# jmhb0/view_neti

Measured on AMD Instinct MI355X. Metric: TI train steps/sec (SD-1.5 512^2 bs=4 per GPU), higher is better.
Workload: dtype f16; 1 GPU; learnable_mode 0, sd15 shapes, 512x512 fp16, bs=4/GPU, grad_accum 1, full train step (VAE+16xCLIP+UNet fwd/bwd+AdamW); global_batch=4, parallelism=dp1, rccl_ranks=1, hipgraph=True

## Files before the change

include/vneti.h:

```cpp
#ifndef VNETI_H
#define VNETI_H
#include <stddef.h>
#include <stdint.h>

#ifdef __cplusplus
extern "C" {
#endif

#define VNETI_ABI_VERSION 1

int vneti_version(void);
int vneti_precision(void);
int vneti_last_error(char* buf, size_t n);

typedef struct vneti_gemm_desc {
  const void* A;
  const void* B;
  void* C;
  long long lda, ldb, ldc;
  int M, N, K;
  int batch;
  long long strideA, strideB, strideC;
  const float* bias;
  const void* rowadd;
  long long ld_rowadd;
  int rows_per_group;
  const void* resid;
  long long ldr;
  float alpha;
  int act;
  int out_f32;
  int conv_mode;
  int Hi, Wi, Ci, Ho, Wo, stride, pad_t, pad_l, ups;
  long long ldx;
  int tile_hint;
  void* workspace;
  long long workspace_bytes;
  int split_k;
  const void* gate_src;
  long long ld_gate;
  int gate_act;
  void* C2;
  long long ldc2;
  int act2;
  void* gn_sums;
  int gn_hw, gn_cpg, gn_groups, gn_slots;
  int geglu;
  int conv_korder;
} vneti_gemm_desc;

int vneti_gemm_f16(const vneti_gemm_desc* d, void* stream);
int vneti_gemm_select_tile(int M, int N, int batch);
int vneti_gemm_select_split(int M, int N, int K, int batch, int tile_hint, long long workspace_bytes);

int vneti_im2col3x3_small(const void* x, int x_is_f32, long long sb, long long sc, long long sy,
                          long long sx, void* out, int Bn, int C, int Hi, int Wi, int Ho, int Wo,
                          int stride, int pad_t, int pad_l, void* stream);

int vneti_conv3x3_in(const void* x, int x_is_f32, long long sb, long long sc, long long sy, long long sx,
                     const void* w_packed, const float* bias, void* out, long long ldo, int Bn, int C, int H, int W,
                     int Co, void* gn_sums, int gn_groups, int gn_slots, void* stream);

int vneti_transpose_f16(const void* in, long long ld_in, long long stride_in, void* out,
                        long long ld_out, long long stride_out, int rows, int cols, int batch,
                        void* stream);
#define VNETI_TRANSPOSE_MAX 4
typedef struct vneti_transpose_desc {
  const void* inp;
  long long ld_in, stride_in;
  void* out;
  long long ld_out, stride_out;
  int rows, cols, batch, _pad;
} vneti_transpose_desc;
int vneti_transpose_f16_multi(const vneti_transpose_desc* descs, int n, void* stream);

long long vneti_groupnorm_ws_floats(int Bn, int HW, int C, int G);
int vneti_groupnorm_fwd(const void* x, long long ldx, void* y, long long ldy, const float* gamma,
                        const float* beta, float* mean, float* rstd, float* ws, int Bn, int HW,
                        int C, int G, float eps, int silu, void* stream);
int vneti_groupnorm_fwd_sums(const void* x, long long ldx, void* y, long long ldy, const float* gamma,
                             const float* beta, const void* sums, int slots, float* mean, float* rstd,
                             int Bn, int HW, int C, int G, float eps, int silu, void* stream);
int vneti_groupnorm_fwd_2l(const void* x, long long ldx, void* y, long long ldy, const float* gamma,
                           const float* beta, void* sums, int slots, float* mean, float* rstd, int Bn, int HW,
                           int C, int G, float eps, int silu, void* stream);
int vneti_groupnorm_bwd_2l(const void* dy, long long lddy, const void* x, long long ldx, const float* gamma,
                           const float* beta, const float* mean, const float* rstd, void* dx, long long lddx,
                           const void* dx_accum, long long ldacc, void* sums, int slots, float* ws, int Bn,
                           int HW, int C, int G, int silu, void* stream);
int vneti_groupnorm_bwd(const void* dy, long long lddy, const void* x, long long ldx,
                        const float* gamma, const float* beta, const float* mean,
                        const float* rstd, void* dx, long long lddx, const void* dx_accum,
                        long long ldacc, float* ws, int Bn, int HW, int C, int G, int silu,
                        void* stream);

int vneti_layernorm_fwd(const void* x, int x_is_f32, long long ldx, void* y, long long ldy,
                        const float* gamma, const float* beta, float* mean, float* rstd, int rows,
                        int C, float eps, void* stream);
int vneti_layernorm_bwd(const void* dy, int dy_is_f32, long long lddy, const void* x,
                        int x_is_f32, long long ldx, const float* gamma, const float* mean,
                        const float* rstd, void* dx, int dx_is_f32, long long lddx,
                        const void* dx_accum, long long ldacc, void* dx_f16_copy, long long ldcopy,
                        int rows, int C, void* stream);

int vneti_attn_fwd(const void* Q, long long ldq, const void* K, long long ldk, const void* V,
                   long long ldv, void* O, long long ldo, float* lse, int Bn, int H, int Nq,
                   int Nk, int D, float scale, int causal, void* stream);
int vneti_attn_bwd_delta(const void* dO, long long lddo, const void* O, long long ldo,
                         float* delta, int Bn, int H, int Nq, int D, void* stream);
int vneti_attn_bwd_dq(const void* Q, long long ldq, const void* K, long long ldk, const void* V,
                      long long ldv, const void* dO, long long lddo, const float* lse, float* delta,
                      const void* O, long long ldo, void* dQ, long long lddq, int Bn, int H, int Nq,
                      int Nk, int D, float scale, int causal, void* stream);
int vneti_attn_bwd_dkv(const void* Q, long long ldq, const void* K, long long ldk, const void* V,
                       long long ldv, const void* dO, long long lddo, const float* lse,
                       const float* delta, void* dK, long long lddk, void* dV, long long lddv,
                       int Bn, int H, int Nq, int Nk, int D, float scale, int causal, float* ws,
                       long long ws_floats, void* stream);
int vneti_attn_bwd_small(const void* Q, long long ldq, const void* K, long long ldk, const void* V, long long ldv,
                         const void* dO, long long lddo, const void* O, long long ldo, const float* lse, void* dQ,
                         long long lddq, void* dK, long long lddk, void* dV, long long lddv, int Bn, int H, int N, int D,
                         float scale, int causal, void* stream);
int vneti_softmax_rows_f16(void* x, long long ld, int rows, int cols, void* stream);

int vneti_add_f16(const void* a, long long lda, const void* b, long long ldb, void* out,
                  long long ldo, int rows, int cols, void* stream);
int vneti_geglu_fwd(const void* p, long long ldp, void* out, long long ldo, int rows, int C4,
                    void* stream);
int vneti_geglu_bwd(const void* dy, long long lddy, const void* p, long long ldp, void* dp,
                    long long lddp, int rows, int C4, void* stream);
int vneti_act_fwd_f16(const void* x, void* y, long long n, int act, void* stream);
int vneti_act_bwd_f16(const void* dy, const void* x, void* dx, long long n, int act, void* stream);
int vneti_timestep_embedding(const void* t, void* out, int Bn, int dim, void* stream);
int vneti_sum2x2_f16(const void* in, long long ldi, void* out, long long ldo, int Bn, int H, int W,
                     int C, void* stream);
int vneti_rng_fill_normal(void* out_f32, long long n, const void* state, unsigned stream_id,
                          void* stream);
int vneti_rng_fill_randint(void* out_i64, int n, int high, const void* state, unsigned stream_id,
                           void* stream);
int vneti_rng_advance(void* state, void* stream);
int vneti_nested_dropout_mask(float* mask, int nl, int Bn, int hidden, float prob, const void* state,
                              unsigned stream_id, void* stream);
int vneti_sample_add_noise(const void* moments, long long ldm, const float* eps,
                           const float* noise, const void* timesteps_i64,
                           const float* alphas_cumprod, float scaling, int v_prediction,
                           float* latents, float* noisy, float* target, int Bn, int Lc, int HW,
                           void* stream);
int vneti_latent_sample(const void* moments, long long ldm, const float* eps, float scaling, float* latents, int Bn,
                        int Lc, int HW, void* stream);
int vneti_add_noise(const float* latents, const float* noise, const void* timesteps_i64, const float* alphas_cumprod,
                    int v_prediction, float* noisy, float* target, int Bn, int Lc, int HW, void* stream);
int vneti_cfg_sampler_step(const void* pred, long long ldp, float* x, float* m_prev, float* x_in, int Bn,
                           int Lc, int HW, float guidance, float alpha_t, float sigma_t, float cx,
                           float c0, float c1, int v_prediction, void* stream);
int vneti_cfg_sampler_step_table(const void* pred, long long ldp, float* x, float* m_prev, float* x_in,
                                 int Bn, int Lc, int HW, float guidance, const float* coef_table,
                                 const int* step, int v_prediction, void* stream);
int vneti_cfg_sampler_step_noise(const void* pred, long long ldp, float* x, float* m_prev, float* x_in,
                                 const float* noise, int Bn, int Lc, int HW, float guidance, float alpha_t,
                                 float sigma_t, float cx, float c0, float c1, float cn, int v_prediction, void* stream);
int vneti_cfg_sampler_step_noise_table(const void* pred, long long ldp, float* x, float* m_prev, float* x_in, int Bn,
                                       int Lc, int HW, float guidance, const float* coef_table,
                                       const float* noise_table, const int* step, int v_prediction, void* stream);
int vneti_table_fill_i64(void* dst_i64, int n, const void* table_i64, const int* step, void* stream);
int vneti_counter_advance(int* counter, void* stream);
int vneti_conv1x1_nchw_f32(const float* x, const float* W, const float* bias, float* out, int Bn, int Ci,
                           int Co, int HW, float in_scale, void* stream);
int vneti_image_postprocess(const void* img, long long ldi, float* out, long long n_pix, int channels,
                            void* stream);
int vneti_mse_loss_grad(const void* pred, long long ldp, const float* target, void* dpred,
                        long long lddp, float* loss_sum, const float* loss_scale, int Bn, int Lc,
                        int HW, void* stream);
int vneti_mse_loss_per_sample(const void* pred, long long ldp, const float* target, float* out, float* ws, int Bn, int Lc,
                              int HW, void* stream);
long long vneti_mse_loss_per_sample_ws_floats(int Bn, int HW);
#define VNETI_OPT_CHECK 1
#define VNETI_OPT_APPLY 2
#define VNETI_OPT_FINISH 4
#define VNETI_OPT_ALL 7
int vneti_adamw_flat(float* p, const float* g, float* m, float* v, long long n, const float* hyper,
                     float* scaler, int* step, int growth_interval, int phases, void* stream);
int vneti_adamw_segments(float* p, const float* g, float* m, float* v, long long seg_len, int n_seg,
                         int* seg_step, const int* active, int n_active, const float* hyper,
                         float* scaler, int* step, int growth_interval, int phases, void* stream);
long long vneti_grad_sumsq_ws_doubles(long long len, int n_active);
int vneti_grad_sumsq(const float* g, long long len, const int* active, int n_active, void* ws, void* stream);
#define VNETI_NORM_OUT_FLOATS 5
int vneti_grad_norm_finish(const void* ws_object, long long n_object, const void* ws_view, long long n_view,
                           const float* scaler, const float* hyper, const float* max_norm, float* out, float* ring,
                           const int* count, int rows, int row_floats, void* stream);
int vneti_adamw_flat_clipped(float* p, const float* g, float* m, float* v, long long n, const float* hyper,
                             float* scaler, int* step, int growth_interval, int phases, const float* clip_coef,
                             void* stream);
int vneti_adamw_segments_clipped(float* p, const float* g, float* m, float* v, long long seg_len, int n_seg,
                                 int* seg_step, const int* active, int n_active, const float* hyper, float* scaler,
                                 int* step, int growth_interval, int phases, const float* clip_coef, void* stream);
#define VNETI_TELEMETRY_SEQ 0
#define VNETI_TELEMETRY_MICRO 1
#define VNETI_TELEMETRY_CLOSED 2
#define VNETI_TELEMETRY_NORM_OBJECT 3
#define VNETI_TELEMETRY_NORM_VIEW 4
#define VNETI_TELEMETRY_NORM_TOTAL 5
#define VNETI_TELEMETRY_FINITE 6
#define VNETI_TELEMETRY_CLIP_COEF 7
#define VNETI_TELEMETRY_LOSS_SCALE 8
#define VNETI_TELEMETRY_LR 9
#define VNETI_TELEMETRY_HEADER 10
int vneti_train_record(float* ring, int* count, int rows, int row_floats, int first_micro, const void* timesteps_i64,
                       const float* losses, int Bn, void* stream);

long long vneti_mapper_num_params(int enc_dim, int hidden, int D, int has_bypass);
long long vneti_mapper_save_floats(int R, int enc_dim, int hidden);
long long vneti_mapper_rowgrad_floats(int R, int hidden, int D, int has_bypass);
int vneti_mapper_fwd(const float* params, const int* slot, long long slot_stride, const float* data,
                     int nfeat, const float* w_enc,
                     const float* hidden_mask, float norm_scale, float* word, float* bypass,
                     float* save, int R, int enc_dim, int hidden, int D, int has_bypass, const float* enc_in,
                     void* stream);
int vneti_mapper_fwd_slots(const float* params, const int* slots, long long slot_stride, int Bn, const float* data,
                           int nfeat, const float* w_enc, const float* hidden_mask, float norm_scale, float* word,
                           float* bypass, float* save, int R, int enc_dim, int hidden, int D, int has_bypass,
                           const float* enc_in, void* stream);
int vneti_mapper_bwd(const float* params, const int* slot, long long slot_stride,
                     const float* hidden_mask, float norm_scale,
                     const float* word, const float* dword_src, const int* dword_rows,
                     long long ld_src, const float* dbypass, const float* save, float* rowgrads,
                     float* grads, int accumulate, int R, int enc_dim, int hidden, int D,
                     int has_bypass, float* denc, void* stream);
long long vneti_mapper_legacy_input_params(int enc_dim, int pe_dim);
int vneti_mapper_legacy_input_fwd(const float* params_in, const int* slot, long long slot_stride,
                                  const void* timesteps_i64, const float* w_pe, float* enc_out, int nl, int Bn,
                                  int enc_dim, int pe_dim, void* stream);
int vneti_mapper_legacy_input_fwd_slots(const float* params_in, const int* slots, long long slot_stride,
                                        const void* timesteps_i64, const float* w_pe, float* enc_out, int nl, int Bn,
                                        int enc_dim, int pe_dim, void* stream);
int vneti_mapper_legacy_input_bwd(const void* timesteps_i64, const float* w_pe, const float* denc, float* grads_in,
                                  const int* slot, long long slot_stride, int accumulate, int nl, int Bn, int enc_dim,
                                  int pe_dim, void* stream);
int vneti_text_embed(const float* tok_emb, const float* pos_emb, const void* ids_i64,
                     const int* pos_obj, const float* word_obj, const int* pos_view,
                     const float* word_view, float* X, int nl, int Bn, int L, int D, void* stream);
int vneti_text_final_fwd(const float* last, const float* gamma, const float* beta, float eps,
                         const int* pos_obj, const float* bypass_obj, float alpha_obj,
                         int unconstrained_obj, const int* pos_view, const float* bypass_view,
                         float alpha_view, int unconstrained_view, float* norm_terms, void* ctx_k,
                         void* ctx_v, int nl, int Bn, int L, int D, void* stream);
int vneti_text_final_bwd(const float* last, const float* gamma, float eps, const int* pos_obj,
// ... 43 lines not shown
```

view_neti_amd/csrc/gemm_conv.hip:

```cpp
#include "common.h"
#include "gemm_args.h"
#include "../../include/vneti.h"

namespace {

template <int BM, int BN, int WM, int WN, bool F32OUT, bool DMA, int NSTG = 2, int EPI = 2, bool CONV = true>
__global__ __launch_bounds__((BM / WM) * (BN / WN) * 64) void gemm_kernel(
    const half_t* pA, const half_t* pB, uint32_t p_a_bytes, uint32_t p_b_bytes, int p_lda, int p_ldb, int pM, int pN, int pK,
    int p_tiles_m, int p_tiles_n, int p_split_conv , const GemmArgs gfull) {
  GemmArgs g = gfull;
  g.A = pA;
  g.B = pB;
  g.a_bytes = p_a_bytes;
  g.b_bytes = p_b_bytes;
  g.lda = p_lda;
  g.ldb = p_ldb;
  g.M = pM;
  g.N = pN;
  g.K = pK;
  g.tiles_m = p_tiles_m;
  g.tiles_n = p_tiles_n;
  g.kt_per_split = p_split_conv & 0xffff;
  g.ksplit = (p_split_conv >> 16) & 0xff;
  g.conv_mode = p_split_conv >> 24;
  static_assert(NSTG == 2 || ((NSTG == 3 || NSTG == 4) && DMA), "the LDS rings are LDS-DMA only");
  const half_t* const e_gate = EPI == 2 ? g.gate_src : nullptr;
  half_t* const e_C2 = EPI == 2 ? g.C2 : nullptr;
  const int e_geglu = EPI == 2 ? g.geglu : 0;
  const int e_act = EPI == 2 ? g.act : 0;
  float* const e_gn_sums = EPI >= 1 ? g.gn_sums : nullptr;
  const half_t* const e_rowadd = EPI >= 1 ? g.rowadd : nullptr;
  const int e_conv = CONV ? g.conv_mode : 0;
  constexpr int NWM = BM / WM, NWN = BN / WN;
  constexpr int NT = NWM * NWN * 64;
  constexpr int RSTEP = NT / 8;
  constexpr int A_IT = BM / RSTEP, B_IT = BN / RSTEP;
  constexpr int STAGE_BYTES = (BM + BN) * 128;
  constexpr int CS_LD = F32OUT ? (BN + 4) : (BN + 8);
  constexpr int CS_BYTES = BM * CS_LD * (F32OUT ? 4 : 2);
  constexpr int LDS_BYTES = (NSTG * STAGE_BYTES > CS_BYTES) ? NSTG * STAGE_BYTES : CS_BYTES;
  constexpr int GN_IMG = 5, GN_NG = BN / 4 + 2;
  constexpr int GN_BYTES = (F32OUT || EPI == 0) ? 0 : GN_IMG * GN_NG * 4 * 8;
  __shared__ __attribute__((aligned(16))) char smem[LDS_BYTES + GN_BYTES];

  const int tid = threadIdx.x;
  const int lane = tid & 63;
  const int wave = __builtin_amdgcn_readfirstlane(tid >> 6);
  const int wm0 = (wave / NWN) * WM;
  const int wn0 = (wave % NWN) * WN;

  int nblk = g.tiles_m * g.tiles_n;
  int bid = blockIdx.x;
  {
    int q = nblk >> 3, r = nblk & 7, xcd = bid & 7, idx = bid >> 3;
    bid = (xcd < r ? xcd * (q + 1) : r * (q + 1) + (xcd - r) * q) + idx;
  }
  const int tile_m = bid / g.tiles_n;
  const int tile_n = bid - tile_m * g.tiles_n;
  const int m0 = tile_m * BM;
  const int n0 = tile_n * BN;
  const int bz = blockIdx.y;
  const int kz = blockIdx.z;

  const half_t* Ab = g.A + (long long)bz * g.strideA;
  const half_t* Bb = g.B + (long long)bz * g.strideB;
  __amdgpu_buffer_rsrc_t rsA = vn_make_rsrc(Ab, g.a_bytes);
  __amdgpu_buffer_rsrc_t rsB = vn_make_rsrc(Bb, g.b_bytes);

  const int lrow = tid >> 3;
  const int gchunk = DMA ? ((tid & 7) ^ ((lrow >> 1) & 7)) : (tid & 7);

  const float rcp_hw = CONV ? __builtin_amdgcn_rcpf((float)(g.Ho * g.Wo)) : 0.f, rcp_wo = CONV ? __builtin_amdgcn_rcpf((float)g.Wo) : 0.f;
  int a_off[A_IT];
  int a_py[A_IT], a_px[A_IT], a_bh[A_IT];
#pragma unroll
  for (int i = 0; i < A_IT; ++i) {
    int m = m0 + lrow + RSTEP * i;
    bool ok = m < g.M;
    if (e_conv == 0) {
      a_off[i] = ok ? (int)((long long)m * g.lda * 2) + gchunk * 16 : -1;
      a_py[i] = a_px[i] = a_bh[i] = 0;
    } else {
      int rem, ox;
      const int b = vn_divmod(m, g.Ho * g.Wo, rcp_hw, rem);
      const int oy = vn_divmod(rem, g.Wo, rcp_wo, ox);
      a_bh[i] = ok ? b * g.Hi : -1;
      if (e_conv == 1) {
        a_py[i] = oy * g.stride - g.pad_t;
        a_px[i] = ox * g.stride - g.pad_l;
      } else {
        a_py[i] = oy + g.pad_t;
        a_px[i] = ox + g.pad_l;
      }
      a_off[i] = ((b * g.Hi + a_py[i]) * g.Wi + a_px[i]) * g.ldx2 + gchunk * 16;
    }
  }
  int b_off[B_IT];
#pragma unroll
  for (int i = 0; i < B_IT; ++i) {
    int n = n0 + lrow + RSTEP * i;
    b_off[i] = (n < g.N) ? (int)((long long)n * g.ldb * 2) + gchunk * 16 : -1;
  }

  u32x4 ra[DMA ? 1 : A_IT], rb[DMA ? 1 : B_IT];

  auto a_offset = [&](int i, int k0, int dy, int dx, int tapoff) -> uint32_t {
    if (e_conv == 0) return a_off[i] < 0 ? VN_OOB : (uint32_t)(a_off[i] + k0 * 2);
    bool ok = a_bh[i] >= 0;
    if (e_conv == 1 && !g.ups) {
      int iy = a_py[i] + dy, ix = a_px[i] + dx;
      ok = ok && (unsigned)iy < (unsigned)g.Hi && (unsigned)ix < (unsigned)g.Wi;
      return ok ? (uint32_t)(a_off[i] + tapoff) : VN_OOB;
    }
    int iy, ix;
    if (e_conv == 1) {
      iy = a_py[i] + dy;
      ix = a_px[i] + dx;
      ok = ok && (unsigned)iy < (unsigned)(2 * g.Hi) && (unsigned)ix < (unsigned)(2 * g.Wi);
      iy >>= 1;
      ix >>= 1;
    } else {
      int ty = a_py[i] - dy, tx = a_px[i] - dx;
      ok = ok && ty >= 0 && tx >= 0;
      if (g.stride == 2) {
        ok = ok && ((ty | tx) & 1) == 0;
        ty >>= 1;
        tx >>= 1;
      }
      iy = ty;
      ix = tx;
      ok = ok && iy < g.Hi && ix < g.Wi;
    }
    return ok ? (uint32_t)(((a_bh[i] + iy) * g.Wi + ix) * g.ldx2 + tapoff) : VN_OOB;
  };

  uint32_t a_cur[A_IT], b_cur[B_IT];
#pragma unroll
  for (int i = 0; i < B_IT; ++i) b_cur[i] = b_off[i] < 0 ? VN_OOB : (uint32_t)b_off[i];

  auto issue = [&](int kt, int stage, bool first) {
    const int k0 = kt * 64;
    bool recompute = first;
    int dy = 0, dx = 0, tapoff = 0;
    if (e_conv != 0) {
      int tap, ci0;
      if (g.korder) {
        const int chunk = kt / 9;
        tap = kt - chunk * 9;
        ci0 = chunk << 6;
        recompute = true;
      } else {
        tap = k0 / g.Ci;
        ci0 = k0 - tap * g.Ci;
        recompute = recompute || ci0 == 0;
// ... 272 lines not shown
      }
      s_lo = q_lo = s_hi = q_hi = 0.f;
    };
    for (int idx = tid; idx < BM * CPR; idx += NT) {
      int r = idx / CPR, c = (idx - r * CPR) * 8;
      int m = m0 + r, n = n0 + c;
      const bool valid = m < g.M && n < g.N;
      if (gn) {
        int gn_rem;
        const int img = valid ? vn_divmod(m, g.gn_hw, rcp_gnhw, gn_rem) : gn_img;
        if (__any(img != gn_img)) {
          gn_flush();
          gn_img = img;
        }
      }
      if (!valid) continue;
      half8 v = as_half8(*reinterpret_cast<const u32x4*>(smem + ((size_t)r * CS_LD + c) * 2));
      int ra_rem;
      const half_t* radd = e_rowadd ? e_rowadd + (long long)vn_divmod(m, g.rows_per_group, rcp_rpg, ra_rem) * g.ld_rowadd + n : nullptr;
      if (n + 8 <= g.N) {
        if (radd) {
          half8 t = *reinterpret_cast<const half8*>(radd);
          v = vn_add8(v, t);
        }
        if (Rb) {
          half8 rr = *reinterpret_cast<const half8*>(Rb + (long long)m * g.ldr + n);
          v = vn_add8(v, rr);
        }
        if (e_geglu == 2) {
          const half_t* pp = e_gate + (long long)m * g.ld_gate + 2 * n;
#pragma unroll
          for (int c2 = 0; c2 < 2; ++c2) {
            const half8 pre = *reinterpret_cast<const half8*>(pp + 8 * c2);
            half8 o;
#pragma unroll
            for (int e = 0; e < 4; ++e) {
              const float d = (float)v[4 * c2 + e], hh = (float)pre[e], gg = (float)pre[4 + e];
              float cdf, xpdf;
              vn_gelu_parts(gg, cdf, xpdf);
              o[e] = (half_t)(d * gg * cdf);
              o[4 + e] = (half_t)(d * hh * (cdf + xpdf));
            }
            vn_st16_wt(rsC, (uint32_t)(((long long)m * g.ldc + 2 * n + 8 * c2) * 2), o);
          }
          continue;
        }
        if (e_gate) {
          half8 pre = *reinterpret_cast<const half8*>(e_gate + (long long)m * g.ld_gate + n);
#pragma unroll
          for (int e = 0; e < 8; ++e) v[e] = (half_t)((float)v[e] * act_grad((float)pre[e], g.gate_act));
        }
        if (e_geglu == 1 || (e_C2 && e_geglu == 0)) vn_st16_wt_saved(rsC, (uint32_t)(((long long)m * g.ldc + n) * 2), v);
        else vn_st16_wt(rsC, (uint32_t)(((long long)m * g.ldc + n) * 2), v);
        if (e_geglu == 1) {
          half4 o2;
#pragma unroll
          for (int e = 0; e < 4; ++e) o2[e] = (half_t)((float)v[e] * vn_gelu_erf((float)v[4 + e]));
          *reinterpret_cast<half4*>(e_C2 + (long long)m * g.ldc2 + (n >> 1)) = o2;
        }
        if (gn) {
#pragma unroll
          for (int e = 0; e < 8; ++e) {
            const float x = (float)v[e];
            if (e < gn_split) {
              s_lo += x;
              q_lo += x * x;
            } else {
              s_hi += x;
              q_hi += x * x;
            }
          }
        }
        if (e_C2 && e_geglu == 0) {
          half8 o2;
#pragma unroll
          for (int e = 0; e < 8; ++e) o2[e] = (half_t)apply_act((float)v[e], g.act2);
          vn_st16_wt(rsC2, (uint32_t)(((long long)m * g.ldc2 + n) * 2), o2);
        }
      } else {
        for (int e = 0; e < 8 && n + e < g.N; ++e) {
          float x = (float)v[e];
          if (radd) x = (float)(half_t)(x + (float)radd[e]);
          if (Rb) x = (float)(half_t)(x + (float)Rb[(long long)m * g.ldr + n + e]);
          if (e_gate) x = (float)(half_t)(x * act_grad((float)e_gate[(long long)m * g.ld_gate + n + e], g.gate_act));
          Cb[(long long)m * g.ldc + n + e] = (half_t)x;
          if (e_C2) e_C2[(long long)m * g.ldc2 + n + e] = (half_t)apply_act((float)(half_t)x, g.act2);
          if (gn) {
            const float xs = (float)(half_t)x;
            if (e < gn_split) {
              s_lo += xs;
              q_lo += xs * xs;
            } else {
              s_hi += xs;
              q_hi += xs * xs;
            }
          }
        }
      }
    }
    if (gn) {
      gn_flush();
      __syncthreads();
      const int slot = tile_m % g.gn_slots;
      for (int i = tid; i < GN_IMG * GN_NG; i += NT) {
        const vn_u64* src = gacc + 4 * i;
        if ((src[0] | src[1] | src[2] | src[3]) == 0) continue;
        const int img = gn_img0 + i / GN_NG, grp = gn_g0t + i % GN_NG;
        vn_u64* dst = reinterpret_cast<vn_u64*>(e_gn_sums) + (((long long)img * g.gn_slots + slot) * g.gn_G + grp) * 4;
#pragma unroll
        for (int w = 0; w < 4; ++w) atomicAdd(dst + w, src[w]);
      }
    }
  }
}

__global__ __launch_bounds__(256) void splitk_reduce_kernel(
    float* p_ws, void* pC, const float* p_bias, const void* p_resid, const half_t* p_rowadd, int pM, int pN, int p_batch,
    int p_ksplit, int p_ldc, int p_ldr, const GemmArgs gfull) {
  GemmArgs g = gfull;
  g.ws = p_ws;
  g.C = pC;
  g.bias = p_bias;
  g.resid = p_resid;
  g.rowadd = p_rowadd;
  g.M = pM;
  g.N = pN;
  g.batch = p_batch;
  g.ksplit = p_ksplit;
  g.ldc = p_ldc;
  g.ldr = p_ldr;
  const unsigned n4 = (unsigned)(g.N + 3) / 4;
  const unsigned gid = blockIdx.x * 256u + threadIdx.x;
  const unsigned total = (unsigned)g.batch * (unsigned)g.M * n4;
  if (gid >= total) return;
  const unsigned row = gid / n4;
  const int c = (int)(gid - row * n4) * 4;
  const int bz = g.batch > 1 ? (int)(row / (unsigned)g.M) : 0;
  const int m = (int)(row - (unsigned)bz * (unsigned)g.M);
  const int ne = min(4, g.N - c);
  const long long zstride = (long long)g.batch * g.M * g.N;
  const float* p0 = g.ws + ((long long)bz * g.M + m) * g.N + c;
  if ((g.N & 3) == 0 && ((g.ldc | g.ldr | g.ld_rowadd | g.ld_gate | g.ldc2) & 3) == 0) {
    const long long co = (long long)bz * g.strideC + (long long)m * g.ldc + c;
    const long long ro = (long long)bz * g.strideC + (long long)m * g.ldr + c;
    f32x4 bv = {0.f, 0.f, 0.f, 0.f}, rf = {0.f, 0.f, 0.f, 0.f};
    half4 rh = {0, 0, 0, 0}, ra = {0, 0, 0, 0}, gt = {0, 0, 0, 0};
    if (g.bias) bv = *reinterpret_cast<const f32x4*>(g.bias + c);
    if (g.resid) {
      if (g.out_f32) rf = *reinterpret_cast<const f32x4*>(reinterpret_cast<const float*>(g.resid) + ro);
      else rh = *reinterpret_cast<const half4*>(reinterpret_cast<const half_t*>(g.resid) + ro);
    }
    if (g.rowadd) ra = *reinterpret_cast<const half4*>(g.rowadd + (long long)(m / g.rows_per_group) * g.ld_rowadd + c);
    if (g.gate_src) gt = *reinterpret_cast<const half4*>(g.gate_src + (long long)m * g.ld_gate + c);
    f32x4 v = {0.f, 0.f, 0.f, 0.f};
    int z = 0;
    for (; z + 4 <= g.ksplit; z += 4) {
      const f32x4 t0 = *reinterpret_cast<const f32x4*>(p0 + (z + 0) * zstride);
      const f32x4 t1 = *reinterpret_cast<const f32x4*>(p0 + (z + 1) * zstride);
      const f32x4 t2 = *reinterpret_cast<const f32x4*>(p0 + (z + 2) * zstride);
      const f32x4 t3 = *reinterpret_cast<const f32x4*>(p0 + (z + 3) * zstride);
      v += t0;
      v += t1;
      v += t2;
      v += t3;
    }
    for (; z < g.ksplit; ++z) v += *reinterpret_cast<const f32x4*>(p0 + z * zstride);
    float x[4];
#pragma unroll
    for (int e = 0; e < 4; ++e) {
      x[e] = v[e] * g.alpha;
      if (g.bias) x[e] += bv[e];
      x[e] = apply_act(x[e], g.act);
    }
    if (g.out_f32) {
      f32x4 o = {x[0], x[1], x[2], x[3]};
      if (g.resid) o += rf;
      vn_st16_wt(vn_make_rsrc(g.C, 0x7fffffffu), (uint32_t)(co * 4), o);
    } else {
      half4 o, o2;
#pragma unroll
      for (int e = 0; e < 4; ++e) {
        float y = (float)(half_t)x[e];
        if (g.rowadd) y = (float)(half_t)(y + (float)ra[e]);
        if (g.resid) y = (float)(half_t)(y + (float)rh[e]);
        if (g.gate_src) y = (float)(half_t)(y * act_grad((float)gt[e], g.gate_act));
        o[e] = (half_t)y;
        o2[e] = (half_t)apply_act((float)(half_t)y, g.act2);
      }
      *reinterpret_cast<half4*>(reinterpret_cast<half_t*>(g.C) + co) = o;
      if (g.C2) *reinterpret_cast<half4*>(g.C2 + (long long)m * g.ldc2 + c) = o2;
    }
    return;
  }
  float v[4] = {0.f, 0.f, 0.f, 0.f};
  for (int z = 0; z < g.ksplit; ++z) {
    const float* p = p0 + z * zstride;
    for (int e = 0; e < ne; ++e) v[e] += p[e];
  }
  for (int e = 0; e < ne; ++e) {
    float x = v[e] * g.alpha;
    if (g.bias) x += g.bias[c + e];
    x = apply_act(x, g.act);
    if (g.out_f32) {
      if (g.resid) x += reinterpret_cast<const float*>(g.resid)[(long long)bz * g.strideC + (long long)m * g.ldr + c + e];
      reinterpret_cast<float*>(g.C)[(long long)bz * g.strideC + (long long)m * g.ldc + c + e] = x;
    } else {
      x = (float)(half_t)x;
      if (g.rowadd) x = (float)(half_t)(x + (float)g.rowadd[(long long)(m / g.rows_per_group) * g.ld_rowadd + c + e]);
      if (g.resid)
        x = (float)(half_t)(x + (float)reinterpret_cast<const half_t*>(g.resid)[(long long)bz * g.strideC + (long long)m * g.ldr + c + e]);
      if (g.gate_src) x = (float)(half_t)(x * act_grad((float)g.gate_src[(long long)m * g.ld_gate + c + e], g.gate_act));
      reinterpret_cast<half_t*>(g.C)[(long long)bz * g.strideC + (long long)m * g.ldc + c + e] = (half_t)x;
      if (g.C2) g.C2[(long long)m * g.ldc2 + c + e] = (half_t)apply_act((float)(half_t)x, g.act2);
    }
  }
}

inline int epilogue_level(const GemmArgs& g) {
  if (g.gate_src || g.C2 || g.geglu || g.act) return 2;
  return (g.gn_sums || g.rowadd) ? 1 : 0;
}

template <int BM, int BN, int WM, int WN, bool F32OUT, bool DMA, int NSTG>
void launch_variant(const GemmArgs& g, dim3 grid, hipStream_t st) {
  const dim3 block((BM / WM) * (BN / WN) * 64);
#define VN_GO(E, C)                                                                                                        \
  hipLaunchKernelGGL((gemm_kernel<BM, BN, WM, WN, F32OUT, DMA, NSTG, E, C>), grid, block, 0, st, g.A, g.B, g.a_bytes, g.b_bytes, \
                     (int)g.lda, (int)g.ldb, g.M, g.N, g.K, g.tiles_m, g.tiles_n, g.kt_per_split | (g.ksplit << 16) | (g.conv_mode << 24), g)
  if constexpr (F32OUT) {
    if (g.conv_mode) { if (g.act) VN_GO(2, true); else VN_GO(0, true); }
    else { if (g.act) VN_GO(2, false); else VN_GO(0, false); }
  } else {
    const int epi = epilogue_level(g);
    if (g.conv_mode) { if (epi == 2) VN_GO(2, true); else if (epi == 1) VN_GO(1, true); else VN_GO(0, true); }
    else { if (epi == 2) VN_GO(2, false); else if (epi == 1) VN_GO(1, false); else VN_GO(0, false); }
  }
#undef VN_GO
}

inline void launch_reduce(const GemmArgs& g, hipStream_t st) {
  if (g.ksplit > 1) {
    long long total = (long long)g.batch * g.M * ((g.N + 3) / 4);
    hipLaunchKernelGGL(splitk_reduce_kernel, dim3((unsigned)cdivl(total, 256)), dim3(256), 0, st, g.ws, g.C, g.bias, g.resid,
                       g.rowadd, g.M, g.N, g.batch, g.ksplit, (int)g.ldc, (int)g.ldr, g);
  }
}

template <int BM, int BN, int WM, int WN, bool DMA>
int launch_cfg(GemmArgs& g, bool f32out, hipStream_t st) {
  g.tiles_m = cdiv(g.M, BM);
  g.tiles_n = cdiv(g.N, BN);
  dim3 grid(g.tiles_m * g.tiles_n, g.batch, g.ksplit);
  if (f32out) launch_variant<BM, BN, WM, WN, true, DMA, 2>(g, grid, st);
  else launch_variant<BM, BN, WM, WN, false, DMA, 2>(g, grid, st);
  launch_reduce(g, st);
  return vneti_check_launch("gemm_kernel");
}

template <int BM, int BN, int WM, int WN, int NSTG = 3>
int launch_cfg_ring(GemmArgs& g, bool f32out, hipStream_t st) {
  g.tiles_m = cdiv(g.M, BM);
  g.tiles_n = cdiv(g.N, BN);
  dim3 grid(g.tiles_m * g.tiles_n, g.batch, g.ksplit);
  if (f32out) launch_variant<BM, BN, WM, WN, true, true, NSTG>(g, grid, st);
  else launch_variant<BM, BN, WM, WN, false, true, NSTG>(g, grid, st);
  launch_reduce(g, st);
  return vneti_check_launch("gemm_kernel");
}

template <int BM, int BN, int WM, int WN, bool DMA>
int launch_cfg_f16(GemmArgs& g, hipStream_t st) {
  g.tiles_m = cdiv(g.M, BM);
  g.tiles_n = cdiv(g.N, BN);
  dim3 grid(g.tiles_m * g.tiles_n, g.batch, g.ksplit);
  launch_variant<BM, BN, WM, WN, false, DMA, 2>(g, grid, st);
  launch_reduce(g, st);
  return vneti_check_launch("gemm_kernel");
}

struct TileDims {
  int bm, bn;
};
constexpr int kMaxTile = 18;
constexpr TileDims kTiles[kMaxTile + 1] = {{0, 0},     {128, 128}, {128, 64},  {64, 64},  {256, 128}, {256, 256}, {256, 128}, {256, 128},
                                          {256, 128}, {128, 128}, {128, 128}, {128, 64},  {64, 64},   {128, 128}, {128, 64},  {64, 64},
                                          {256, 256}, {256, 128}, {256, 128}};

int select_tile(int M, int N, int batch) {
  long long t256 = (long long)cdiv(M, 256) * cdiv(N, 128) * batch;
  long long t128 = (long long)cdiv(M, 128) * cdiv(N, 128) * batch;
  long long t12864 = (long long)cdiv(M, 128) * cdiv(N, 64) * batch;
  if (N <= 64) return (M >= 2048) ? 2 : 3;
  (void)t256;
  if (t128 >= 384) return 1;
  if (t12864 >= 384) return 2;
  return 3;
}

int select_ksplit(int M, int N, int K, int batch, int tile, long long ws_floats) {
  if (ws_floats <= 0) return 1;
  const int nk = K / 64;
  long long tiles = (long long)cdiv(M, kTiles[tile].bm) * cdiv(N, kTiles[tile].bn) * batch;
  if (tiles >= 256 || nk < 16) return 1;
  int s = (int)(512 / tiles);
  if (s > nk / 8) s = nk / 8;
  if (s > 16) s = 16;
  while (s > 1 && (long long)s * batch * M * N > ws_floats) --s;
  return s < 2 ? 1 : s;
}

}

extern "C" int vneti_gemm_select_tile(int M, int N, int batch) { return select_tile(M, N, batch > 0 ? batch : 1); }

extern "C" int vneti_gemm_select_split(int M, int N, int K, int batch, int tile_hint, long long workspace_bytes) {
  if (batch <= 0) batch = 1;
  int cfg = tile_hint >= 100 ? tile_hint - 100 : tile_hint;
  if (cfg == 0) cfg = select_tile(M, N, batch);
  if (cfg < 1 || cfg > kMaxTile || K % 64 != 0) return -1;
  int ks = select_ksplit(M, N, K, batch, cfg, workspace_bytes / 4);
  const int nk = K / 64;
  if (ks > nk) ks = nk;
  if (ks < 1) ks = 1;
  return cdiv(nk, cdiv(nk, ks));
}

extern "C" int vneti_gemm_f16(const vneti_gemm_desc* d, void* stream) {
  VN_REQUIRE(d != nullptr, "gemm: null descriptor");
  VN_REQUIRE(d->A && d->B && d->C, "gemm: null operand pointer");
  VN_REQUIRE(d->M > 0 && d->N > 0 && d->K > 0, "gemm: bad shape M=%d N=%d K=%d", d->M, d->N, d->K);
  VN_REQUIRE(d->K % 64 == 0, "gemm: K=%d must be a multiple of 64", d->K);
  VN_REQUIRE(d->ldb % 8 == 0, "gemm: ldb=%lld must be a multiple of 8", d->ldb);
  int batch = d->batch > 0 ? d->batch : 1;
  GemmArgs g;
  memset(&g, 0, sizeof(g));
  g.A = (const half_t*)d->A;
  g.B = (const half_t*)d->B;
  g.C = d->C;
  g.bias = d->bias;
  g.rowadd = (const half_t*)d->rowadd;
  g.resid = d->resid;
  g.gate_src = (const half_t*)d->gate_src;
  g.ld_gate = d->ld_gate;
  g.gate_act = d->gate_act;
  g.C2 = (half_t*)d->C2;
  g.ldc2 = d->ldc2;
  g.act2 = d->act2;
  g.gn_sums = (float*)d->gn_sums;
  g.gn_hw = d->gn_hw;
  g.gn_cpg = d->gn_cpg;
  g.gn_G = d->gn_groups;
  g.gn_slots = d->gn_slots;
  g.geglu = d->geglu;
  g.lda = d->lda;
  g.ldb = d->ldb;
  g.ldc = d->ldc;
  g.ld_rowadd = d->ld_rowadd;
  g.ldr = d->ldr;
  g.strideA = d->strideA;
  g.strideB = d->strideB;
  g.strideC = d->strideC;
  g.M = d->M;
  g.N = d->N;
  g.K = d->K;
  g.batch = batch;
  g.rows_per_group = d->rows_per_group > 0 ? d->rows_per_group : 1;
  g.alpha = d->alpha;
  g.act = d->act;
  g.out_f32 = d->out_f32 ? 1 : 0;
  g.conv_mode = d->conv_mode;
  long long a_bytes;
  if (d->conv_mode == 0) {
    VN_REQUIRE(d->lda % 8 == 0, "gemm: lda=%lld must be a multiple of 8", d->lda);
    a_bytes = ((long long)(d->M - 1) * d->lda + d->K) * 2;
  } else {
    VN_REQUIRE(d->conv_mode == 1 || d->conv_mode == 2, "gemm: bad conv_mode %d", d->conv_mode);
    VN_REQUIRE(d->Ci > 0 && d->Ci % 64 == 0, "conv: Ci=%d must be a multiple of 64", d->Ci);
    VN_REQUIRE(d->K == 9 * d->Ci, "conv: K=%d must equal 9*Ci=%d", d->K, 9 * d->Ci);
    VN_REQUIRE(d->stride == 1 || d->stride == 2, "conv: stride %d unsupported", d->stride);
    VN_REQUIRE(d->Ho > 0 && d->Wo > 0 && d->M % (d->Ho * d->Wo) == 0, "conv: M=%d not a multiple of Ho*Wo", d->M);
    VN_REQUIRE(d->ldx % 8 == 0, "conv: ldx must be a multiple of 8");
    VN_REQUIRE(!(d->ups && d->conv_mode != 1), "conv: fused upsample only in forward gather mode");
    VN_REQUIRE(!(d->ups && d->stride != 1), "conv: fused upsample needs stride 1");
    g.Hi = d->Hi;
    g.Wi = d->Wi;
    g.Ci = d->Ci;
    g.Ho = d->Ho;
    g.Wo = d->Wo;
    g.stride = d->stride;
    g.pad_t = d->pad_t;
    g.pad_l = d->pad_l;
    g.ups = d->ups;
    g.ldx2 = (int)(d->ldx * 2);
    VN_REQUIRE(!d->conv_korder || d->Ci % 64 == 0, "conv: conv_korder=1 needs Ci=%d to be a multiple of 64", d->Ci);
    g.korder = d->conv_korder ? 1 : 0;
    long long nb = d->M / (d->Ho * d->Wo);
    a_bytes = nb * d->Hi * d->Wi * d->ldx * 2;
  }
  long long b_bytes = ((long long)(d->N - 1) * d->ldb + d->K) * 2;
  VN_REQUIRE(a_bytes < 0x7fffffffLL && b_bytes < 0x7fffffffLL, "gemm: operand larger than 2 GiB");
  g.a_bytes = (uint32_t)a_bytes;
  g.b_bytes = (uint32_t)b_bytes;
  if (!d->out_f32) {
    VN_REQUIRE(d->ldc % 8 == 0 || d->N < 8, "gemm: ldc=%lld must be a multiple of 8", d->ldc);
  }
  VN_REQUIRE_OUT("gemm C", vn_out_bytes(d->M, d->ldc, d->N, d->out_f32 ? 4 : 2, batch, d->strideC));
  if (d->C2) VN_REQUIRE_OUT("gemm C2", vn_out_bytes(d->M, d->ldc2, d->geglu == 1 ? d->N / 2 : d->N, 2));
  hipStream_t st = (hipStream_t)stream;
  bool f32 = d->out_f32 != 0;
  VN_REQUIRE(!(f32 && d->rowadd), "gemm: rowadd is only supported for f16 output");
  if (d->gate_src || d->C2) {
    VN_REQUIRE(!f32 && batch == 1, "gemm: gate/C2 epilogues need f16 output and batch 1");
    VN_REQUIRE(!d->gate_src || (d->gate_act >= 1 && d->gate_act <= 3 && d->ld_gate % 8 == 0), "gemm: bad gate arguments");
    VN_REQUIRE(!d->C2 || (d->act2 >= 0 && d->act2 <= 3 && d->ldc2 % 8 == 0), "gemm: bad C2 arguments");
  }

  if (d->geglu) {
    VN_REQUIRE(d->geglu == 1 || d->geglu == 2, "gemm: geglu must be 0, 1 or 2");
    VN_REQUIRE(!f32 && batch == 1 && d->N % 8 == 0, "gemm: geglu needs f16 output, batch 1 and N %% 8 == 0");
    VN_REQUIRE(d->split_k == 1, "gemm: geglu needs split_k = 1 (it lives in the fused epilogue)");
    VN_REQUIRE(!d->gn_sums, "gemm: geglu and gn_sums are exclusive");
    if (d->geglu == 1) {
      VN_REQUIRE(d->C2 && d->ldc2 % 4 == 0 && !d->gate_src, "gemm: geglu forward needs C2 ([M][N/2]) and no gate");
    } else {
      VN_REQUIRE(d->gate_src && d->ld_gate % 8 == 0 && !d->C2 && !d->resid && !d->rowadd,
                 "gemm: geglu backward needs gate_src ([M][2N] saved pre-activation) and a plain epilogue");
      VN_REQUIRE(d->ldc % 8 == 0, "gemm: geglu backward writes [M][2N]: ldc %% 8");
    }
  }
  if (d->gn_sums) {
    VN_REQUIRE(!f32 && batch == 1, "gemm: gn_sums needs f16 output and batch 1");
    VN_REQUIRE(d->gn_hw >= 64 && d->gn_cpg >= 4 && d->gn_groups > 0 && d->gn_slots > 0 && d->N == d->gn_cpg * d->gn_groups &&
                   d->M % d->gn_hw == 0 && (d->gn_cpg >= 8 || d->gn_cpg == 4),
               "gemm: bad gn_sums geometry hw=%d cpg=%d G=%d", d->gn_hw, d->gn_cpg, d->gn_groups);
    VN_REQUIRE(d->split_k == 1, "gemm: gn_sums needs split_k = 1 (the statistics live in the fused epilogue)");
  }

  int cfg = d->tile_hint;
  bool dma = true;
  if (cfg >= 100) {
    dma = false;
    cfg -= 100;
  }
  if (cfg == 0) cfg = select_tile(d->M, d->N, batch);
  VN_REQUIRE(cfg >= 1 && cfg <= kMaxTile, "gemm: unknown tile_hint %d", d->tile_hint);
  if (cfg == 18 &&
      (d->conv_mode < 1 || d->conv_mode > 2 || d->stride != 1 || d->ups || d->pad_t != 1 || d->pad_l != 1 || d->Hi != d->Ho ||
       d->Wi != d->Wo || (d->Ho & 15) || (d->Wo & 15) || (d->Ci & 63) || !d->conv_korder || batch != 1 || f32))
    cfg = 17;
  if (cfg == 18 && d->gn_sums && (d->gn_cpg & 1)) cfg = 17;
  if ((cfg == 16 || cfg == 17) && (!dma || (d->conv_mode && (d->ups || (d->conv_mode == 2 && d->stride == 2))) ||
                    (d->gn_sums && (d->gn_cpg & 1)) ||
                    (d->M >= (1 << 24) && (d->conv_mode || d->rowadd || d->gn_sums)))) cfg = cfg == 16 ? 5 : 7;
  if ((cfg == 5 || cfg == 16) && f32) cfg = 4;
  if (cfg == 17 && f32) cfg = 7;
  if ((cfg == 6 || cfg == 7) && !dma) cfg = 4;
  if (cfg >= 10 && !dma) cfg = kTiles[cfg].bm == 128 ? (kTiles[cfg].bn == 128 ? 1 : 2) : 3;
  long long ws_floats = d->workspace ? d->workspace_bytes / 4 : 0;
  int ks = d->split_k;
  if (ks == 0) ks = select_ksplit(d->M, d->N, d->K, batch, cfg, ws_floats);
  if (ks < 1) ks = 1;
  const int nk = d->K / 64;
  if (ks > nk) ks = nk;
  if (ks > 1) {
    VN_REQUIRE(d->workspace && (long long)ks * batch * d->M * d->N <= ws_floats,
               "gemm: split_k=%d needs %lld workspace bytes", ks, (long long)ks * batch * d->M * d->N * 4);
    VN_REQUIRE(batch == 1 || (d->strideC != 0), "gemm: batched split-K needs strideC");
    VN_REQUIRE((long long)batch * d->M * ((d->N + 3) / 4) < 0x7fffffffLL, "gemm: split-K output larger than 2^31 chunks");
    VN_REQUIRE_OUT("gemm split-K workspace", (long long)ks * batch * d->M * d->N * 4);
  }
  if (cfg == 18 && ks > d->Ci / 64) ks = d->Ci / 64;
  g.ksplit = ks;
  g.kt_per_split = cdiv(nk, ks);
  g.ksplit = cdiv(nk, g.kt_per_split);
  VN_REQUIRE(g.ksplit <= 255 && g.kt_per_split <= 0xffff, "gemm: split_k=%d / K=%d out of range", g.ksplit, d->K);
  g.ws = (float*)d->workspace;

#define LAUNCH(BM, BN, WM, WN) \
  return dma ? launch_cfg<BM, BN, WM, WN, true>(g, f32, st) : launch_cfg<BM, BN, WM, WN, false>(g, f32, st)
  switch (cfg) {
    case 1: LAUNCH(128, 128, 64, 64);
    case 2: LAUNCH(128, 64, 64, 32);
    case 3: LAUNCH(64, 64, 32, 32);
    case 4: LAUNCH(256, 128, 64, 64);
    case 6: return launch_cfg_ring<256, 128, 64, 64>(g, f32, st);
    case 7: return launch_cfg_ring<256, 128, 64, 32>(g, f32, st);
    case 8: LAUNCH(256, 128, 64, 32);
    case 9: LAUNCH(128, 128, 64, 32);
    case 10: return launch_cfg_ring<128, 128, 64, 32>(g, f32, st);
    case 11: return launch_cfg_ring<128, 64, 64, 32>(g, f32, st);
    case 12: return launch_cfg_ring<64, 64, 32, 32>(g, f32, st);
    case 13: return launch_cfg_ring<128, 128, 64, 32, 4>(g, f32, st);
    case 14: return launch_cfg_ring<128, 64, 64, 32, 4>(g, f32, st);
    case 15: return launch_cfg_ring<64, 64, 32, 32, 4>(g, f32, st);
    case 16:
    case 17:
    case 18: {
      const int rc = vneti_launch_gemm8(&g, cfg == 16 ? 256 : 128, cfg == 18 ? 1 : 0, st);
      if (rc != VNETI_OK) return rc;
      launch_reduce(g, st);
      return vneti_check_launch("gemm8_kernel");
    }
    default:
      return dma ? launch_cfg_f16<256, 256, 64, 64, true>(g, st) : launch_cfg_f16<256, 256, 64, 64, false>(g, st);
  }
#undef LAUNCH
}
```

view_neti_amd/csrc/norms.hip:

```cpp
#include "common.h"
#include "../../include/vneti.h"

namespace {

#ifndef GN_APPLY_U
#define GN_APPLY_U 4
#endif
struct GNGeom {
  int Bn, HW, C, G, cpg, CC, TX, TY, rps, nslab;
  double inv_n;
};

__device__ __forceinline__ void vn_mean_rstd(double s0, double s1, double inv_n, float eps, float& m, float& r) {
  const double mu = s0 * inv_n;
  const double var = s1 * inv_n - mu * mu;
  const float v = fmaxf((float)var, 0.f) + eps;
  float y = __builtin_amdgcn_rsqf(v);
  y = y * (1.5f - 0.5f * v * y * y);
  m = (float)mu;
  r = y;
}

__device__ __forceinline__ void gn_thread_coords(const GNGeom& g, int& tx, int& ty, bool& active) {
  int tid = threadIdx.x;
  tx = tid % g.TX;
  ty = tid / g.TX;
  active = ty < g.TY;
}

template <bool BWD, bool SILU, bool SLOTS = false>
__global__ __launch_bounds__(256) void gn_stats_kernel(GNGeom g, const half_t* __restrict__ x, long long ldx,
                                                       const half_t* __restrict__ dy, long long lddy,
                                                       const float* __restrict__ gamma,
                                                       const float* __restrict__ beta,
                                                       const float* __restrict__ mean,
                                                       const float* __restrict__ rstd,
                                                       float* __restrict__ part, int slots = 0) {
  __shared__ vn_u64 gacc[64 * 4];
  const int slab = blockIdx.x, b = blockIdx.y;
  for (int i = threadIdx.x; i < 4 * g.G; i += 256) gacc[i] = 0;
  __syncthreads();
  int tx, ty;
  bool active;
  gn_thread_coords(g, tx, ty, active);
  const int r0 = slab * g.rps;
  const int r1 = min(r0 + g.rps, g.HW);
  if (active) {
    for (int cb = 0; cb < g.CC; cb += g.TX) {
      const int cx = cb + tx;
      if (cx >= g.CC) break;
      const int ch0 = cx * 8;
      const int g0 = ch0 / g.cpg;
      const int split = (g0 + 1) * g.cpg - ch0;
      float ga[8], be[8];
      float mlo = 0.f, rlo = 0.f, mhi = 0.f, rhi = 0.f;
      if (BWD) {
#pragma unroll
        for (int j = 0; j < 8; ++j) {
          ga[j] = gamma[ch0 + j];
          be[j] = beta[ch0 + j];
        }
        mlo = mean[b * g.G + g0];
        rlo = rstd[b * g.G + g0];
        if (split < 8) {
          mhi = mean[b * g.G + g0 + 1];
          rhi = rstd[b * g.G + g0 + 1];
        }
      }
      float a_lo = 0.f, b_lo = 0.f, a_hi = 0.f, b_hi = 0.f;
      constexpr int U = 4;
      for (int rb = r0 + ty; rb < r1; rb += U * g.TY) {
        half8 xu[U], du[U];
#pragma unroll
        for (int u = 0; u < U; ++u) {
          const int r = rb + u * g.TY;
          const long long row = (long long)b * g.HW + (r < r1 ? r : rb);
          xu[u] = *reinterpret_cast<const half8*>(x + row * ldx + ch0);
          if (BWD) du[u] = *reinterpret_cast<const half8*>(dy + row * lddy + ch0);
        }
#pragma unroll
        for (int u = 0; u < U; ++u) {
          if (rb + u * g.TY >= r1) continue;
          const half8 xv = xu[u];
          if (!BWD) {
#pragma unroll
            for (int j = 0; j < 8; ++j) {
              float v = (float)xv[j];
              if (j < split) {
                a_lo += v;
                b_lo += v * v;
              } else {
                a_hi += v;
                b_hi += v * v;
              }
            }
          } else {
            const half8 dv = du[u];
#pragma unroll
            for (int j = 0; j < 8; ++j) {
              const bool lo = j < split;
              float xh = ((float)xv[j] - (lo ? mlo : mhi)) * (lo ? rlo : rhi);
              float d = (float)dv[j];
              if (SILU) {
                float z = xh * ga[j] + be[j];
                float s = vn_sigmoid(z);
                d *= s * (1.f + z * (1.f - s));
              }
              float dxh = d * ga[j];
              if (lo) {
                a_lo += dxh;
                b_lo += dxh * xh;
              } else {
                a_hi += dxh;
                b_hi += dxh * xh;
              }
            }
          }
        }
      }
      vn_fx_add2(&gacc[4 * g0], a_lo, b_lo);
      if (split < 8) vn_fx_add2(&gacc[4 * (g0 + 1)], a_hi, b_hi);
    }
  }
  __syncthreads();
  if constexpr (SLOTS) {
    vn_u64* p = reinterpret_cast<vn_u64*>(part) + ((long long)b * slots + slab % slots) * (4 * g.G);
    for (int i = threadIdx.x; i < 4 * g.G; i += 256) atomicAdd(p + i, gacc[i]);
  } else {
    float* p = part + ((long long)b * g.nslab + slab) * (2 * g.G);
    for (int i = threadIdx.x; i < 2 * g.G; i += 256) p[i] = (float)vn_fx_decode(gacc[2 * i], gacc[2 * i + 1]);
  }
}

template <bool BWD>
__global__ __launch_bounds__(256) void gn_finalize_kernel(GNGeom g, const float* __restrict__ part, float eps,
                                                          float* __restrict__ o0, float* __restrict__ o1) {
  __shared__ double red[2][256];
  const int b = blockIdx.x;
  const int lpg = 256 / g.G;
  const int gi = threadIdx.x % g.G, ln = threadIdx.x / g.G;
  double s0 = 0.0, s1 = 0.0;
  if (ln < lpg) {
    for (int s = ln; s < g.nslab; s += lpg) {
      const float* p = part + ((long long)b * g.nslab + s) * (2 * g.G) + 2 * gi;
      s0 += (double)p[0];
      s1 += (double)p[1];
    }
  }
  red[0][threadIdx.x] = s0;
  red[1][threadIdx.x] = s1;
  __syncthreads();
  if (threadIdx.x < g.G) {
    s0 = 0.0;
// ... 68 lines not shown
      for (int sl = 0; sl < 8; ++sl) {
        const vn_u64* p = p0 + (long long)(sl < slots ? sl : 0) * g.G * 4;
#pragma unroll
        for (int w = 0; w < 4; ++w) v[sl][w] = p[w];
      }
#pragma unroll
      for (int sl = 0; sl < 8; ++sl)
#pragma unroll
        for (int w = 0; w < 4; ++w) t[w] += sl < slots ? v[sl][w] : 0;
      for (int s0 = 8; s0 < slots; s0 += 8) {
#pragma unroll
        for (int sl = 0; sl < 8; ++sl) {
          const vn_u64* p = p0 + (long long)(s0 + sl < slots ? s0 + sl : 0) * g.G * 4;
#pragma unroll
          for (int w = 0; w < 4; ++w) v[sl][w] = p[w];
        }
#pragma unroll
        for (int sl = 0; sl < 8; ++sl)
#pragma unroll
          for (int w = 0; w < 4; ++w) t[w] += s0 + sl < slots ? v[sl][w] : 0;
      }
      const double s0 = vn_fx_decode(t[0], t[1]), s1 = vn_fx_decode(t[2], t[3]);
      if constexpr (!BWD) {
        float m, r;
        vn_mean_rstd(s0, s1, g.inv_n, eps, m, r);
        s_stat[0][gi] = m;
        s_stat[1][gi] = r;
        if (slab == 0) {
          mean_out[b * g.G + gi] = m;
          rstd_out[b * g.G + gi] = r;
        }
      } else {
        s_stat[0][gi] = (float)(s0 * g.inv_n);
        s_stat[1][gi] = (float)(s1 * g.inv_n);
      }
    }
    __syncthreads();
  }
  if (!active) return;
  const int r0 = slab * g.rps;
  const int r1 = min(r0 + g.rps, g.HW);
  for (int cb = 0; cb < g.CC; cb += g.TX) {
    const int cx = cb + tx;
    if (cx >= g.CC) break;
    const int ch0 = cx * 8;
    const int g0 = ch0 / g.cpg;
    const int split = (g0 + 1) * g.cpg - ch0;
    const int g1 = (split < 8) ? g0 + 1 : g0;
    float ga[8], be[8];
    {
      const f32x4 ga0 = *reinterpret_cast<const f32x4*>(gamma + ch0), ga1 = *reinterpret_cast<const f32x4*>(gamma + ch0 + 4);
      const f32x4 be0 = *reinterpret_cast<const f32x4*>(beta + ch0), be1 = *reinterpret_cast<const f32x4*>(beta + ch0 + 4);
#pragma unroll
      for (int j = 0; j < 4; ++j) {
        ga[j] = ga0[j];
        ga[4 + j] = ga1[j];
        be[j] = be0[j];
        be[4 + j] = be1[j];
      }
    }
    float mlo, rlo, mhi, rhi;
    if constexpr (FROM_SUMS && !BWD) {
      mlo = s_stat[0][g0];
      rlo = s_stat[1][g0];
      mhi = s_stat[0][g1];
      rhi = s_stat[1][g1];
    } else {
      mlo = mean[b * g.G + g0];
      rlo = rstd[b * g.G + g0];
      mhi = mean[b * g.G + g1];
      rhi = rstd[b * g.G + g1];
    }
    float c1lo = 0.f, c2lo = 0.f, c1hi = 0.f, c2hi = 0.f;
    if constexpr (BWD && FROM_SUMS) {
      c1lo = s_stat[0][g0];
      c2lo = s_stat[1][g0];
      c1hi = s_stat[0][g1];
      c2hi = s_stat[1][g1];
    } else if (BWD) {
      c1lo = c1[b * g.G + g0];
      c2lo = c2[b * g.G + g0];
      c1hi = c1[b * g.G + g1];
      c2hi = c2[b * g.G + g1];
    }
    int r = r0 + ty;
    float sc[8], sh[8];
    if (!BWD) {
#pragma unroll
      for (int j = 0; j < 8; ++j) {
        const bool lo = j < split;
        sc[j] = (lo ? rlo : rhi) * ga[j];
        sh[j] = fmaf(-(lo ? mlo : mhi), sc[j], be[j]);
      }
    }
    if (!BWD) {
      constexpr int U = GN_APPLY_U;
      for (; r + (U - 1) * g.TY < r1; r += U * g.TY) {
        half8 xv[U];
#pragma unroll
        for (int u = 0; u < U; ++u)
          xv[u] = __builtin_nontemporal_load(reinterpret_cast<const half8*>(x + ((long long)b * g.HW + r + u * g.TY) * ldx + ch0));
#pragma unroll
        for (int u = 0; u < U; ++u) {
          half8 ov;
#pragma unroll
          for (int j = 0; j < 8; ++j) {
            float z = fmaf((float)xv[u][j], sc[j], sh[j]);
            if (SILU) z = vn_silu(z);
            ov[j] = (half_t)z;
          }
          vn_st16_wt(rsO, (uint32_t)((((long long)b * g.HW + r + u * g.TY) * ldo + ch0) * 2), ov);
        }
      }
    }
    for (; r < r1; r += g.TY) {
      const long long row = (long long)b * g.HW + r;
      half8 xv = *reinterpret_cast<const half8*>(x + row * ldx + ch0);
      half8 ov;
      if (!BWD) {
#pragma unroll
        for (int j = 0; j < 8; ++j) {
          const bool lo = j < split;
          float xh = ((float)xv[j] - (lo ? mlo : mhi)) * (lo ? rlo : rhi);
          float z = xh * ga[j] + be[j];
          if (SILU) z = vn_silu(z);
          ov[j] = (half_t)z;
        }
      } else {
        half8 dv = *reinterpret_cast<const half8*>(dy + row * lddy + ch0);
        half8 av;
        if (accum) av = *reinterpret_cast<const half8*>(accum + row * ldacc + ch0);
#pragma unroll
        for (int j = 0; j < 8; ++j) {
          const bool lo = j < split;
          const float rs = lo ? rlo : rhi;
          float xh = ((float)xv[j] - (lo ? mlo : mhi)) * rs;
          float d = (float)dv[j];
          if (SILU) {
            float z = xh * ga[j] + be[j];
            float s = vn_sigmoid(z);
            d *= s * (1.f + z * (1.f - s));
          }
          float dxh = d * ga[j];
          float dx = rs * (dxh - (lo ? c1lo : c1hi) - xh * (lo ? c2lo : c2hi));
          if (accum) dx += (float)av[j];
          ov[j] = (half_t)dx;
        }
      }
      vn_st16_wt(rsO, (uint32_t)((row * ldo + ch0) * 2), ov);
    }
  }
}

template <bool BWD, bool SILU>
__global__ __launch_bounds__(512) void gn_small_kernel(int HW, int C, int G, const half_t* __restrict__ x, long long ldx,
                                                       const half_t* __restrict__ dy, long long lddy,
                                                       const float* __restrict__ gamma, const float* __restrict__ beta,
                                                       float* __restrict__ mean, float* __restrict__ rstd, float eps,
                                                       half_t* __restrict__ out, long long ldo,
                                                       const half_t* __restrict__ accum, long long ldacc, double inv_n) {
  constexpr int MAXU = BWD ? 16 : 20;
  constexpr int NTH = 512;
  __shared__ double red[2][8];
  __shared__ float stat[2];
  __shared__ float sga[128], sbe[128];
  const int gi = blockIdx.x, b = blockIdx.y;
  const int cpg = C / G, hp = cpg / 2;
  const int c0 = gi * cpg;
  const int total = HW * hp;
  const int lane = threadIdx.x & 63, wave = threadIdx.x >> 6;
  typedef half2v half2_t;
  for (int i = threadIdx.x; i < cpg; i += NTH) {
    sga[i] = gamma[c0 + i];
    sbe[i] = beta[c0 + i];
  }
  float m = 0.f, rs = 0.f;
  if (BWD) {
    m = mean[b * G + gi];
    rs = rstd[b * G + gi];
  }
  const half_t* xb = x + (long long)b * HW * ldx + c0;
  const half_t* dyb = BWD ? dy + (long long)b * HW * lddy + c0 : nullptr;
  const half_t* ab = accum ? accum + (long long)b * HW * ldacc + c0 : nullptr;
  const float rcp_hp = __builtin_amdgcn_rcpf((float)hp);
  half2_t xv[MAXU], dv[BWD ? MAXU : 1], av[BWD ? MAXU : 1];
  int rows[MAXU], cps[MAXU];
#pragma unroll
  for (int u = 0; u < MAXU; ++u) {
    const int p = threadIdx.x + u * NTH;
    int cp;
    rows[u] = vn_divmod(p, hp, rcp_hp, cp);
    cps[u] = cp * 2;
    xv[u] = half2_t{(half_t)0.f, (half_t)0.f};
    if (BWD) {
      dv[u] = xv[u];
      av[u] = xv[u];
    }
    if (p < total) {
      xv[u] = *reinterpret_cast<const half2_t*>(xb + (long long)rows[u] * ldx + cps[u]);
      if (BWD) {
        dv[u] = *reinterpret_cast<const half2_t*>(dyb + (long long)rows[u] * lddy + cps[u]);
        if (ab) av[u] = *reinterpret_cast<const half2_t*>(ab + (long long)rows[u] * ldacc + cps[u]);
      }
    }
  }
  __syncthreads();
  float s0 = 0.f, s1 = 0.f;
#pragma unroll
  for (int u = 0; u < MAXU; ++u) {
    if (!BWD) {
      const float v0 = (float)xv[u][0], v1 = (float)xv[u][1];
      s0 += v0 + v1;
      s1 += v0 * v0 + v1 * v1;
    } else if (threadIdx.x + u * NTH < total) {
#pragma unroll
      for (int j = 0; j < 2; ++j) {
        const float ga = sga[cps[u] + j];
        const float xh = ((float)xv[u][j] - m) * rs;
        float d = (float)dv[u][j];
        if (SILU) {
          const float z = xh * ga + sbe[cps[u] + j];
          const float sg = vn_sigmoid(z);
          d *= sg * (1.f + z * (1.f - sg));
        }
        const float dxh = d * ga;
        s0 += dxh;
        s1 += dxh * xh;
      }
    }
  }
  double d0 = (double)s0, d1 = (double)s1;
#pragma unroll
  for (int off = 32; off > 0; off >>= 1) {
    d0 += __shfl_xor(d0, off);
    d1 += __shfl_xor(d1, off);
  }
  if (lane == 0) {
    red[0][wave] = d0;
    red[1][wave] = d1;
  }
  __syncthreads();
  if (threadIdx.x == 0) {
    double t0 = 0.0, t1 = 0.0;
    for (int w = 0; w < (NTH >> 6); ++w) {
      t0 += red[0][w];
      t1 += red[1][w];
    }
    if (!BWD) {
      vn_mean_rstd(t0, t1, inv_n, eps, stat[0], stat[1]);
      mean[b * G + gi] = stat[0];
      rstd[b * G + gi] = stat[1];
    } else {
      stat[0] = (float)(t0 * inv_n);
      stat[1] = (float)(t1 * inv_n);
    }
  }
  __syncthreads();
  const float a0 = stat[0], a1 = stat[1];
  half_t* ob = out + (long long)b * HW * ldo + c0;
#pragma unroll
  for (int u = 0; u < MAXU; ++u) {
    if (threadIdx.x + u * NTH >= total) break;
    half2_t ov;
#pragma unroll
    for (int j = 0; j < 2; ++j) {
      const float ga = sga[cps[u] + j], be = sbe[cps[u] + j];
      if (!BWD) {
        float z = ((float)xv[u][j] - a0) * a1 * ga + be;
        if (SILU) z = vn_silu(z);
        ov[j] = (half_t)z;
      } else {
        const float xh = ((float)xv[u][j] - m) * rs;
        float d = (float)dv[u][j];
        if (SILU) {
          const float z = xh * ga + be;
          const float sg = vn_sigmoid(z);
          d *= sg * (1.f + z * (1.f - sg));
        }
        float dx = rs * (d * ga - a0 - xh * a1);
        if (ab) dx += (float)av[u][j];
        ov[j] = (half_t)dx;
      }
    }
    *reinterpret_cast<half2_t*>(ob + (long long)rows[u] * ldo + cps[u]) = ov;
  }
}

inline bool gn_use_small(int Bn, int HW, int C, int G, bool bwd) {
  const int cpg = C / G;
  if (cpg % 2 != 0 || cpg > 128 || getenv("VNETI_GN_NO_SMALL")) return false;
  return (long long)HW * cpg * 2 <= (bwd ? 32 : 40) * 1024 && Bn * G >= 64;
}

int gn_geom(GNGeom& g, int Bn, int HW, int C, int G) {
  if (Bn <= 0 || HW <= 0 || C <= 0 || G <= 0 || G > 64 || C % G != 0 || C % 8 != 0) return -1;
  g.Bn = Bn;
  g.HW = HW;
  g.C = C;
  g.G = G;
  g.cpg = C / G;
  if (g.cpg < 4) return -1;
  g.CC = C / 8;
  g.TX = g.CC < 256 ? g.CC : 256;
  g.TY = 256 / g.TX;
  int rps = 8192 / C;
  if (rps < 1) rps = 1;
  rps = ((rps + g.TY - 1) / g.TY) * g.TY;
  int nslab = (HW + rps - 1) / rps;
  while (nslab > 256) {
    rps *= 2;
    nslab = (HW + rps - 1) / rps;
  }
  g.rps = rps;
  g.nslab = nslab;
  g.inv_n = 1.0 / ((double)HW * g.cpg);
  return 0;
}

template <bool XF32>
__device__ __forceinline__ void ln_load(const void* x, long long off, float v[8]) {
  if (XF32) {
    const float* p = reinterpret_cast<const float*>(x) + off;
    f32x4 a = *reinterpret_cast<const f32x4*>(p);
    f32x4 b = *reinterpret_cast<const f32x4*>(p + 4);
#pragma unroll
    for (int j = 0; j < 4; ++j) {
      v[j] = a[j];
      v[4 + j] = b[j];
    }
  } else {
    half8 h = *reinterpret_cast<const half8*>(reinterpret_cast<const half_t*>(x) + off);
#pragma unroll
    for (int j = 0; j < 8; ++j) v[j] = (float)h[j];
  }
}
template <bool F32>
__device__ __forceinline__ void ln_store(void* y, long long off, const float v[8]) {
  const __amdgpu_buffer_rsrc_t rs = vn_make_rsrc(y, 0x7fffffffu);
  if (F32) {
    f32x4 a = {v[0], v[1], v[2], v[3]}, b = {v[4], v[5], v[6], v[7]};
    vn_st16_wt(rs, (uint32_t)(off * 4), a);
    vn_st16_wt(rs, (uint32_t)(off * 4 + 16), b);
  } else {
    half8 h;
#pragma unroll
    for (int j = 0; j < 8; ++j) h[j] = (half_t)v[j];
    vn_st16_wt(rs, (uint32_t)(off * 2), h);
  }
}

constexpr int LN_MAXC = 4;

__device__ __forceinline__ void ln_load_f32x8(const float* p, float v[8]) {
  const f32x4 a = *reinterpret_cast<const f32x4*>(p), b = *reinterpret_cast<const f32x4*>(p + 4);
#pragma unroll
  for (int j = 0; j < 4; ++j) {
    v[j] = a[j];
    v[4 + j] = b[j];
  }
}

template <bool XF32, int NC>
__global__ __launch_bounds__(256) void ln_fwd_kernel(const void* __restrict__ x, long long ldx,
                                                     half_t* __restrict__ y, long long ldy,
                                                     const float* __restrict__ gamma,
                                                     const float* __restrict__ beta, float* __restrict__ mean,
                                                     float* __restrict__ rstd, int rows, int C, float eps) {
  const int row = blockIdx.x * 4 + (threadIdx.x >> 6);
  const int lane = threadIdx.x & 63;
  if (row >= rows) return;
  const int CC = C / 8;
  float v[NC][8], ga[NC][8], be[NC][8];
  bool ok[NC];
  int cc[NC];
#pragma unroll
  for (int i = 0; i < NC; ++i) {
    const int c = lane + 64 * i;
    ok[i] = c < CC;
    cc[i] = ok[i] ? c : CC - 1;
    ln_load<XF32>(x, (long long)row * ldx + cc[i] * 8, v[i]);
  }
#pragma unroll
  for (int i = 0; i < NC; ++i) {
    ln_load_f32x8(gamma + cc[i] * 8, ga[i]);
    ln_load_f32x8(beta + cc[i] * 8, be[i]);
  }
  float s = 0.f;
#pragma unroll
  for (int i = 0; i < NC; ++i) {
    float t = 0.f;
#pragma unroll
    for (int j = 0; j < 8; ++j) t += v[i][j];
    s += ok[i] ? t : 0.f;
  }
  s = wave_sum(s);
  const float inv_c = __builtin_amdgcn_rcpf((float)C);
  const float m = s * inv_c;
  float q = 0.f;
#pragma unroll
  for (int i = 0; i < NC; ++i) {
    float t = 0.f;
#pragma unroll
    for (int j = 0; j < 8; ++j) {
      const float d = v[i][j] - m;
      t += d * d;
    }
    q += ok[i] ? t : 0.f;
  }
  q = wave_sum(q);
  const float rs = rsqrtf(q * inv_c + eps);
  if (lane == 0) {
    if (mean) mean[row] = m;
    if (rstd) rstd[row] = rs;
  }
#pragma unroll
  for (int i = 0; i < NC; ++i) {
    if (ok[i]) {
      float o[8];
#pragma unroll
      for (int j = 0; j < 8; ++j) o[j] = (v[i][j] - m) * rs * ga[i][j] + be[i][j];
      ln_store<false>(y, (long long)row * ldy + cc[i] * 8, o);
    }
  }
}

template <bool DYF32, bool XF32, bool DXF32, int NC>
__global__ __launch_bounds__(256) void ln_bwd_kernel(const void* __restrict__ dy, long long lddy,
                                                     const void* __restrict__ x, long long ldx,
                                                     const float* __restrict__ gamma,
                                                     const float* __restrict__ mean,
                                                     const float* __restrict__ rstd, void* __restrict__ dx,
                                                     long long lddx, const void* __restrict__ accum,
                                                     long long ldacc, half_t* __restrict__ dx16, long long ld16,
                                                     int rows, int C) {
  const int row = blockIdx.x * 4 + (threadIdx.x >> 6);
  const int lane = threadIdx.x & 63;
  if (row >= rows) return;
  const int CC = C / 8;
  float xh[NC][8], dh[NC][8], ac[NC][8];
  bool ok[NC];
  int cc[NC];
#pragma unroll
  for (int i = 0; i < NC; ++i) {
    const int c = lane + 64 * i;
    ok[i] = c < CC;
    cc[i] = ok[i] ? c : CC - 1;
    ln_load<XF32>(x, (long long)row * ldx + cc[i] * 8, xh[i]);
    ln_load<DYF32>(dy, (long long)row * lddy + cc[i] * 8, dh[i]);
  }
  const float m = mean[row], rs = rstd[row];
  if (accum) {
#pragma unroll
    for (int i = 0; i < NC; ++i) ln_load<DXF32>(accum, (long long)row * ldacc + cc[i] * 8, ac[i]);
  }
  float s1 = 0.f, s2 = 0.f;
#pragma unroll
  for (int i = 0; i < NC; ++i) {
    float g8[8];
    ln_load_f32x8(gamma + cc[i] * 8, g8);
    float t1 = 0.f, t2 = 0.f;
#pragma unroll
    for (int j = 0; j < 8; ++j) {
      xh[i][j] = (xh[i][j] - m) * rs;
      dh[i][j] = dh[i][j] * g8[j];
      t1 += dh[i][j];
      t2 += dh[i][j] * xh[i][j];
    }
    s1 += ok[i] ? t1 : 0.f;
    s2 += ok[i] ? t2 : 0.f;
  }
  const float inv_c = __builtin_amdgcn_rcpf((float)C);
  s1 = wave_sum(s1) * inv_c;
  s2 = wave_sum(s2) * inv_c;
#pragma unroll
  for (int i = 0; i < NC; ++i) {
    if (ok[i]) {
      float o[8];
#pragma unroll
      for (int j = 0; j < 8; ++j) o[j] = rs * (dh[i][j] - s1 - xh[i][j] * s2);
      if (accum) {
#pragma unroll
        for (int j = 0; j < 8; ++j) o[j] += ac[i][j];
      }
      ln_store<DXF32>(dx, (long long)row * lddx + cc[i] * 8, o);
      if (dx16) ln_store<false>(dx16, (long long)row * ld16 + cc[i] * 8, o);
    }
  }
}

constexpr int SM_MAXC = 8;
__global__ __launch_bounds__(256) void softmax_rows_kernel(half_t* __restrict__ x, long long ld, int cols) {
  __shared__ float red[4];
  half_t* p = x + (long long)blockIdx.x * ld;
  const int CC = cols / 8;
  float v[SM_MAXC][8];
  float mx = -INFINITY;
#pragma unroll
  for (int i = 0; i < SM_MAXC; ++i) {
    int c = threadIdx.x + 256 * i;
    if (c < CC) {
      half8 h = *reinterpret_cast<const half8*>(p + c * 8);
#pragma unroll
      for (int j = 0; j < 8; ++j) {
        v[i][j] = (float)h[j];
        mx = fmaxf(mx, v[i][j]);
      }
    }
  }
  mx = wave_max(mx);
  if ((threadIdx.x & 63) == 0) red[threadIdx.x >> 6] = mx;
  __syncthreads();
  mx = fmaxf(fmaxf(red[0], red[1]), fmaxf(red[2], red[3]));
  __syncthreads();
  float s = 0.f;
#pragma unroll
  for (int i = 0; i < SM_MAXC; ++i) {
    int c = threadIdx.x + 256 * i;
    if (c < CC) {
#pragma unroll
      for (int j = 0; j < 8; ++j) {
        v[i][j] = __expf(v[i][j] - mx);
        s += v[i][j];
      }
    }
  }
  s = wave_sum(s);
  if ((threadIdx.x & 63) == 0) red[threadIdx.x >> 6] = s;
  __syncthreads();
  s = red[0] + red[1] + red[2] + red[3];
  const float inv = 1.f / s;
#pragma unroll
  for (int i = 0; i < SM_MAXC; ++i) {
    int c = threadIdx.x + 256 * i;
    if (c < CC) {
      half8 h;
#pragma unroll
      for (int j = 0; j < 8; ++j) h[j] = (half_t)(v[i][j] * inv);
      *reinterpret_cast<half8*>(p + c * 8) = h;
    }
  }
}

}

extern "C" long long vneti_groupnorm_ws_floats(int Bn, int HW, int C, int G) {
  GNGeom g;
  if (gn_geom(g, Bn, HW, C, G) != 0) return -1;
  return (long long)Bn * g.nslab * 2 * G + 2LL * Bn * G;
}

extern "C" int vneti_groupnorm_fwd(const void* x, long long ldx, void* y, long long ldy, const float* gamma,
                                   const float* beta, float* mean, float* rstd, float* ws, int Bn, int HW,
                                   int C, int G, float eps, int silu, void* stream) {
  GNGeom g;
  VN_REQUIRE(gn_geom(g, Bn, HW, C, G) == 0, "groupnorm: unsupported shape B=%d HW=%d C=%d G=%d", Bn, HW, C, G);
  VN_REQUIRE(x && y && gamma && beta && mean && rstd && ws, "groupnorm_fwd: null pointer");
  VN_REQUIRE(ldx % 8 == 0 && ldy % 8 == 0, "groupnorm_fwd: ld must be a multiple of 8");
  VN_REQUIRE_OUT("groupnorm_fwd", vn_out_bytes((long long)Bn * HW, ldy, C, 2));
  hipStream_t st = (hipStream_t)stream;
  if (gn_use_small(Bn, HW, C, G, false)) {
    if (silu)
      hipLaunchKernelGGL((gn_small_kernel<false, true>), dim3(G, Bn), dim3(512), 0, st, HW, C, G, (const half_t*)x, ldx,
                         (const half_t*)nullptr, 0LL, gamma, beta, mean, rstd, eps, (half_t*)y, ldy,
                         (const half_t*)nullptr, 0LL, g.inv_n);
    else
      hipLaunchKernelGGL((gn_small_kernel<false, false>), dim3(G, Bn), dim3(512), 0, st, HW, C, G, (const half_t*)x, ldx,
                         (const half_t*)nullptr, 0LL, gamma, beta, mean, rstd, eps, (half_t*)y, ldy,
                         (const half_t*)nullptr, 0LL, g.inv_n);
    return vneti_check_launch("groupnorm_fwd");
  }
  dim3 grid(g.nslab, Bn);
  hipLaunchKernelGGL((gn_stats_kernel<false, false>), grid, dim3(256), 0, st, g, (const half_t*)x, ldx,
                     (const half_t*)nullptr, 0LL, gamma, beta, (const float*)nullptr, (const float*)nullptr, ws);
  hipLaunchKernelGGL((gn_finalize_kernel<false>), dim3(Bn), dim3(256), 0, st, g, (const float*)ws, eps, mean, rstd);
  if (silu)
    hipLaunchKernelGGL((gn_apply_kernel<false, true>), grid, dim3(256), 0, st, g, (const half_t*)x, ldx,
                       (const half_t*)nullptr, 0LL, gamma, beta, (const float*)mean, (const float*)rstd,
                       (const float*)nullptr, (const float*)nullptr, (half_t*)y, ldy, (const half_t*)nullptr, 0LL);
  else
    hipLaunchKernelGGL((gn_apply_kernel<false, false>), grid, dim3(256), 0, st, g, (const half_t*)x, ldx,
                       (const half_t*)nullptr, 0LL, gamma, beta, (const float*)mean, (const float*)rstd,
                       (const float*)nullptr, (const float*)nullptr, (half_t*)y, ldy, (const half_t*)nullptr, 0LL);
  return vneti_check_launch("groupnorm_fwd");
}

extern "C" int vneti_groupnorm_fwd_sums(const void* x, long long ldx, void* y, long long ldy, const float* gamma,
                                        const float* beta, const void* sums_v, int slots, float* mean, float* rstd,
                                        int Bn, int HW, int C, int G, float eps, int silu, void* stream) {
  const float* sums = reinterpret_cast<const float*>(sums_v);
  GNGeom g;
  VN_REQUIRE(gn_geom(g, Bn, HW, C, G) == 0, "groupnorm: unsupported shape B=%d HW=%d C=%d G=%d", Bn, HW, C, G);
  VN_REQUIRE(x && y && gamma && beta && sums && mean && rstd && slots > 0, "groupnorm_fwd_sums: null pointer");
  VN_REQUIRE(ldx % 8 == 0 && ldy % 8 == 0, "groupnorm_fwd_sums: ld % 8 != 0");
  VN_REQUIRE_OUT("groupnorm_fwd_sums", vn_out_bytes((long long)Bn * HW, ldy, C, 2));
  hipStream_t st = (hipStream_t)stream;
  dim3 grid(g.nslab, Bn);
  if (silu)
    hipLaunchKernelGGL((gn_apply_kernel<false, true, true>), grid, dim3(256), 0, st, g, (const half_t*)x, ldx,
                       (const half_t*)nullptr, 0LL, gamma, beta, (const float*)nullptr, (const float*)nullptr,
                       (const float*)nullptr, (const float*)nullptr, (half_t*)y, ldy, (const half_t*)nullptr, 0LL,
                       sums, slots, eps, mean, rstd);
  else
    hipLaunchKernelGGL((gn_apply_kernel<false, false, true>), grid, dim3(256), 0, st, g, (const half_t*)x, ldx,
                       (const half_t*)nullptr, 0LL, gamma, beta, (const float*)nullptr, (const float*)nullptr,
                       (const float*)nullptr, (const float*)nullptr, (half_t*)y, ldy, (const half_t*)nullptr, 0LL,
                       sums, slots, eps, mean, rstd);
  return vneti_check_launch("groupnorm_fwd_sums");
}

extern "C" int vneti_groupnorm_fwd_2l(const void* x, long long ldx, void* y, long long ldy, const float* gamma,
                                      const float* beta, void* sums_v, int slots, float* mean, float* rstd, int Bn, int HW,
                                      int C, int G, float eps, int silu, void* stream) {
  float* sums = reinterpret_cast<float*>(sums_v);
  GNGeom g;
  VN_REQUIRE(gn_geom(g, Bn, HW, C, G) == 0, "groupnorm: unsupported shape B=%d HW=%d C=%d G=%d", Bn, HW, C, G);
  VN_REQUIRE(x && y && gamma && beta && mean && rstd && sums && slots > 0, "groupnorm_fwd_2l: null pointer");
  VN_REQUIRE(ldx % 8 == 0 && ldy % 8 == 0, "groupnorm_fwd_2l: ld must be a multiple of 8");
  VN_REQUIRE_OUT("groupnorm_fwd_2l", vn_out_bytes((long long)Bn * HW, ldy, C, 2));
  if (gn_use_small(Bn, HW, C, G, false))
    return vneti_groupnorm_fwd(x, ldx, y, ldy, gamma, beta, mean, rstd, sums, Bn, HW, C, G, eps, silu, stream);
  hipStream_t st = (hipStream_t)stream;
  dim3 grid(g.nslab, Bn);
  hipLaunchKernelGGL((gn_stats_kernel<false, false, true>), grid, dim3(256), 0, st, g, (const half_t*)x, ldx,
                     (const half_t*)nullptr, 0LL, gamma, beta, (const float*)nullptr, (const float*)nullptr, sums, slots);
  return vneti_groupnorm_fwd_sums(x, ldx, y, ldy, gamma, beta, sums, slots, mean, rstd, Bn, HW, C, G, eps, silu, stream);
}

extern "C" int vneti_groupnorm_bwd_2l(const void* dy, long long lddy, const void* x, long long ldx, const float* gamma,
                                      const float* beta, const float* mean, const float* rstd, void* dx, long long lddx,
                                      const void* dx_accum, long long ldacc, void* sums_v, int slots, float* ws, int Bn,
                                      int HW, int C, int G, int silu, void* stream);

extern "C" int vneti_groupnorm_bwd(const void* dy, long long lddy, const void* x, long long ldx,
                                   const float* gamma, const float* beta, const float* mean, const float* rstd,
                                   void* dx, long long lddx, const void* dx_accum, long long ldacc, float* ws,
                                   int Bn, int HW, int C, int G, int silu, void* stream) {
  GNGeom g;
  VN_REQUIRE(gn_geom(g, Bn, HW, C, G) == 0, "groupnorm: unsupported shape B=%d HW=%d C=%d G=%d", Bn, HW, C, G);
  VN_REQUIRE(dy && x && gamma && beta && mean && rstd && dx && ws, "groupnorm_bwd: null pointer");
  VN_REQUIRE(ldx % 8 == 0 && lddy % 8 == 0 && lddx % 8 == 0 && ldacc % 8 == 0, "groupnorm_bwd: ld % 8 != 0");
  VN_REQUIRE_OUT("groupnorm_bwd", vn_out_bytes((long long)Bn * HW, lddx, C, 2));
  hipStream_t st = (hipStream_t)stream;
  if (gn_use_small(Bn, HW, C, G, true)) {
    if (silu)
      hipLaunchKernelGGL((gn_small_kernel<true, true>), dim3(G, Bn), dim3(512), 0, st, HW, C, G, (const half_t*)x, ldx,
                         (const half_t*)dy, lddy, gamma, beta, const_cast<float*>(mean), const_cast<float*>(rstd), 0.f,
                         (half_t*)dx, lddx, (const half_t*)dx_accum, ldacc, g.inv_n);
    else
      hipLaunchKernelGGL((gn_small_kernel<true, false>), dim3(G, Bn), dim3(512), 0, st, HW, C, G, (const half_t*)x, ldx,
                         (const half_t*)dy, lddy, gamma, beta, const_cast<float*>(mean), const_cast<float*>(rstd), 0.f,
                         (half_t*)dx, lddx, (const half_t*)dx_accum, ldacc, g.inv_n);
    return vneti_check_launch("groupnorm_bwd");
  }
  dim3 grid(g.nslab, Bn);
  float* c1 = ws + (long long)Bn * g.nslab * 2 * G;
  float* c2 = c1 + (long long)Bn * G;
  if (silu)
    hipLaunchKernelGGL((gn_stats_kernel<true, true>), grid, dim3(256), 0, st, g, (const half_t*)x, ldx,
                       (const half_t*)dy, lddy, gamma, beta, mean, rstd, ws);
  else
    hipLaunchKernelGGL((gn_stats_kernel<true, false>), grid, dim3(256), 0, st, g, (const half_t*)x, ldx,
                       (const half_t*)dy, lddy, gamma, beta, mean, rstd, ws);
  hipLaunchKernelGGL((gn_finalize_kernel<true>), dim3(Bn), dim3(256), 0, st, g, (const float*)ws, 0.f, c1, c2);
  if (silu)
    hipLaunchKernelGGL((gn_apply_kernel<true, true>), grid, dim3(256), 0, st, g, (const half_t*)x, ldx,
                       (const half_t*)dy, lddy, gamma, beta, mean, rstd, (const float*)c1, (const float*)c2,
                       (half_t*)dx, lddx, (const half_t*)dx_accum, ldacc);
  else
    hipLaunchKernelGGL((gn_apply_kernel<true, false>), grid, dim3(256), 0, st, g, (const half_t*)x, ldx,
                       (const half_t*)dy, lddy, gamma, beta, mean, rstd, (const float*)c1, (const float*)c2,
                       (half_t*)dx, lddx, (const half_t*)dx_accum, ldacc);
  return vneti_check_launch("groupnorm_bwd");
}

extern "C" int vneti_groupnorm_bwd_2l(const void* dy, long long lddy, const void* x, long long ldx, const float* gamma,
                                      const float* beta, const float* mean, const float* rstd, void* dx, long long lddx,
                                      const void* dx_accum, long long ldacc, void* sums_v, int slots, float* ws, int Bn,
                                      int HW, int C, int G, int silu, void* stream) {
  float* sums = reinterpret_cast<float*>(sums_v);
  GNGeom g;
  VN_REQUIRE(gn_geom(g, Bn, HW, C, G) == 0, "groupnorm: unsupported shape B=%d HW=%d C=%d G=%d", Bn, HW, C, G);
  VN_REQUIRE(dy && x && gamma && beta && mean && rstd && dx && sums && slots > 0, "groupnorm_bwd_2l: null pointer");
  VN_REQUIRE(ldx % 8 == 0 && lddy % 8 == 0 && lddx % 8 == 0 && ldacc % 8 == 0, "groupnorm_bwd_2l: ld % 8 != 0");
  VN_REQUIRE_OUT("groupnorm_bwd_2l", vn_out_bytes((long long)Bn * HW, lddx, C, 2));
  if (gn_use_small(Bn, HW, C, G, true))
    return vneti_groupnorm_bwd(dy, lddy, x, ldx, gamma, beta, mean, rstd, dx, lddx, dx_accum, ldacc, ws, Bn, HW, C, G, silu,
                               stream);
  hipStream_t st = (hipStream_t)stream;
  dim3 grid(g.nslab, Bn);
#define GN_BWD_2L(S)                                                                                                     \
  hipLaunchKernelGGL((gn_stats_kernel<true, S, true>), grid, dim3(256), 0, st, g, (const half_t*)x, ldx, (const half_t*)dy, \
                     lddy, gamma, beta, mean, rstd, sums, slots);                                                         \
  hipLaunchKernelGGL((gn_apply_kernel<true, S, true>), grid, dim3(256), 0, st, g, (const half_t*)x, ldx, (const half_t*)dy, \
                     lddy, gamma, beta, mean, rstd, (const float*)nullptr, (const float*)nullptr, (half_t*)dx, lddx,      \
                     (const half_t*)dx_accum, ldacc, (const float*)sums, slots, 0.f, (float*)nullptr, (float*)nullptr)
  if (silu) {
    GN_BWD_2L(true);
  } else {
    GN_BWD_2L(false);
  }
#undef GN_BWD_2L
  return vneti_check_launch("groupnorm_bwd_2l");
}

extern "C" int vneti_layernorm_fwd(const void* x, int x_is_f32, long long ldx, void* y, long long ldy,
                                   const float* gamma, const float* beta, float* mean, float* rstd, int rows,
                                   int C, float eps, void* stream) {
  VN_REQUIRE(x && y && gamma && beta, "layernorm_fwd: null pointer");
  VN_REQUIRE(rows > 0 && C > 0 && C % 8 == 0 && C <= 8 * 64 * LN_MAXC, "layernorm: unsupported C=%d", C);
  VN_REQUIRE(ldx % 8 == 0 && ldy % 8 == 0, "layernorm_fwd: ld % 8 != 0");
  VN_REQUIRE_OUT("layernorm_fwd", vn_out_bytes(rows, ldy, C, 2));
  hipStream_t st = (hipStream_t)stream;
  dim3 grid(cdiv(rows, 4));
#define LN_FWD(F, NCH)                                                                                        \
  hipLaunchKernelGGL((ln_fwd_kernel<F, NCH>), grid, dim3(256), 0, st, x, ldx, (half_t*)y, ldy, gamma, beta, mean, \
                     rstd, rows, C, eps)
  const int nc = cdiv(C / 8, 64);
  if (x_is_f32) {
    switch (nc) {
      case 1: LN_FWD(true, 1); break;
      case 2: LN_FWD(true, 2); break;
      case 3: LN_FWD(true, 3); break;
      default: LN_FWD(true, 4); break;
    }
  } else {
    switch (nc) {
      case 1: LN_FWD(false, 1); break;
      case 2: LN_FWD(false, 2); break;
      case 3: LN_FWD(false, 3); break;
      default: LN_FWD(false, 4); break;
    }
  }
#undef LN_FWD
  return vneti_check_launch("layernorm_fwd");
}

extern "C" int vneti_layernorm_bwd(const void* dy, int dy_is_f32, long long lddy, const void* x, int x_is_f32,
                                   long long ldx, const float* gamma, const float* mean, const float* rstd,
                                   void* dx, int dx_is_f32, long long lddx, const void* dx_accum, long long ldacc,
                                   void* dx_f16_copy, long long ldcopy, int rows, int C, void* stream) {
  VN_REQUIRE(dy && x && gamma && mean && rstd && dx, "layernorm_bwd: null pointer");
  VN_REQUIRE(ldcopy % 8 == 0, "layernorm_bwd: ldcopy % 8 != 0");
  VN_REQUIRE(rows > 0 && C > 0 && C % 8 == 0 && C <= 8 * 64 * LN_MAXC, "layernorm: unsupported C=%d", C);
  VN_REQUIRE(ldx % 8 == 0 && lddy % 8 == 0 && lddx % 8 == 0 && ldacc % 8 == 0, "layernorm_bwd: ld % 8 != 0");
  VN_REQUIRE_OUT("layernorm_bwd", vn_out_bytes(rows, lddx, C, dx_is_f32 ? 4 : 2));
  if (dx_f16_copy) VN_REQUIRE_OUT("layernorm_bwd f16 copy", vn_out_bytes(rows, ldcopy, C, 2));
  hipStream_t st = (hipStream_t)stream;
  dim3 grid(cdiv(rows, 4));
  const int nc = cdiv(C / 8, 64);
#define LN_BWD_N(A, B, Cc, NCH)                                                                                         \
  hipLaunchKernelGGL((ln_bwd_kernel<A, B, Cc, NCH>), grid, dim3(256), 0, st, dy, lddy, x, ldx, gamma, mean, rstd, dx, \
                     lddx, dx_accum, ldacc, (half_t*)dx_f16_copy, ldcopy, rows, C)
#define LN_BWD(A, B, Cc)                      \
  switch (nc) {                               \
    case 1: LN_BWD_N(A, B, Cc, 1); break;     \
    case 2: LN_BWD_N(A, B, Cc, 2); break;     \
    case 3: LN_BWD_N(A, B, Cc, 3); break;     \
    default: LN_BWD_N(A, B, Cc, 4); break;    \
  }
  int key = (dy_is_f32 ? 4 : 0) | (x_is_f32 ? 2 : 0) | (dx_is_f32 ? 1 : 0);
  switch (key) {
    case 0: LN_BWD(false, false, false); break;
    case 1: LN_BWD(false, false, true); break;
    case 2: LN_BWD(false, true, false); break;
    case 3: LN_BWD(false, true, true); break;
    case 4: LN_BWD(true, false, false); break;
    case 5: LN_BWD(true, false, true); break;
    case 6: LN_BWD(true, true, false); break;
    default: LN_BWD(true, true, true); break;
  }
#undef LN_BWD
#undef LN_BWD_N
  return vneti_check_launch("layernorm_bwd");
}

extern "C" int vneti_softmax_rows_f16(void* x, long long ld, int rows, int cols, void* stream) {
  VN_REQUIRE(x && rows > 0 && cols > 0 && cols % 8 == 0 && cols <= 8 * 256 * SM_MAXC && ld % 8 == 0,
             "softmax_rows: unsupported cols=%d ld=%lld", cols, ld);
  hipLaunchKernelGGL(softmax_rows_kernel, dim3(rows), dim3(256), 0, (hipStream_t)stream, (half_t*)x, ld, cols);
  return vneti_check_launch("softmax_rows");
}
```

view_neti_amd/engine/schedule.py:

```python
from __future__ import annotations

from functools import partial
from typing import Dict, List

import torch

from .. import lib, ops, packing


class T:

    __slots__ = ("v", "g", "gw", "rows", "cols", "children", "need_grad", "producer")

    def __init__(self, v, g=None, need_grad=True):
        self.v = v
        self.g = g
        self.gw = False
        self.rows, self.cols = v.shape
        self.children: List["T"] = []
        self.need_grad = need_grad
        self.producer = None


def rup(x, m):
# ... 2 lines not shown

class Schedule:
    def __init__(self, batch: int, groups: int, eps: float, device: str = "cuda", need_backward: bool = True):
        self.B = batch
        self.groups = groups
        self.eps = eps
        self.dev = device
        self.need_backward = need_backward
        self.fwd_pre: List = []
        self.fwd: List = []
        self.bwd: List = []
        self.tape: List = []
        self.bytes = 0
        self._scratch: Dict[str, torch.Tensor] = {}
        self.temb_off: Dict[str, tuple] = {}
        self.temb_all = None
        self.gn_ws = self._buf((batch * 256 * 2 * groups + 2 * batch * groups,), torch.float32)
        self.ws = self._buf((16 * 2 ** 20,), torch.float32)
        self._gn_fusable: List[dict] = []
        self.gn_sums = None
        if ops._default_ws is None or ops._default_ws.device != torch.device(device, torch.cuda.current_device()):
            ops.set_default_gemm_workspace(torch.empty(16 * 2 ** 20, dtype=torch.float32, device=device))

    def _buf(self, shape, dtype=None, zero=False):
        dtype = dtype or lib.act_dtype()
        t = (torch.zeros if zero else torch.empty)(shape, dtype=dtype, device=self.dev)
        self.bytes += t.numel() * t.element_size()
        return t

    def _tmp(self, name, rows, cols, dtype=None):
        dtype = dtype or lib.act_dtype()
        key = f"{name}:{dtype}"
        n = rows * cols
        cur = self._scratch.get(key)
        if cur is None or cur.numel() < n:
            self._scratch[key] = self._buf((n,), dtype)
            cur = self._scratch[key]
        return cur[:n].view(rows, cols)

    def _w16(self, t):
        w = t.to(device=self.dev, dtype=lib.act_dtype()).contiguous()
        self.bytes += w.numel() * 2
        return w

    def _w32(self, t):
        w = t.to(device=self.dev, dtype=torch.float32).contiguous()
        self.bytes += w.numel() * 4
        return w

    def _grad(self, t: T):
        if t.g is None:
            t.g = self._buf((t.rows, t.cols))
        return t.g

    def _contrib(self, t: T, fn, extra=None):
        g = self._grad(t)
        if t.gw:
            if extra is not None:
                self.bwd.append(partial(ops.add, g, extra, g))
            self.bwd.append(self._tagged(partial(fn, g, g), fn))
        else:
            self.bwd.append(self._tagged(partial(fn, g, extra), fn))
            t.gw = True
            for c in t.children:
                c.gw = True

    @staticmethod
    def _tagged(p, fn):
        if hasattr(fn, "vn_cost"):
            p.vn_cost = fn.vn_cost
        return p

    def _contrib_gemm(self, t: T, A, Bm, **kw):
        g = self._grad(t)
        resid = g if t.gw else None
        self.bwd.append(partial(ops.gemm, A, Bm, g, resid=resid, **kw))
        if not t.gw:
            t.gw = True
            for c in t.children:
                c.gw = True

    _tile_cache: Dict[tuple, int] = {}
    _TILE_DIMS = {1: (128, 128), 2: (128, 64), 3: (64, 64), 4: (256, 128), 5: (256, 256), 6: (256, 128), 7: (256, 128),
                  8: (256, 128), 9: (128, 128), 10: (128, 128), 11: (128, 64), 12: (64, 64), 13: (128, 128), 14: (128, 64),
                  15: (64, 64), 16: (256, 256), 17: (256, 128), 18: (256, 128)}

    @staticmethod
    def _gemm_key(f):
        kw = f.keywords
        A, Bm, out = f.args[:3]
        conv = kw.get("conv")
        M = kw.get("M") or A.shape[-2]
        N = kw.get("N") or Bm.shape[-2]
        K = kw.get("K") or Bm.shape[-1]
        ck = (conv["mode"], conv["stride"], conv["ups"], conv["Hi"], conv["Wi"]) if conv else None
        return (M, N, K, kw.get("batch") or 1, ck, out.dtype == torch.float32, kw.get("geglu") or 0)

    def autotune(self, candidates=(1, 2, 3, 5, 6, 7, 8, 9, 10, 11, 12, 13, 14, 15, 16, 17, 18), reps=8):
        if not torch.cuda.is_available():
            return
        import json
        import os
        from .. import parallel
        if os.environ.get("VNETI_AUTOTUNE_CANDS"):
            candidates = tuple(int(x) for x in os.environ["VNETI_AUTOTUNE_CANDS"].split(","))
        how = _timing_switches(self.dev, reps)
        cache = Schedule._tile_cache
        cache_path = os.environ.get("VNETI_AUTOTUNE_CACHE")
        if cache_path and os.path.exists(cache_path) and not cache:
            cache.update(picks_from_json(json.load(open(cache_path))))
        n_before = len(cache)
        share = parallel.sharing_picks() and parallel._dist() is not None
        rank0 = (not share) or parallel._dist().get_rank() == 0
        if share and not rank0:
            cache.update(parallel.share_from_rank0(None))
        for lst in (self.fwd_pre, self.fwd, self.bwd):
            for idx, f in enumerate(lst):
                if getattr(f, "func", None) is not ops.gemm or f.keywords.get("tile_hint"):
                    continue
                key = self._gemm_key(f)
                B_cm = None
                if key not in cache:
                    cache[key], B_cm = self._measure(f, key, candidates, how)
                lst[idx] = self._pin(f, cache[key], B_cm)
        if share and rank0:
            parallel.share_from_rank0(dict(cache))
        if cache_path and len(cache) != n_before and parallel.world_info()[0] == 0:
            tmp = f"{cache_path}.{os.getpid()}.tmp"
            with open(tmp, "w") as fh:
                json.dump(picks_to_json(cache), fh)
            os.replace(tmp, cache_path)

    def _measure(self, f, key, candidates, how):
        conv = f.keywords.get("conv")
        B_cm = packing._chunk_major(f.args[1], f.args[1].shape[0], conv["Ci"]) if _chunk_major_ok(conv) else None
        best, best_t = (0, 0, 0), float("inf")
        for h, sk, ko in gemm_variants(key, conv, f.keywords.get("geglu"), candidates):
            kw = dict(f.keywords)
            kw["tile_hint"], kw["split_k"] = h, sk
            args = f.args
            if ko:
                kw["conv"] = dict(conv, korder=1)
                args = (f.args[0], B_cm) + tuple(f.args[2:])
            t = _time_call(partial(ops.gemm, *args, **kw), args[0], *how)
            if t < best_t:
                best, best_t = (h, sk, ko), t
        return best, B_cm

    def _pin(self, f, pick, B_cm=None):
        pick = tuple(pick) + (0,) * (3 - len(pick))
        conv = f.keywords.get("conv")
        kw = dict(f.keywords)
        kw["tile_hint"], kw["split_k"] = pick[0], pick[1]
        args = f.args
        if pick[2] and _chunk_major_ok(conv):
            if B_cm is None:
                B_cm = packing._chunk_major(f.args[1], f.args[1].shape[0], conv["Ci"])
            kw["conv"] = dict(conv, korder=1)
            self.bytes += B_cm.numel() * B_cm.element_size()
            args = (f.args[0], B_cm) + tuple(f.args[2:])
        return partial(ops.gemm, *args, **kw)

    def bind_workspace(self):
        for lst in (self.fwd_pre, self.fwd, self.bwd):
            for idx, f in enumerate(lst):
                fn = getattr(f, "func", None)
                if fn is ops.gemm or fn is ops.attn_bwd_dkv:
                    lst[idx] = self._rebound(f, fn, dict(f.keywords, workspace=self.ws))

    @staticmethod
    def _rebound(f, fn, kw):
        return partial(fn, *f.args, **kw)

    GN_SLOTS = 8

    def _produced(self, t: T):
        t.producer = len(self.fwd) - 1
        return t

    GN2_MAX = 512

    def _gn2_slice(self):
        if not hasattr(self, "_gn2_arena"):
            self._gn2_arena = self._buf((self.GN2_MAX, self.B, self.GN_SLOTS, self.groups, 4), torch.int64, zero=True)
            self._gn2_used = 0
        assert self._gn2_used < self.GN2_MAX
        self._gn2_used += 1
        return self._gn2_arena[self._gn2_used - 1]

    def fuse_gn_stats(self, fuse: bool = True):
        n = self._fuse_gn_stats() if fuse else 0
        if getattr(self, "_gn2_used", 0):
            self.fwd.insert(0, self._gn2_arena[:self._gn2_used].zero_)
        return n

    def _fuse_gn_stats(self):
        import os
        if os.environ.get("VNETI_NO_GN_FUSE"):
            return 0
        S, G, B = self.GN_SLOTS, self.groups, self.B
        todo = []
        for rec in self._gn_fusable:
            f = self.fwd[rec["prod"]]
            kw = f.keywords
            hw, Cc = rec["hw"], rec["C"]
            cpg = Cc // G
            if getattr(f, "func", None) is ops.conv3x3_in:
                if hw % 256 == 0 and cpg % 4 == 0 and 128 % cpg == 0 and kw.get("gn_sums") is None:
                    todo.append(rec)
                continue
            if getattr(f, "func", None) is not ops.gemm or kw.get("batch"):
                continue
            if kw.get("split_k") != 1:
                M_, N_, K_ = self._gemm_key(f)[:3]
                ws = kw.get("workspace")
                wsb = ws.numel() * ws.element_size() if ws is not None else 0
                if ops.gemm_select_split(M_, N_, K_, 1, kw.get("tile_hint") or 0, wsb) != 1:
                    continue
            if hw < 64 or not (cpg >= 8 or cpg == 4) or kw.get("gn_sums") is not None:
                continue
            todo.append(rec)
        if not todo:
            return 0
        self.gn_sums = self._buf((len(todo), B, S, G, 4), torch.int64, zero=True)
        for i, rec in enumerate(todo):
            sums = self.gn_sums[i]
            f = self.fwd[rec["prod"]]
            kw = dict(f.keywords)
            kw.update(gn_sums=sums, gn_hw=rec["hw"], gn_groups=G, gn_slots=S)
            if f.func is ops.gemm:
                kw.update(split_k=1)
            self.fwd[rec["prod"]] = self._rebound(f, f.func, kw)
            g = rec["gn"]
            self.fwd[rec["idx"]] = partial(ops.groupnorm_fwd_sums, rec["x"], rec["y"], g["gamma"], g["beta"], sums, S,
                                           g["mean"], g["rstd"], B, rec["hw"], rec["C"], G, rec["eps"], rec["silu"])
        arena = self.gn_sums
        self.fwd.insert(0, arena.zero_)
        self._gn_fusable = []
        return len(todo)

    def _gn(self, x: T, name, w, eps, silu):
        Cc = x.cols
        hw = x.rows // self.B
        rec = dict(kind="gn", x=x, gamma=self._w32(w[name + ".weight"]), beta=self._w32(w[name + ".bias"]),
                   mean=self._buf((self.B * self.groups,), torch.float32),
                   rstd=self._buf((self.B * self.groups,), torch.float32), silu=silu, hw=hw)
        y = self._buf((x.rows, Cc))
        import os
        if os.environ.get("VNETI_GN_3L"):
            self.fwd.append(partial(ops.groupnorm_fwd, x.v, y, rec["gamma"], rec["beta"], rec["mean"], rec["rstd"],
                                    self.gn_ws, self.B, hw, Cc, self.groups, eps, silu))
        else:
            self.fwd.append(partial(ops.groupnorm_fwd_2l, x.v, y, rec["gamma"], rec["beta"], self._gn2_slice(),
                                    self.GN_SLOTS, rec["mean"], rec["rstd"], self.B, hw, Cc, self.groups, eps, silu))
            if self.need_backward:
                rec["bsums"] = self._gn2_slice()
        if x.producer is not None:
            self._gn_fusable.append(dict(idx=len(self.fwd) - 1, prod=x.producer, gn=rec, x=x.v, y=y, hw=hw, C=Cc,
                                         eps=eps, silu=silu))
        return y, rec

    def _gn_bwd_fn(self, rec, dy):
        x = rec["x"]
        if "bsums" not in rec:
            fn = lambda out, accum: ops.groupnorm_bwd(dy, x.v, rec["gamma"], rec["beta"], rec["mean"], rec["rstd"], out,
                                                      self.gn_ws, self.B, rec["hw"], x.cols, self.groups,
                                                      rec["silu"], accum=accum)
        else:
            fn = lambda out, accum: ops.groupnorm_bwd_2l(dy, x.v, rec["gamma"], rec["beta"], rec["mean"], rec["rstd"], out,
                                                         rec["bsums"], self.GN_SLOTS, self.gn_ws, self.B, rec["hw"], x.cols,
                                                         self.groups, rec["silu"], accum=accum)
        fn.vn_cost = ("GroupNorm(+SiLU) bwd", 5.0 * self.B * rec["hw"] * x.cols * 2)
        return fn

    def _conv_desc(self, Hi, Wi, Ci, Ho, Wo, stride, pad, ups, ldx, mode=1):
        return dict(mode=mode, Hi=Hi, Wi=Wi, Ci=Ci, Ho=Ho, Wo=Wo, stride=stride, pad_t=pad, pad_l=pad, ups=ups,
                    ldx=ldx, korder=1 if (packing.KORDER_CM and Ci % 64 == 0) else 0)

    def _resnet(self, x: T, cin, cout, name, w, out_view, h, wd, need_dx=True):
        M = x.rows
        n1, gn1 = self._gn(x, name + "norm1", w, self.eps, True)
        w1 = self._w16(packing.conv3x3_fwd(w[name + "conv1.weight"]))
        b1 = self._w32(w[name + "conv1.bias"])
        radd = None
        if name in self.temb_off:
            off, n = self.temb_off[name]
            radd = self.temb_all[:, off:off + n]
        h1 = T(self._buf((M, cout)))
        self.fwd.append(partial(ops.gemm, n1, w1, h1.v, bias=b1, rowadd=radd, rows_per_group=h * wd, M=M,
                                conv=self._conv_desc(h, wd, cin, h, wd, 1, 1, 0, cin)))
        self._produced(h1)
        n2, gn2 = self._gn(h1, name + "norm2", w, self.eps, True)
        w2 = self._w16(packing.conv3x3_fwd(w[name + "conv2.weight"]))
        b2 = self._w32(w[name + "conv2.bias"])
        out = T(out_view if out_view is not None else self._buf((M, cout)))
        wsc = None
        if cin != cout:
            wsc = self._w16(w[name + "conv_shortcut.weight"].reshape(cout, cin))
            bsc = self._w32(w[name + "conv_shortcut.bias"])
            sc_buf = self._buf((M, cout))
            self.fwd.append(partial(ops.gemm, x.v, wsc, sc_buf, bias=bsc))
            resid = sc_buf
        else:
            resid = x.v
        self.fwd.append(partial(ops.gemm, n2, w2, out.v, bias=b2, resid=resid, M=M,
                                conv=self._conv_desc(h, wd, cout, h, wd, 1, 1, 0, cout)))
        self._produced(out)
        rec = dict(kind="resnet", x=x, out=out, h1=h1, gn1=gn1, gn2=gn2, cin=cin, cout=cout, h=h, wd=wd,
                   need_dx=need_dx, name=name)
        if self.need_backward and need_dx:
            rec["w2d"] = self._w16(packing.conv3x3_dgrad(w[name + "conv2.weight"]))
            rec["w1d"] = self._w16(packing.conv3x3_dgrad(w[name + "conv1.weight"]))
            if wsc is not None:
                rec["wscd"] = self._w16(w[name + "conv_shortcut.weight"].reshape(cout, cin).t())
        self.tape.append(rec)
        return out

    def _resnet_bwd(self, r):
        if not r["need_dx"]:
            return
        x, out, h, wd, cin, cout = r["x"], r["out"], r["h"], r["wd"], r["cin"], r["cout"]
        M = x.rows
        dout = out.g
        assert out.gw, f"resnet {r['name']}: output gradient was never produced"
        dn2 = self._tmp("dA", M, cout)
        self.bwd.append(partial(ops.gemm, dout, r["w2d"], dn2, M=M,
                                conv=self._conv_desc(h, wd, cout, h, wd, 1, 1, 0, dout.stride(0), mode=2)))
        dh1 = self._tmp("dB", M, cout)
        self.bwd.append(partial(self._gn_bwd_fn(r["gn2"], dn2), dh1, None))
        dn1 = self._tmp("dC", M, cin)
        self.bwd.append(partial(ops.gemm, dh1, r["w1d"], dn1, M=M,
                                conv=self._conv_desc(h, wd, cout, h, wd, 1, 1, 0, cout, mode=2)))
        if "wscd" in r:
            self._contrib_gemm(x, dout, r["wscd"])
            self._contrib(x, self._gn_bwd_fn(r["gn1"], dn1))
        else:
            self._contrib(x, self._gn_bwd_fn(r["gn1"], dn1), extra=dout)

    def _ln(self, xv, name, w):
        rows, Cc = xv.shape
        rec = dict(x=xv, gamma=self._w32(w[name + ".weight"]), beta=self._w32(w[name + ".bias"]),
                   mean=self._buf((rows,), torch.float32), rstd=self._buf((rows,), torch.float32))
        y = self._buf((rows, Cc))
        self.fwd.append(partial(ops.layernorm_fwd, xv, y, rec["gamma"], rec["beta"], rec["mean"], rec["rstd"], 1e-5))
        return y, rec

    def _ln_bwd(self, rec, dy, dx, accum, f16_copy=None):
        ops.layernorm_bwd(dy, rec["x"], rec["gamma"], rec["mean"], rec["rstd"], dx, accum=accum, f16_copy=f16_copy)

    def _downsample(self, x: T, Cc, name, w, out_view, h, wd, pad=1):
        M = x.rows // 4
        wf = self._w16(packing.conv3x3_fwd(w[name + "weight"]))
        b = self._w32(w[name + "bias"])
        out = T(out_view if out_view is not None else self._buf((M, Cc)))
        self.fwd.append(partial(ops.gemm, x.v, wf, out.v, bias=b, M=M,
                                conv=self._conv_desc(h, wd, Cc, h // 2, wd // 2, 2, pad, 0, x.v.stride(0))))
        self._produced(out)
        rec = dict(kind="down", x=x, out=out, C=Cc, h=h, wd=wd, pad=pad)
        if self.need_backward:
            rec["wd_"] = self._w16(packing.conv3x3_dgrad(w[name + "weight"]))
        self.tape.append(rec)
        return out

    def _downsample_bwd(self, r):
        x, out, Cc, h, wd = r["x"], r["out"], r["C"], r["h"], r["wd"]
        assert out.gw
        desc = self._conv_desc(h // 2, wd // 2, Cc, h, wd, 2, r["pad"], 0, out.g.stride(0), mode=2)
        self._contrib_gemm(x, out.g, r["wd_"], M=x.rows, conv=desc)

    def forward_pre(self):
        for f in self.fwd_pre:
            f()

    def forward_main(self):
        for f in self.fwd:
            f()

    def forward(self):
        self.forward_pre()
        self.forward_main()

    def backward(self):
        for f in self.bwd:
            f()


def _chunk_major_ok(conv) -> bool:
    return bool(conv) and not conv.get("ups") and not conv.get("korder") and \
        not (conv["mode"] == 2 and conv["stride"] == 2) and conv["Ci"] % 64 == 0 and conv["Ci"] >= 128


def gemm_variants(key, conv, geglu, candidates) -> List[tuple]:
    M, N, K, batch = key[:4]
    try_cm = _chunk_major_ok(conv)
    halo_ok = try_cm and conv["mode"] in (1, 2) and conv["stride"] == 1 and conv["pad_t"] == 1 and conv["pad_l"] == 1 \
        and conv["Ho"] % 16 == 0 and conv["Wo"] % 16 == 0 and conv["Hi"] == conv["Ho"] and conv["Wi"] == conv["Wo"]
    tiles_ko = [(h, 0) for h in candidates if h != 18] + \
        ([(h, 1) for h in candidates if h in (16, 17) or (h == 18 and halo_ok)] if try_cm else [])
    out = []
    for h, ko in tiles_ko:
        bm, bn = Schedule._TILE_DIMS[h]
        tiles = -(-M // bm) * -(-N // bn) * batch
        sks = (0, 1) + (tuple(x for x in (2, 3, 4, 6, 8, 12)
                              if x * 8 <= K // 64 and tiles * x <= 1024 and x * batch * M * N <= 16 * 2 ** 20)
                        if tiles < 256 else ())
        if geglu:
            sks = (1,)
        out += [(h, sk, ko) for sk in sks]
    return out


def _timing_switches(dev, reps):
    import os
    cold = None if os.environ.get("VNETI_AUTOTUNE_HOT") else torch.empty(160 * 2 ** 20, dtype=torch.float32, device=dev)
    return (cold, reps, int(os.environ.get("VNETI_AUTOTUNE_REPS", "9")),
            bool(int(os.environ.get("VNETI_AUTOTUNE_WARM_A", "1"))))


def _time_call(call, act, cold, reps, cold_reps, warm_a):
    call()
    call()

    def timed(n):
        s, e = torch.cuda.Event(enable_timing=True), torch.cuda.Event(enable_timing=True)
        s.record()
        for _ in range(n):
            call()
        e.record()
        e.synchronize()
        return s.elapsed_time(e)

    if cold is None:
        return timed(reps)
    ts = []
    for _ in range(cold_reps):
        cold.fill_(0)
        if warm_a:
            act.add_(0)
        ts.append(timed(1))
    return sorted(ts)[len(ts) // 2]


def picks_to_json(cache: Dict) -> Dict:
    return {repr(k): [int(x) for x in v] for k, v in cache.items()}


def picks_from_json(data: Dict) -> Dict:
    import ast
    return {ast.literal_eval(k): tuple(int(x) for x in v) for k, v in data.items()}


def export_picks() -> Dict:
    from ..roofline import kernel_tree_sha
    return {"kernel_tree_sha": kernel_tree_sha(), "picks": picks_to_json(Schedule._tile_cache)}


def preload_picks(data: Dict) -> bool:
    from ..roofline import kernel_tree_sha
    if data.get("kernel_tree_sha") != kernel_tree_sha():
        return False
    Schedule._tile_cache.update(picks_from_json(data["picks"]))
    return True
```

view_neti_amd/engine/unet.py:

```python
from __future__ import annotations

from functools import partial
from typing import Dict

import torch

from .. import ops, packing
from .. import sd_config as sc
from .schedule import Schedule, T, rup as _rup


class UNetEngine(Schedule):
    def __init__(self, cfg: sc.UNetConfig, weights: Dict[str, torch.Tensor], batch: int, height: int, width: int,
                 ctx_len: int = 77, device: str = "cuda", need_backward: bool = True, autotune: bool = True,
                 fuse_gn: bool = True):
        super().__init__(batch, cfg.norm_num_groups, cfg.norm_eps, device, need_backward)
        self.cfg = cfg
        self.H, self.W = height, width
        self.L = ctx_len
        self.nl = cfg.n_cross_layers
        B, L, Dc = batch, ctx_len, cfg.cross_attention_dim
        self.x_in = self._buf((B, cfg.in_channels, height, width), torch.float32)
        self.timesteps = torch.zeros(B, dtype=torch.int64, device=device)
        self.ctx_k = self._buf((self.nl, B * L, Dc))
# ... 65 lines not shown
        while l0 < len(ws):
            n = 1
            while l0 + n < len(ws) and ws[l0 + n] == ws[l0]:
                n += 1
            Cc = ws[l0]
            run = dict(l0=l0, n=n, C=Cc, wk=self._buf((n, Cc, Dc)), wv=self._buf((n, Cc, Dc)),
                       k=self._buf((n, B * L, Cc)), v=self._buf((n, B * L, Cc)))
            if self.need_backward:
                run.update(wkd=self._buf((n, Dc, Cc)), wvd=self._buf((n, Dc, Cc)),
                           dk=self._buf((n, B * L, Cc)), dv=self._buf((n, B * L, Cc)))
            for j in range(n):
                self.kv_slot[l0 + j] = (run, j)
            self.kv_runs.append(run)
            l0 += n

    def _kv_fwd_ops(self):
        B, L, Dc = self.B, self.L, self.cfg.cross_attention_dim
        for run in self.kv_runs:
            l0, n, Cc = run["l0"], run["n"], run["C"]
            for ctx, wgt, out in ((self.ctx_k, run["wk"], run["k"]), (self.ctx_v, run["wv"], run["v"])):
                self.fwd_pre.append(partial(ops.gemm, ctx[l0], wgt[0], out[0], batch=n, strideA=B * L * Dc,
                                            strideB=Cc * Dc, strideC=B * L * Cc))

    def _kv_bwd_ops(self):
        B, L, Dc = self.B, self.L, self.cfg.cross_attention_dim
        for run in self.kv_runs:
            l0, n, Cc = run["l0"], run["n"], run["C"]
            for dsrc, wgt, dctx in ((run["dk"], run["wkd"], self.dctx_k), (run["dv"], run["wvd"], self.dctx_v)):
                self.bwd.append(partial(ops.gemm, dsrc[0], wgt[0], dctx[l0], batch=n, strideA=B * L * Cc,
                                        strideB=Dc * Cc, strideC=B * L * Dc))

    def _transformer(self, x: T, Cc, heads, name, w, layer_idx, out_view, h, wd, need_dx=True):
        cfg = self.cfg
        B, L, Dc = self.B, self.L, cfg.cross_attention_dim
        M, N = x.rows, h * wd
        D = Cc // heads
        scale = D ** -0.5
        t = name + "transformer_blocks.0."
        r = dict(kind="transformer", x=x, C=Cc, heads=heads, D=D, N=N, name=name, layer=layer_idx, need_dx=need_dx,
                 scale=scale)
        g, r["gn"] = self._gn(x, name + "norm", w, 1e-6, False)
        w_in = w[name + "proj_in.weight"].reshape(Cc, Cc)
        r["w_in"], b_in = self._w16(w_in), self._w32(w[name + "proj_in.bias"])
        h0 = self._buf((M, Cc))
        self.fwd.append(partial(ops.gemm, g, r["w_in"], h0, bias=b_in))
        n1, r["ln1"] = self._ln(h0, t + "norm1", w)
        wqkv = torch.cat([w[t + "attn1.to_q.weight"], w[t + "attn1.to_k.weight"], w[t + "attn1.to_v.weight"]], 0)
        r["wqkv"] = self._w16(wqkv)
        qkv = self._buf((M, 3 * Cc))
        self.fwd.append(partial(ops.gemm, n1, r["wqkv"], qkv))
        q, k, v = qkv[:, :Cc], qkv[:, Cc:2 * Cc], qkv[:, 2 * Cc:]
        o1 = self._buf((M, Cc))
        lse1 = self._buf((B, heads, N), torch.float32)
        self.fwd.append(partial(ops.attn_fwd, q, k, v, o1, lse1, B, heads, N, N, D, scale, False))
        r["wo1"], bo1 = self._w16(w[t + "attn1.to_out.0.weight"]), self._w32(w[t + "attn1.to_out.0.bias"])
        h1 = self._buf((M, Cc))
        self.fwd.append(partial(ops.gemm, o1, r["wo1"], h1, bias=bo1, resid=h0))
        n2, r["ln2"] = self._ln(h1, t + "norm2", w)
        r["wq2"] = self._w16(w[t + "attn2.to_q.weight"])
        run, slot = self.kv_slot[layer_idx]
        assert run["C"] == Cc, (name, layer_idx, Cc, run["C"])
        run["wk"][slot].copy_(w[t + "attn2.to_k.weight"])
        run["wv"][slot].copy_(w[t + "attn2.to_v.weight"])
        q2 = self._buf((M, Cc))
        k2, v2 = run["k"][slot], run["v"][slot]
        self.fwd.append(partial(ops.gemm, n2, r["wq2"], q2))
        o2 = self._buf((M, Cc))
        lse2 = self._buf((B, heads, N), torch.float32)
        self.fwd.append(partial(ops.attn_fwd, q2, k2, v2, o2, lse2, B, heads, N, L, D, scale, False))
        r["wo2"], bo2 = self._w16(w[t + "attn2.to_out.0.weight"]), self._w32(w[t + "attn2.to_out.0.bias"])
        h2 = self._buf((M, Cc))
        self.fwd.append(partial(ops.gemm, o2, r["wo2"], h2, bias=bo2, resid=h1))
        n3, r["ln3"] = self._ln(h2, t + "norm3", w)
        wff1_il = packing.geglu_interleave(w[t + "ff.net.0.proj.weight"])
        r["wff1"], bff1 = self._w16(wff1_il), self._w32(packing.geglu_interleave(w[t + "ff.net.0.proj.bias"]))
        r["wff2"], bff2 = self._w16(w[t + "ff.net.2.weight"]), self._w32(w[t + "ff.net.2.bias"])
        p = self._buf((M, 8 * Cc))
        gg = self._buf((M, 4 * Cc))
        self.fwd.append(partial(ops.gemm, n3, r["wff1"], p, bias=bff1, out2=gg, geglu=1, split_k=1))
        h3 = self._buf((M, Cc))
        self.fwd.append(partial(ops.gemm, gg, r["wff2"], h3, bias=bff2, resid=h2))
        r["w_out"], b_out = self._w16(w[name + "proj_out.weight"].reshape(Cc, Cc)), self._w32(w[name + "proj_out.bias"])
        out = T(out_view if out_view is not None else self._buf((M, Cc)))
        self.fwd.append(partial(ops.gemm, h3, r["w_out"], out.v, bias=b_out, resid=x.v))
        self._produced(out)
        r.update(out=out, h0=h0, h1=h1, h2=h2, qkv=qkv, o1=o1, lse1=lse1, q2=q2, k2=k2, v2=v2, o2=o2, lse2=lse2,
                 p=p)
        if self.need_backward:
            tr = lambda a: self._w16(a.t())
            run["wkd"][slot].copy_(w[t + "attn2.to_k.weight"].t())
            run["wvd"][slot].copy_(w[t + "attn2.to_v.weight"].t())
            r["w_outd"] = tr(w[name + "proj_out.weight"].reshape(Cc, Cc))
            r["wff2d"], r["wff1d"] = tr(w[t + "ff.net.2.weight"]), tr(wff1_il)
            r["wo2d"] = tr(w[t + "attn2.to_out.0.weight"])
            if need_dx:
                r["wq2d"] = tr(w[t + "attn2.to_q.weight"])
                r["wo1d"] = tr(w[t + "attn1.to_out.0.weight"])
                r["wqkvd"] = tr(wqkv)
                r["w_ind"] = tr(w_in)
        self.tape.append(r)
        return out

    def _transformer_bwd(self, r):
        B, L, Cc, heads, D, N = self.B, self.L, r["C"], r["heads"], r["D"], r["N"]
        x, out = r["x"], r["out"]
        M = x.rows
        dout = out.g
        assert out.gw, f"transformer {r['name']}: output gradient was never produced"
        li = r["layer"]
        bw = self.bwd
        dh3 = self._tmp("tA", M, Cc)
        bw.append(partial(ops.gemm, dout, r["w_outd"], dh3))
        dp = self._tmp("tC", M, 8 * Cc)
        bw.append(partial(ops.gemm, dh3, r["wff2d"], dp, gate=r["p"], gate_act=ops.ACT_GELU, geglu=2, split_k=1))
        dn3 = self._tmp("tD", M, Cc)
        bw.append(partial(ops.gemm, dp, r["wff1d"], dn3))
        dh2 = self._tmp("tE", M, Cc)
        bw.append(partial(self._ln_bwd, r["ln3"], dn3, dh2, dh3))
        do2 = self._tmp("tA", M, Cc)
        bw.append(partial(ops.gemm, dh2, r["wo2d"], do2))
        delta = self._tmp("tdelta", B * heads, N, torch.float32)
        dq2 = self._tmp("tD", M, Cc)
        if r["need_dx"]:
            bw.append(partial(ops.attn_bwd_dq, r["q2"], r["k2"], r["v2"], do2, r["lse2"], delta, dq2, B, heads, N, L, D,
                              r["scale"], False, O=r["o2"]))
        else:
            bw.append(partial(ops.attn_bwd_delta, do2, r["o2"], delta, B, heads, N, D))
        run, slot = self.kv_slot[li]
        dk2, dv2 = run["dk"][slot], run["dv"][slot]
        bw.append(partial(ops.attn_bwd_dkv, r["q2"], r["k2"], r["v2"], do2, r["lse2"], delta, dk2, dv2, B, heads, N, L,
                          D, r["scale"], False))
        if not r["need_dx"]:
            return
        dn2 = self._tmp("tA", M, Cc)
        bw.append(partial(ops.gemm, dq2, r["wq2d"], dn2))
        dh1 = self._tmp("tF", M, Cc)
        bw.append(partial(self._ln_bwd, r["ln2"], dn2, dh1, dh2))
        do1 = self._tmp("tA", M, Cc)
        bw.append(partial(ops.gemm, dh1, r["wo1d"], do1))
        qkv = r["qkv"]
        q, k, v = qkv[:, :Cc], qkv[:, Cc:2 * Cc], qkv[:, 2 * Cc:]
        dqkv = self._tmp("tC", M, 3 * Cc)
        dq, dk, dv = dqkv[:, :Cc], dqkv[:, Cc:2 * Cc], dqkv[:, 2 * Cc:]
        bw.append(partial(ops.attn_bwd_dq, q, k, v, do1, r["lse1"], delta, dq, B, heads, N, N, D, r["scale"], False,
                          O=r["o1"]))
        bw.append(partial(ops.attn_bwd_dkv, q, k, v, do1, r["lse1"], delta, dk, dv, B, heads, N, N, D, r["scale"],
                          False))
        dn1 = self._tmp("tD", M, Cc)
        bw.append(partial(ops.gemm, dqkv, r["wqkvd"], dn1))
        dh0 = self._tmp("tE", M, Cc)
        bw.append(partial(self._ln_bwd, r["ln1"], dn1, dh0, dh1))
        dg = self._tmp("tA", M, Cc)
        bw.append(partial(ops.gemm, dh0, r["w_ind"], dg))
        self._contrib(x, self._gn_bwd_fn(r["gn"], dg), extra=dout)

    def _upsample(self, x: T, Cc, name, w, out_view, h, wd):
        M = x.rows * 4
        wf = self._w16(packing.conv3x3_fwd(w[name + "weight"]))
        b = self._w32(w[name + "bias"])
        out = T(out_view if out_view is not None else self._buf((M, Cc)))
        self.fwd.append(partial(ops.gemm, x.v, wf, out.v, bias=b, M=M,
                                conv=self._conv_desc(h, wd, Cc, 2 * h, 2 * wd, 1, 1, 1, x.v.stride(0))))
        self._produced(out)
        rec = dict(kind="up", x=x, out=out, C=Cc, h=h, wd=wd)
        if self.need_backward:
            rec["wd_"] = self._w16(packing.conv3x3_dgrad(w[name + "weight"]))
        self.tape.append(rec)
        return out

    def _upsample_bwd(self, r):
        x, out, Cc, h, wd = r["x"], r["out"], r["C"], r["h"], r["wd"]
        assert out.gw and not x.gw
        M = out.rows
        dup = self._tmp("dA", M, Cc)
        self.bwd.append(partial(ops.gemm, out.g, r["wd_"], dup, M=M,
                                conv=self._conv_desc(2 * h, 2 * wd, Cc, 2 * h, 2 * wd, 1, 1, 0, out.g.stride(0), mode=2)))
        g = self._grad(x)
        self.bwd.append(partial(ops.sum2x2, dup, g, self.B, h, wd, Cc))
        x.gw = True

    def _build(self, w):
        cfg = self.cfg
        B, H, W = self.B, self.H, self.W
        boc = cfg.block_out_channels
        nlev = len(boc)
        nres = cfg.layers_per_block + 1
        self._time_ops()
        catT = {}
        for i in range(nlev):
            lvl = nlev - 1 - i
            m = B * (H >> lvl) * (W >> lvl)
            for j in range(nres):
                rin, skip, _ = sc.up_block_channels(cfg, i, j)
                catT[(i, j)] = T(self._buf((m, rin + skip)),
                                 self._buf((m, rin + skip)) if self.need_backward else None)

        def h_slot(key):
            rin = sc.up_block_channels(cfg, *key)[0]
            return catT[key].v[:, :rin]

        def adopt(t: T, key, part):
            rin = sc.up_block_channels(cfg, *key)[0]
            cat = catT[key]
            if cat.g is not None:
                t.g = cat.g[:, :rin] if part == "h" else cat.g[:, rin:]
            cat.children.append(t)
            return t

        skip_targets = list(reversed([(i, j) for i in range(nlev) for j in range(nres)]))
        nskip = [0]

        def next_skip():
            key = skip_targets[nskip[0]]
            nskip[0] += 1
            rin = sc.up_block_channels(cfg, *key)[0]
            return key, catT[key].v[:, rin:]

        M0 = B * H * W
        col = self._buf((M0, 64))
        w_in = self._w16(packing.pad_rows(packing.conv3x3_fwd(w["conv_in.weight"]), 64))
        b_in = self._w32(w["conv_in.bias"])
        key, sv = next_skip()
        self.fwd.append(partial(ops.im2col3x3_small, self.x_in, col, B, cfg.in_channels, H, W, H, W, 1, 1, 1,
                                self.x_in.stride()))
        self.fwd.append(partial(ops.gemm, col, w_in, sv, bias=b_in))
        hcur = adopt(self._produced(T(sv, need_grad=False)), key, "skip")
        layer = 0
        first = True
        cin = boc[0]
        for i, cout in enumerate(boc):
            h, wd = H >> i, W >> i
            for j in range(cfg.layers_per_block):
                name = f"down_blocks.{i}.resnets.{j}."
                key, sv = next_skip()
                if cfg.down_has_attn[i]:
                    r_out = self._resnet(hcur, cin if j == 0 else cout, cout, name, w, None, h, wd, need_dx=not first)
                    hcur = self._transformer(r_out, cout, cfg.num_heads[i], f"down_blocks.{i}.attentions.{j}.", w,
                                             layer, sv, h, wd, need_dx=not first)
                    layer += 1
                else:
                    hcur = self._resnet(hcur, cin if j == 0 else cout, cout, name, w, sv, h, wd, need_dx=not first)
                adopt(hcur, key, "skip")
                first = False
            if i < nlev - 1:
                key, sv = next_skip()
                hcur = self._downsample(hcur, cout, f"down_blocks.{i}.downsamplers.0.conv.", w, sv, h, wd)
                adopt(hcur, key, "skip")
            cin = cout
        assert nskip[0] == len(skip_targets)
        lvl = nlev - 1
        h, wd = H >> lvl, W >> lvl
        cm = boc[-1]
        hcur = self._resnet(hcur, cm, cm, "mid_block.resnets.0.", w, None, h, wd)
        hcur = self._transformer(hcur, cm, cfg.num_heads[-1], "mid_block.attentions.0.", w, layer, None, h, wd)
        layer += 1
        hcur = self._resnet(hcur, cm, cm, "mid_block.resnets.1.", w, h_slot((0, 0)), h, wd)
        adopt(hcur, (0, 0), "h")
        up_has_attn = tuple(reversed(cfg.down_has_attn))
        up_heads = tuple(reversed(cfg.num_heads))
        for i in range(nlev):
            lvl = nlev - 1 - i
            h, wd = H >> lvl, W >> lvl
            for j in range(nres):
                rin, skip, out_c = sc.up_block_channels(cfg, i, j)
                nxt = (i, j + 1) if j < nres - 1 else None
                nxt_view = h_slot(nxt) if nxt is not None else None
                name = f"up_blocks.{i}.resnets.{j}."
                if up_has_attn[i]:
                    r_out = self._resnet(catT[(i, j)], rin + skip, out_c, name, w, None, h, wd)
                    hcur = self._transformer(r_out, out_c, up_heads[i], f"up_blocks.{i}.attentions.{j}.", w, layer,
                                             nxt_view, h, wd)
                    layer += 1
                else:
                    hcur = self._resnet(catT[(i, j)], rin + skip, out_c, name, w, nxt_view, h, wd)
                if nxt is not None:
                    adopt(hcur, nxt, "h")
            if i < nlev - 1:
                out_c = tuple(reversed(boc))[i]
                hcur = self._upsample(hcur, out_c, f"up_blocks.{i}.upsamplers.0.conv.", w, h_slot((i + 1, 0)), h, wd)
                adopt(hcur, (i + 1, 0), "h")
        assert layer == self.nl
        c0 = boc[0]
        n, gn = self._gn(hcur, "conv_norm_out", w, cfg.norm_eps, True)
        w_o = self._w16(packing.conv3x3_fwd(w["conv_out.weight"]))
        b_o = self._w32(w["conv_out.bias"])
        self.fwd.append(partial(ops.gemm, n, w_o, self.pred, bias=b_o, M=M0,
                                conv=self._conv_desc(H, W, c0, H, W, 1, 1, 0, c0)))
        rec = dict(kind="head", x=hcur, gn=gn)
        if self.need_backward:
            wt = w["conv_out.weight"].flip(2, 3).transpose(0, 1).contiguous()
            rec["wd_"] = self._w16(packing.pad_rows(packing.conv3x3_fwd(wt), 64))
        self.tape.append(rec)

    def _head_bwd(self, r):
        x = r["x"]
        M0 = self.B * self.H * self.W
        col = self._tmp("hcol", M0, 64)
        dp = self.dpred
        ld = dp.stride(0)
        self.bwd.append(partial(ops.im2col3x3_small, dp, col, self.B, self.cfg.out_channels, self.H, self.W, self.H,
                                self.W, 1, 1, 1, (self.H * self.W * ld, 1, self.W * ld, ld)))
        dn = self._tmp("dA", M0, x.cols)
        self.bwd.append(partial(ops.gemm, col, r["wd_"], dn))
        self._contrib(x, self._gn_bwd_fn(r["gn"], dn))

    def _build_backward(self):
        for r in reversed(self.tape):
            k = r["kind"]
            if k == "head":
                self._head_bwd(r)
            elif k == "resnet":
                self._resnet_bwd(r)
            elif k == "transformer":
                self._transformer_bwd(r)
            elif k == "down":
                self._downsample_bwd(r)
            elif k == "up":
                self._upsample_bwd(r)
```

view_neti_amd/lib.py:

```python
from __future__ import annotations

import ctypes as C
import keyword
import os
import re

_HERE = os.path.dirname(os.path.abspath(__file__))
HEADER_PATH = os.path.join(os.path.dirname(_HERE), "include", "vneti.h")

_PRECISIONS = {"fp16": ("libvneti_hip.so", 0), "bf16": ("libvneti_hip_bf16.so", 1)}
_precision = os.environ.get("VNETI_PRECISION", "fp16")
if _precision not in _PRECISIONS:
    raise RuntimeError(f"VNETI_PRECISION={_precision!r}: expected one of {sorted(_PRECISIONS)}")

_lib = None


def so_path(precision: str = None) -> str:
    return os.environ.get("VNETI_LIB_PATH") or os.path.join(_HERE, "csrc", _PRECISIONS[precision or _precision][0])


SO_PATH = so_path()


def precision() -> str:
    return _precision


def set_precision(p: str) -> None:
    global _precision, SO_PATH
    if p not in _PRECISIONS:
        raise ValueError(f"precision {p!r}: expected one of {sorted(_PRECISIONS)}")
    if _lib is not None and p != _precision:
        raise RuntimeError(f"libvneti is already loaded in {_precision}; {p} needs its own process")
    _precision = p
    SO_PATH = so_path()


def act_dtype():
    import torch
    return torch.bfloat16 if _precision == "bf16" else torch.float16


_SCALARS = {"int": C.c_int, "long long": C.c_longlong, "float": C.c_float, "unsigned": C.c_uint, "unsigned int": C.c_uint,
            "uint32_t": C.c_uint, "size_t": C.c_size_t}


def _ctype(ctype: str, structs: dict, where: str):
    words = [w for w in ctype.replace("*", " * ").split() if w != "const"]
    stars, base = words.count("*"), " ".join(w for w in words if w != "*")
    if stars == 0 and base in _SCALARS:
        return _SCALARS[base]
    if stars == 1 and base == "char":
        return C.c_char_p
    if stars == 1 and base in structs:
        return C.POINTER(structs[base])
    if stars and (base in _SCALARS or base in ("void", "char")):
        return C.c_void_p
    raise ValueError(f"vneti.h {where}: no ctypes rule for the type {ctype.strip()!r}")


def _declarator(decl: str, where: str):
    m = re.fullmatch(r"(.*[\s*])(\w+)", decl.strip(), re.S)
    if not m:
        raise ValueError(f"vneti.h {where}: cannot read the declaration {' '.join(decl.split())!r}")
    return m.group(1), m.group(2)


def parse_header(text: str):
    blank = lambda m: "\n" * m.group().count("\n")
    text = re.sub(r"/\*.*?\*/|//[^\n]*", blank, text, flags=re.S)
    text = re.sub(r'^[ \t]*#.*$|extern\s+"C"\s*\{|^\}[ \t]*$', "", text, flags=re.M)
    at = lambda src, pos: f"line {src.count(chr(10), 0, pos) + 1}"
    structs, protos = {}, {}
    typedef = r"typedef\s+struct\s+\w*\s*\{(.*?)\}\s*(\w+)\s*;"
    for m in re.finditer(typedef, text, flags=re.S):
        fields = []
        for d in re.finditer(r"[^;\s][^;]*", m.group(1)):
            where = at(text, m.start(1) + d.start())
            first, *more = d.group().split(",")
            ctype, name = _declarator(first, where)
            for n in [name] + [x.strip() for x in more]:
                if not n.isidentifier() or keyword.iskeyword(n):
                    raise ValueError(f"vneti.h {where}: cannot bind the field {n!r}")
                fields.append((n, _ctype(ctype, structs, where)))
        structs[m.group(2)] = type(m.group(2), (C.Structure,), {"_fields_": fields})
    rest = re.sub(typedef, blank, text, flags=re.S)
    for m in re.finditer(r"[^;\s][^;]*", rest):
        p = re.fullmatch(r"(int|long long)\s+(vneti_\w+)\s*\((.*)\)\s*", m.group(), re.S)
        if not p:
            raise ValueError(f"vneti.h {at(rest, m.start())}: cannot read {' '.join(m.group().split())!r} as a prototype")
        argtypes = []
        for x in re.finditer(r"[^,\s][^,]*", "" if p.group(3).strip() == "void" else p.group(3)):
            where = at(rest, m.start() + p.start(3) + x.start())
            argtypes.append(_ctype(_declarator(x.group(), where)[0], structs, where))
        protos[p.group(2)] = (_SCALARS[p.group(1)], argtypes)
    return structs, protos


with open(HEADER_PATH) as _f:
    _STRUCTS, _PROTOS = parse_header(_f.read())
GemmDesc, TransposeDesc = _STRUCTS["vneti_gemm_desc"], _STRUCTS["vneti_transpose_desc"]
SIGNATURES = {n[len("vneti_"):]: argtypes for n, (_, argtypes) in _PROTOS.items()}
VALUE_FUNCS = frozenset({
    "version", "precision", "last_error", "gemm_select_tile", "gemm_select_split", "img_resample_ksize",
    "groupnorm_ws_floats", "lpips_ws_floats", "mse_loss_per_sample_ws_floats", "mapper_num_params", "mapper_save_floats",
    "mapper_rowgrad_floats", "mapper_legacy_input_params", "grad_sumsq_ws_doubles"})
_stray = ({n[len("vneti_"):] for n, (res, _) in _PROTOS.items() if res is C.c_longlong} - VALUE_FUNCS) | (VALUE_FUNCS - set(SIGNATURES))
if _stray:
    raise RuntimeError(f"lib.VALUE_FUNCS is out of step with include/vneti.h: {sorted(_stray)}")


def declared_symbols() -> list[str]:
    src = open(HEADER_PATH).read()
    src = re.sub(r"/\*.*?\*/", "", src, flags=re.S)
    return sorted(set(re.findall(r"\b(vneti_[a-z0-9_]+)\s*\(", src)))


def load():
    global _lib
    if _lib is not None:
        return _lib
    if not os.path.exists(SO_PATH):
        raise RuntimeError(
            f"{os.path.basename(SO_PATH)} not found at {SO_PATH}: build it with "
            "`python view_neti_amd/csrc/build.py` (hipcc, gfx950). There is no fallback path.")
    lib = C.CDLL(SO_PATH)
    for name, (restype, argtypes) in _PROTOS.items():
        fn = getattr(lib, name, None)
        if fn is None:
            raise RuntimeError(f"{SO_PATH} does not export {name}, which include/vneti.h declares: rebuild it")
        fn.restype, fn.argtypes = restype, argtypes
    if lib.vneti_precision() != _PRECISIONS[_precision][1]:
        raise RuntimeError(f"{SO_PATH} computes in precision {lib.vneti_precision()}, the process asked for {_precision}")
    _lib = lib
    return lib


def last_error() -> str:
    lib = load()
    buf = C.create_string_buffer(512)
    lib.vneti_last_error(buf, 512)
    return buf.value.decode(errors="replace")


def check(rc: int, what: str = ""):
    if rc != 0:
        raise RuntimeError(f"vneti call failed ({what}) rc={rc}: {last_error()}")


def call(name: str, *args):
    check(getattr(load(), "vneti_" + name)(*args), name)


def query(name: str, *args) -> int:
    if name not in VALUE_FUNCS:
        raise KeyError(f"vneti_{name} returns a status: use call()")
    return int(getattr(load(), "vneti_" + name)(*args))
```

view_neti_amd/ops.py:

```python
from __future__ import annotations

import ctypes as C

import torch

from . import lib as _l

ACT_NONE, ACT_SILU, ACT_QUICK_GELU, ACT_GELU = 0, 1, 2, 3


def stream() -> int:
    return torch.cuda.current_stream().cuda_stream


def _p(t):
    return None if t is None else t.data_ptr()


def _ld(t):
    if t is None:
        return 0
    assert t.stride(-1) == 1, "last dim must be contiguous"
    return t.stride(-2) if t.dim() >= 2 else t.shape[-1]


_default_ws = None


def set_default_gemm_workspace(t):
    global _default_ws
    _default_ws = t


def gemm(A, B, out, *, bias=None, rowadd=None, rows_per_group=1, resid=None, alpha=1.0, act=0,
         tile_hint=0, batch=0, strideA=0, strideB=0, strideC=0, M=None, N=None, K=None, conv=None,
         lda=None, ldc=None, workspace=None, split_k=0, gate=None, gate_act=0, out2=None, act2=0,
         gn_sums=None, gn_hw=0, gn_groups=0, gn_slots=0, geglu=0):
    d = _l.GemmDesc()
    d.A, d.B, d.C = _p(A), _p(B), _p(out)
    d.ldb = _ld(B)
    d.ldc = ldc if ldc is not None else _ld(out)
    d.N = N if N is not None else B.shape[-2]
    d.K = K if K is not None else B.shape[-1]
    if conv is None:
        d.M = M if M is not None else A.shape[-2]
        d.lda = lda if lda is not None else _ld(A)
        d.conv_mode = 0
    else:
        d.M = M
        d.lda = 0
        d.conv_mode = conv["mode"]
        for k in ("Hi", "Wi", "Ci", "Ho", "Wo", "stride", "pad_t", "pad_l", "ups", "ldx"):
            setattr(d, k, int(conv.get(k, 0)))
        d.conv_korder = int(conv.get("korder", 0))
    d.batch = batch
    d.strideA, d.strideB, d.strideC = strideA, strideB, strideC
    d.bias = _p(bias)
    d.rowadd = _p(rowadd)
    d.ld_rowadd = _ld(rowadd) if rowadd is not None else 0
    d.rows_per_group = rows_per_group
    d.resid = _p(resid)
    d.ldr = _ld(resid) if resid is not None else 0
    d.alpha = alpha
    d.act = act
    d.out_f32 = 1 if out.dtype == torch.float32 else 0
    d.tile_hint = tile_hint
    if gate is not None:
        d.gate_src, d.ld_gate, d.gate_act = _p(gate), _ld(gate), gate_act
    if out2 is not None:
        d.C2, d.ldc2, d.act2 = _p(out2), _ld(out2), act2
    if gn_sums is not None:
        d.gn_sums, d.gn_hw, d.gn_groups, d.gn_slots = _p(gn_sums), gn_hw, gn_groups, gn_slots
        d.gn_cpg = d.N // gn_groups
    d.geglu = geglu
    ws = workspace if workspace is not None else _default_ws
    if ws is not None:
        d.workspace = ws.data_ptr()
        d.workspace_bytes = ws.numel() * ws.element_size()
    d.split_k = split_k if ws is not None else 1
    _l.call("gemm_f16", C.byref(d), stream())


def im2col3x3_small(x, out, Bn, Cc, Hi, Wi, Ho, Wo, stride, pad_t, pad_l, strides):
    sb, sc, sy, sx = strides
    _l.call("im2col3x3_small", _p(x), 1 if x.dtype == torch.float32 else 0, sb, sc, sy, sx, _p(out),
            Bn, Cc, Hi, Wi, Ho, Wo, stride, pad_t, pad_l, stream())


def conv3x3_in(x, w_packed, bias, out, Bn, Cc, H, W, strides, gn_sums=None, gn_hw=0, gn_groups=0, gn_slots=0):
    sb, sc, sy, sx = strides
    assert gn_sums is None or gn_hw == H * W
    _l.call("conv3x3_in", _p(x), 1 if x.dtype == torch.float32 else 0, sb, sc, sy, sx, _p(w_packed), _p(bias), _p(out),
            _ld(out), Bn, Cc, H, W, w_packed.shape[0], _p(gn_sums), gn_groups, gn_slots, stream())


def transpose(inp, out, rows, cols, batch, ld_in, stride_in, ld_out, stride_out):
    _l.call("transpose_f16", _p(inp), ld_in, stride_in, _p(out), ld_out, stride_out, rows, cols, batch, stream())


def transpose_multi(items):
    arr = (_l.TransposeDesc * len(items))()
    for d, (inp, out, rows, cols, batch, ld_in, stride_in, ld_out, stride_out) in zip(arr, items):
        d.inp, d.ld_in, d.stride_in = _p(inp), ld_in, stride_in
        d.out, d.ld_out, d.stride_out = _p(out), ld_out, stride_out
        d.rows, d.cols, d.batch = rows, cols, batch
    _l.call("transpose_f16_multi", arr, len(items), stream())


def groupnorm_ws_floats(Bn, HW, Cc, G):
    n = _l.query("groupnorm_ws_floats", Bn, HW, Cc, G)
    if n < 0:
        raise RuntimeError(f"groupnorm: unsupported shape {(Bn, HW, Cc, G)}")
    return n


def groupnorm_fwd(x, y, gamma, beta, mean, rstd, ws, Bn, HW, Cc, G, eps, silu):
    _l.call("groupnorm_fwd", _p(x), _ld(x), _p(y), _ld(y), _p(gamma), _p(beta), _p(mean), _p(rstd), _p(ws),
            Bn, HW, Cc, G, eps, 1 if silu else 0, stream())


def groupnorm_fwd_sums(x, y, gamma, beta, sums, slots, mean, rstd, Bn, HW, Cc, G, eps, silu):
    _l.call("groupnorm_fwd_sums", _p(x), _ld(x), _p(y), _ld(y), _p(gamma), _p(beta), _p(sums), slots, _p(mean), _p(rstd),
            Bn, HW, Cc, G, eps, 1 if silu else 0, stream())


def groupnorm_fwd_2l(x, y, gamma, beta, sums, slots, mean, rstd, Bn, HW, Cc, G, eps, silu):
    _l.call("groupnorm_fwd_2l", _p(x), _ld(x), _p(y), _ld(y), _p(gamma), _p(beta), _p(sums), slots, _p(mean), _p(rstd),
            Bn, HW, Cc, G, eps, 1 if silu else 0, stream())


def groupnorm_bwd_2l(dy, x, gamma, beta, mean, rstd, dx, sums, slots, ws, Bn, HW, Cc, G, silu, accum=None):
    _l.call("groupnorm_bwd_2l", _p(dy), _ld(dy), _p(x), _ld(x), _p(gamma), _p(beta), _p(mean), _p(rstd),
            _p(dx), _ld(dx), _p(accum), _ld(accum) if accum is not None else 0, _p(sums), slots, _p(ws),
            Bn, HW, Cc, G, 1 if silu else 0, stream())


def groupnorm_bwd(dy, x, gamma, beta, mean, rstd, dx, ws, Bn, HW, Cc, G, silu, accum=None):
    _l.call("groupnorm_bwd", _p(dy), _ld(dy), _p(x), _ld(x), _p(gamma), _p(beta), _p(mean), _p(rstd),
            _p(dx), _ld(dx), _p(accum), _ld(accum) if accum is not None else 0, _p(ws),
            Bn, HW, Cc, G, 1 if silu else 0, stream())


def layernorm_fwd(x, y, gamma, beta, mean, rstd, eps):
    rows, Cc = x.shape
    _l.call("layernorm_fwd", _p(x), 1 if x.dtype == torch.float32 else 0, _ld(x), _p(y), _ld(y), _p(gamma),
            _p(beta), _p(mean), _p(rstd), rows, Cc, eps, stream())


def layernorm_bwd(dy, x, gamma, mean, rstd, dx, accum=None, f16_copy=None):
    rows, Cc = x.shape
    _l.call("layernorm_bwd", _p(dy), 1 if dy.dtype == torch.float32 else 0, _ld(dy), _p(x),
            1 if x.dtype == torch.float32 else 0, _ld(x), _p(gamma), _p(mean), _p(rstd), _p(dx),
            1 if dx.dtype == torch.float32 else 0, _ld(dx), _p(accum),
            _ld(accum) if accum is not None else 0, _p(f16_copy), _ld(f16_copy) if f16_copy is not None else 0,
            rows, Cc, stream())


def attn_fwd(Q, K, V, O, lse, Bn, H, Nq, Nk, D, scale, causal):
    _l.call("attn_fwd", _p(Q), _ld(Q), _p(K), _ld(K), _p(V), _ld(V), _p(O), _ld(O), _p(lse), Bn, H, Nq, Nk, D,
            scale, 1 if causal else 0, stream())


def attn_bwd_delta(dO, O, delta, Bn, H, Nq, D):
    _l.call("attn_bwd_delta", _p(dO), _ld(dO), _p(O), _ld(O), _p(delta), Bn, H, Nq, D, stream())


def attn_bwd_dq(Q, K, V, dO, lse, delta, dQ, Bn, H, Nq, Nk, D, scale, causal, O=None):
    _l.call("attn_bwd_dq", _p(Q), _ld(Q), _p(K), _ld(K), _p(V), _ld(V), _p(dO), _ld(dO), _p(lse), _p(delta),
            _p(O), _ld(O) if O is not None else 0, _p(dQ), _ld(dQ), Bn, H, Nq, Nk, D, scale, 1 if causal else 0,
            stream())


def attn_bwd_dkv(Q, K, V, dO, lse, delta, dK, dV, Bn, H, Nq, Nk, D, scale, causal, workspace=None):
    ws = workspace if workspace is not None else _default_ws
    _l.call("attn_bwd_dkv", _p(Q), _ld(Q), _p(K), _ld(K), _p(V), _ld(V), _p(dO), _ld(dO), _p(lse), _p(delta),
            _p(dK), _ld(dK), _p(dV), _ld(dV), Bn, H, Nq, Nk, D, scale, 1 if causal else 0, _p(ws),
            ws.numel() if ws is not None else 0, stream())


def attn_bwd_small_ok(N, D):
    return N <= 96 and D == 64


def attn_bwd_small(Q, K, V, dO, O, lse, dQ, dK, dV, Bn, H, N, D, scale, causal):
    _l.call("attn_bwd_small", _p(Q), _ld(Q), _p(K), _ld(K), _p(V), _ld(V), _p(dO), _ld(dO), _p(O), _ld(O), _p(lse),
            _p(dQ), _ld(dQ), _p(dK), _ld(dK), _p(dV), _ld(dV), Bn, H, N, D, scale, 1 if causal else 0, stream())


def softmax_rows(x, rows, cols):
    _l.call("softmax_rows_f16", _p(x), _ld(x), rows, cols, stream())


def add(a, b, out):
    rows, cols = out.shape
    _l.call("add_f16", _p(a), _ld(a), _p(b), _ld(b), _p(out), _ld(out), rows, cols, stream())


def geglu_fwd(p, out):
    rows, c4 = out.shape
    _l.call("geglu_fwd", _p(p), _ld(p), _p(out), _ld(out), rows, c4, stream())


def geglu_bwd(dy, p, dp):
    rows, c4 = dy.shape
    _l.call("geglu_bwd", _p(dy), _ld(dy), _p(p), _ld(p), _p(dp), _ld(dp), rows, c4, stream())


def act_fwd(x, y, act):
    _l.call("act_fwd_f16", _p(x), _p(y), x.numel(), act, stream())


def act_bwd(dy, x, dx, act):
    _l.call("act_bwd_f16", _p(dy), _p(x), _p(dx), x.numel(), act, stream())


def timestep_embedding(t, out):
    Bn, dim = out.shape
    _l.call("timestep_embedding", _p(t), _p(out), Bn, dim, stream())


def sum2x2(inp, out, Bn, H, W, Cc):
    _l.call("sum2x2_f16", _p(inp), _ld(inp), _p(out), _ld(out), Bn, H, W, Cc, stream())


def rng_fill_normal(out, state, stream_id):
    _l.call("rng_fill_normal", _p(out), out.numel(), _p(state), stream_id, stream())


def rng_fill_randint(out, high, state, stream_id):
    _l.call("rng_fill_randint", _p(out), out.numel(), high, _p(state), stream_id, stream())


def rng_advance(state):
    _l.call("rng_advance", _p(state), stream())


def sample_add_noise(moments, eps, noise, t, ac, scaling, vpred, latents, noisy, target, Bn, Lc, HW):
    _l.call("sample_add_noise", _p(moments), _ld(moments), _p(eps), _p(noise), _p(t), _p(ac), scaling,
            1 if vpred else 0, _p(latents), _p(noisy), _p(target), Bn, Lc, HW, stream())


def gn_sums_decode(sums: torch.Tensor) -> torch.Tensor:
    import numpy as np
    a = sums.detach().cpu().numpy().astype(np.int64)
    out = np.empty(a.shape[:-1] + (2,), dtype=np.float64)
    for q in range(2):
        hi, lo = a[..., 2 * q].astype(object), a[..., 2 * q + 1].astype(object)
        k = np.vectorize(lambda h, l: (h * 2 ** 36 - l + 2 ** 63) // 2 ** 64, otypes=[object])(hi, lo)
        out[..., q] = np.vectorize(lambda l, kk: float(l + kk * 2 ** 64) / 2.0 ** 40, otypes=[np.float64])(lo, k)
    return torch.from_numpy(out)


def latent_sample(moments, eps, scaling, latents, Bn, Lc, HW):
    _l.call("latent_sample", _p(moments), _ld(moments), _p(eps), scaling, _p(latents), Bn, Lc, HW, stream())


def add_noise(latents, noise, t, ac, vpred, noisy, target, Bn, Lc, HW):
    _l.call("add_noise", _p(latents), _p(noise), _p(t), _p(ac), 1 if vpred else 0, _p(noisy), _p(target), Bn, Lc, HW,
            stream())


def cfg_sampler_step(pred, x, m_prev, x_in, Bn, Lc, HW, guidance, alpha_t, sigma_t, cx, c0, c1, v_prediction):
    _l.call("cfg_sampler_step", _p(pred), _ld(pred), _p(x), _p(m_prev), _p(x_in), Bn, Lc, HW, guidance, alpha_t,
            sigma_t, cx, c0, c1, 1 if v_prediction else 0, stream())


def cfg_sampler_step_table(pred, x, m_prev, x_in, Bn, Lc, HW, guidance, coef_table, step, v_prediction):
    _l.call("cfg_sampler_step_table", _p(pred), _ld(pred), _p(x), _p(m_prev), _p(x_in), Bn, Lc, HW, guidance,
            _p(coef_table), _p(step), 1 if v_prediction else 0, stream())


def cfg_sampler_step_noise(pred, x, m_prev, x_in, noise, Bn, Lc, HW, guidance, alpha_t, sigma_t, cx, c0, c1, cn,
                           v_prediction):
    _l.call("cfg_sampler_step_noise", _p(pred), _ld(pred), _p(x), _p(m_prev), _p(x_in), _p(noise), Bn, Lc, HW, guidance,
            alpha_t, sigma_t, cx, c0, c1, cn, 1 if v_prediction else 0, stream())


def cfg_sampler_step_noise_table(pred, x, m_prev, x_in, Bn, Lc, HW, guidance, coef_table, noise_table, step,
                                 v_prediction):
    _l.call("cfg_sampler_step_noise_table", _p(pred), _ld(pred), _p(x), _p(m_prev), _p(x_in), Bn, Lc, HW, guidance,
            _p(coef_table), _p(noise_table), _p(step), 1 if v_prediction else 0, stream())


def table_fill_i64(dst, table, step):
    _l.call("table_fill_i64", _p(dst), dst.numel(), _p(table), _p(step), stream())


def counter_advance(counter):
    _l.call("counter_advance", _p(counter), stream())


def conv1x1_nchw(x, W, bias, out, Bn, Ci, Co, HW, in_scale=1.0):
# ... 259 lines not shown
```

view_neti_amd/roofline.py:

```python
from __future__ import annotations

import torch

from . import ops

import os as _os

_CSRC = _os.path.join(_os.path.dirname(_os.path.abspath(__file__)), "csrc")
MFMA_PEAK_TFLOPS = 2500.0
HBM_PEAK_TBS = 8.0
PF, TB = MFMA_PEAK_TFLOPS, HBM_PEAK_TBS


def kernel_tree_sha() -> str:
    import hashlib
    import os
    here = _CSRC
    files = sorted(os.path.join(here, f) for f in os.listdir(here) if f.endswith((".hip", ".h")))
    files.append(os.path.join(os.path.dirname(os.path.dirname(here)), "include", "vneti.h"))
    h = hashlib.sha256()
    for f in files:
        h.update(os.path.basename(f).encode())
        h.update(open(f, "rb").read())
    return h.hexdigest()[:16]


def gemm_cost(f):
    kw = f.keywords
    A, Bm = f.args[0], f.args[1]
    M = kw.get("M") or A.shape[-2]
    N, K = kw.get("N") or Bm.shape[-2], kw.get("K") or Bm.shape[-1]
    batch = kw.get("batch") or 1
    conv = kw.get("conv")
    a_bytes = (M // (conv["Ho"] * conv["Wo"])) * conv["Hi"] * conv["Wi"] * conv["Ci"] * 2 if conv else M * K * 2 * batch
    out = f.args[2]
    c_cols = N * (2 if kw.get("geglu") == 2 else 1)
    extra = sum(M * c * 2 for c, key in ((N, "resid"), (N, "out2"), (c_cols, "gate")) if kw.get(key) is not None)
    if kw.get("geglu") == 1:
        extra -= M * N
    nbytes = a_bytes + N * K * 2 * batch + M * c_cols * out.element_size() * batch + extra
    flops = 2.0 * M * N * K * batch
    return M, N, K, batch, flops, nbytes, flops / (MFMA_PEAK_TFLOPS * 1e12), nbytes / (HBM_PEAK_TBS * 1e12)



def cost(f):
    fn, a, kw = getattr(f, "func", None), getattr(f, "args", ()), getattr(f, "keywords", {}) or {}
    if fn is ops.gemm:
        M, N, K, batch, flops, nbytes, t_mfma, t_hbm = gemm_cost(f)
        if t_hbm > t_mfma:
            return ("gemm, below the ridge (short-K linears: HBM-bound)", 0, nbytes)
        return ("gemm / implicit-GEMM conv (MFMA-bound)", flops, 0)
    if fn in (ops.attn_fwd, ops.attn_bwd_dq, ops.attn_bwd_dkv):
        i = {ops.attn_fwd: 5, ops.attn_bwd_dq: 7, ops.attn_bwd_dkv: 8}[fn]
        Bn, H, Nq, Nk, D = a[i:i + 5]
        causal = a[i + 6]
        mm = {ops.attn_fwd: 2, ops.attn_bwd_dq: 3, ops.attn_bwd_dkv: 4}[fn]
        name = {ops.attn_fwd: "attention fwd", ops.attn_bwd_dq: "attention bwd dQ", ops.attn_bwd_dkv: "attention bwd dK/dV"}[fn]
        scores = Bn * H * Nq * Nk * (0.5 if causal else 1.0)
        ks, db = -(-D // 16), -(-D // 32)
        mfma_c = {ops.attn_fwd: ks + 2 * db, ops.attn_bwd_dq: 2 * ks + 2 * db, ops.attn_bwd_dkv: 2 * ks + 4 * db}[fn] * 32 / 1024.0
        valu_c = {ops.attn_fwd: 2.8, ops.attn_bwd_dq: 4.0, ops.attn_bwd_dkv: 4.0}[fn] * 2 / 64.0 + (2 * 5 / 3) / 64.0
        cob = scores * (mfma_c + valu_c) / (1024 * 2.4e9)
        return (name, mm * 2.0 * scores * D, 0, cob)
    if fn is ops.attn_bwd_small:
        Bn, H, N, D = a[9:13]
        return ("attention bwd (short sequences, one launch)", 7 * 2.0 * Bn * H * N * N * D * (0.5 if a[14] else 1.0), 0)
    if fn in (ops.groupnorm_fwd, ops.groupnorm_fwd_sums, ops.groupnorm_fwd_2l):
        Bn, HW, C = (a[7], a[8], a[9]) if fn is ops.groupnorm_fwd else (a[8], a[9], a[10])
        return ("GroupNorm(+SiLU) fwd" + (" (stats in producer)" if fn is ops.groupnorm_fwd_sums else ""), 0, 2.0 * Bn * HW * C * 2)
    if fn is ops.layernorm_fwd:
        x, y = a[0], a[1]
        return ("LayerNorm fwd", 0, x.numel() * x.element_size() + y.numel() * y.element_size())
    if getattr(f, "vn_cost", None) is not None:
        return (f.vn_cost[0], 0, f.vn_cost[1])
    if getattr(fn, "__name__", "") == "_ln_bwd":
        x = a[0]["x"]
        n = x.numel()
        extra = (a[3].numel() * a[3].element_size() if a[3] is not None else 0) + (n * 2 if len(a) > 4 and a[4] is not None else 0)
        return ("LayerNorm bwd", 0, n * x.element_size() + a[1].numel() * a[1].element_size() + a[2].numel() * a[2].element_size() + extra)
    if fn in (ops.groupnorm_bwd, ops.groupnorm_bwd_2l):
        x = a[1]
        return ("GroupNorm(+SiLU) bwd", 0, 5.0 * x.numel() * 2)
    if fn is ops.add:
        return ("elementwise glue (add, 2x2 sum, transposes, noise, loss)", 0, sum(t.numel() * t.element_size() for t in a[:3]))
    if fn is ops.sum2x2:
        return ("elementwise glue (add, 2x2 sum, transposes, noise, loss)", 0, a[0].numel() * 2 + a[1].numel() * 2)
    if fn in (ops.sample_add_noise, ops.mse_loss_grad, getattr(ops, "transpose", None), getattr(ops, "timestep_embedding", None)):
        return ("elementwise glue (add, 2x2 sum, transposes, noise, loss)", 0,
                sum(t.numel() * t.element_size() for t in a if isinstance(t, torch.Tensor)))
    if fn is ops.layernorm_bwd:
        return ("LayerNorm bwd", 0, sum(t.numel() * t.element_size() for t in (a[0], a[1], a[5])))
    if fn is ops.conv3x3_in:
        return ("VAE conv_in (direct)", 0, a[0].numel() * 4 + a[3].numel() * 2)
    if fn is ops.softmax_rows:
        return ("softmax rows (VAE mid attention)", 0, 2.0 * a[0].numel() * 2)
    if fn is ops.geglu_fwd:
        return ("GEGLU fwd", 0, a[0].numel() * 2 + a[1].numel() * 2)
    if fn is ops.geglu_bwd:
        return ("GEGLU bwd", 0, a[0].numel() * 2 + 2 * a[1].numel() * 2)
    return None




def classify(launches):
    classes = {}
    for f in launches:
        c = cost(f)
        if c is None:
            args = list(getattr(f, "args", ())) + list((getattr(f, "keywords", None) or {}).values())
            c = ("small launches (text path, RNG, layout glue)", 0,
                 float(sum(t.numel() * t.element_size() for t in args if isinstance(t, torch.Tensor))) or 1.0)
        d = classes.setdefault(c[0], dict(fs=[], flops=0.0, bytes=0.0, cob=0.0))
        d["fs"].append(f)
        d["flops"] += c[1]
        d["bytes"] += c[2]
        if len(c) > 3:
            d["cob"] += c[3]
    return classes


def time_classes(launches, classes=None, reps: int = 2):
    classes = classes or classify(launches)
    owner = {id(f): name for name, d in classes.items() for f in d["fs"]}
    tot = {name: 0.0 for name in classes}
    for rep in range(reps + 1):
        evs = []
        for f in launches:
            s, e = torch.cuda.Event(enable_timing=True), torch.cuda.Event(enable_timing=True)
            s.record()
            f()
            e.record()
            evs.append((owner[id(f)], s, e))
        torch.cuda.synchronize()
        if rep:
            for name, s, e in evs:
                tot[name] += s.elapsed_time(e)
    out = {}
    for name, d in classes.items():
        ms = tot[name] / reps
        r = dict(launches=len(d["fs"]), ms_per_step=ms)
        if d["flops"]:
            r.update(bound="mfma", algorithmic_gflop=d["flops"] / 1e9, achieved=d["flops"] / (ms * 1e-3) / 1e12, peak=PF,
                     unit="TFLOP/s")
            r["frac"] = r["achieved"] / PF
            if d.get("cob"):
                r["cobound_frac_of_peak"] = d["flops"] / d["cob"] / 1e12 / PF
                r["frac_of_cobound"] = d["cob"] / (ms * 1e-3)
        elif d["bytes"]:
            r.update(bound="hbm", algorithmic_mb=d["bytes"] / 1e6, achieved=d["bytes"] / (ms * 1e-3) / 1e12, peak=TB,
                     unit="TB/s")
            r["frac"] = r["achieved"] / TB
        out[name] = r
    return out
```

Baseline: 38.39 steps/s.

## Fuse split-K partial reduction into following GroupNorm forward and backward kernels

Split-K GEMMs that feed a GroupNorm can now skip their separate reduce kernel and leave fp32 partials in the workspace. The small one-launch GroupNorm kernel sums those partials itself, applying alpha, bias, rowadd and residual, and optionally stores the f16 result. This removes one launch per pair and one f16 write plus read of the activation. The cost is extra validation plumbing, a thread-local flag in the GEMM launcher, and a strict rule that the consumer must be the very next launch.

```diff
diff --git a/include/vneti.h b/include/vneti.h
--- a/include/vneti.h
+++ b/include/vneti.h
@@ -12,6 +12,22 @@
 int vneti_version(void);
 int vneti_precision(void);
 int vneti_last_error(char* buf, size_t n);
+
+typedef struct vneti_splitk_partials {
+  const float* ws;
+  long long zstride;
+  int ksplit;
+  int M, N;
+  float alpha;
+  const float* bias;
+  const void* rowadd;
+  long long ld_rowadd;
+  int rows_per_group;
+  const void* resid;
+  long long ldr;
+  void* C;
+  long long ldc;
+} vneti_splitk_partials;
 
 typedef struct vneti_gemm_desc {
   const void* A;
@@ -47,6 +63,7 @@
   int gn_hw, gn_cpg, gn_groups, gn_slots;
   int geglu;
   int conv_korder;
+  void* leave_partials;
 } vneti_gemm_desc;
 
 int vneti_gemm_f16(const vneti_gemm_desc* d, void* stream);
@@ -93,6 +110,14 @@
                         const float* rstd, void* dx, long long lddx, const void* dx_accum,
                         long long ldacc, float* ws, int Bn, int HW, int C, int G, int silu,
                         void* stream);
+
+int vneti_groupnorm_fwd_partials(const vneti_splitk_partials* p, void* x, long long ldx, void* y, long long ldy,
+                                 const float* gamma, const float* beta, float* mean, float* rstd, int Bn, int HW,
+                                 int C, int G, float eps, int silu, void* stream);
+int vneti_groupnorm_bwd_partials(const vneti_splitk_partials* p, void* dy_out, long long lddy, const void* x,
+                                 long long ldx, const float* gamma, const float* beta, const float* mean,
+                                 const float* rstd, void* dx, long long lddx, const void* dx_accum, long long ldacc,
+                                 int Bn, int HW, int C, int G, int silu, void* stream);
 
 int vneti_layernorm_fwd(const void* x, int x_is_f32, long long ldx, void* y, long long ldy,
                         const float* gamma, const float* beta, float* mean, float* rstd, int rows,
diff --git a/view_neti_amd/csrc/gemm_conv.hip b/view_neti_amd/csrc/gemm_conv.hip
--- a/view_neti_amd/csrc/gemm_conv.hip
+++ b/view_neti_amd/csrc/gemm_conv.hip
@@ -1,5 +1,6 @@
 #include "common.h"
 #include "gemm_args.h"
+#include "splitk_epilogue.h"
 #include "../../include/vneti.h"
 
 namespace {
@@ -578,26 +579,10 @@
     }
     if (g.rowadd) ra = *reinterpret_cast<const half4*>(g.rowadd + (long long)(m / g.rows_per_group) * g.ld_rowadd + c);
     if (g.gate_src) gt = *reinterpret_cast<const half4*>(g.gate_src + (long long)m * g.ld_gate + c);
-    f32x4 v = {0.f, 0.f, 0.f, 0.f};
-    int z = 0;
-    for (; z + 4 <= g.ksplit; z += 4) {
-      const f32x4 t0 = *reinterpret_cast<const f32x4*>(p0 + (z + 0) * zstride);
-      const f32x4 t1 = *reinterpret_cast<const f32x4*>(p0 + (z + 1) * zstride);
-      const f32x4 t2 = *reinterpret_cast<const f32x4*>(p0 + (z + 2) * zstride);
-      const f32x4 t3 = *reinterpret_cast<const f32x4*>(p0 + (z + 3) * zstride);
-      v += t0;
-      v += t1;
-      v += t2;
-      v += t3;
-    }
-    for (; z < g.ksplit; ++z) v += *reinterpret_cast<const f32x4*>(p0 + z * zstride);
+    const f32x4 v = vn_splitk_sum<f32x4>(p0, g.ksplit, zstride);
     float x[4];
 #pragma unroll
-    for (int e = 0; e < 4; ++e) {
-      x[e] = v[e] * g.alpha;
-      if (g.bias) x[e] += bv[e];
-      x[e] = apply_act(x[e], g.act);
-    }
+    for (int e = 0; e < 4; ++e) x[e] = apply_act(vn_splitk_scale_bias(v[e], g.alpha, g.bias != nullptr, bv[e]), g.act);
     if (g.out_f32) {
       f32x4 o = {x[0], x[1], x[2], x[3]};
       if (g.resid) o += rf;
@@ -606,9 +591,7 @@
       half4 o, o2;
 #pragma unroll
       for (int e = 0; e < 4; ++e) {
-        float y = (float)(half_t)x[e];
-        if (g.rowadd) y = (float)(half_t)(y + (float)ra[e]);
-        if (g.resid) y = (float)(half_t)(y + (float)rh[e]);
+        float y = vn_splitk_round_add(x[e], g.rowadd != nullptr, ra[e], g.resid != nullptr, rh[e]);
         if (g.gate_src) y = (float)(half_t)(y * act_grad((float)gt[e], g.gate_act));
         o[e] = (half_t)y;
         o2[e] = (half_t)apply_act((float)(half_t)y, g.act2);
@@ -664,8 +647,10 @@
 #undef VN_GO
 }
 
+thread_local bool t_leave_partials = false;
+
 inline void launch_reduce(const GemmArgs& g, hipStream_t st) {
-  if (g.ksplit > 1) {
+  if (g.ksplit > 1 && !t_leave_partials) {
     long long total = (long long)g.batch * g.M * ((g.N + 3) / 4);
     hipLaunchKernelGGL(splitk_reduce_kernel, dim3((unsigned)cdivl(total, 256)), dim3(256), 0, st, g.ws, g.C, g.bias, g.resid,
                        g.rowadd, g.M, g.N, g.batch, g.ksplit, (int)g.ldc, (int)g.ldr, g);
@@ -901,9 +886,22 @@
   g.ksplit = cdiv(nk, g.kt_per_split);
   VN_REQUIRE(g.ksplit <= 255 && g.kt_per_split <= 0xffff, "gemm: split_k=%d / K=%d out of range", g.ksplit, d->K);
   g.ws = (float*)d->workspace;
+  if (d->leave_partials) {
+    VN_REQUIRE(!f32 && batch == 1 && !d->C2 && !d->geglu && !d->gate_src && !d->act && !d->gn_sums,
+               "gemm: leave_partials supports alpha / bias / rowadd / f16 resid only (out_f32=%d batch=%d C2=%d geglu=%d gate=%d "
+               "act=%d gn_sums=%d)", d->out_f32, batch, d->C2 != nullptr, d->geglu, d->gate_src != nullptr, d->act,
+               d->gn_sums != nullptr);
+    VN_REQUIRE(g.ksplit == 1 || (d->N % 4 == 0 && d->ldc % 4 == 0 && d->ldr % 4 == 0 && d->ld_rowadd % 4 == 0),
+               "gemm: leave_partials needs N, ldc, ldr and ld_rowadd to be multiples of 4");
+  }
+  struct LeaveScope {
+    explicit LeaveScope(bool on) { t_leave_partials = on; }
+    ~LeaveScope() { t_leave_partials = false; }
+  } leave_scope(d->leave_partials != nullptr);
 
 #define LAUNCH(BM, BN, WM, WN) \
   return dma ? launch_cfg<BM, BN, WM, WN, true>(g, f32, st) : launch_cfg<BM, BN, WM, WN, false>(g, f32, st)
+  const auto dispatch = [&]() -> int {
   switch (cfg) {
     case 1: LAUNCH(128, 128, 64, 64);
     case 2: LAUNCH(128, 64, 64, 32);
@@ -930,5 +928,28 @@
     default:
       return dma ? launch_cfg_f16<256, 256, 64, 64, true>(g, st) : launch_cfg_f16<256, 256, 64, 64, false>(g, st);
   }
+  };
 #undef LAUNCH
-}
+  const int rc = dispatch();
+  if (rc == VNETI_OK && d->leave_partials) {
+    vneti_splitk_partials* r = static_cast<vneti_splitk_partials*>(d->leave_partials);
+    memset(r, 0, sizeof(*r));
+    r->ksplit = g.ksplit;
+    r->M = g.M;
+    r->N = g.N;
+    r->C = g.C;
+    r->ldc = g.ldc;
+    if (g.ksplit > 1) {
+      r->ws = g.ws;
+      r->zstride = (long long)g.M * g.N;
+      r->alpha = g.alpha;
+      r->bias = g.bias;
+      r->rowadd = g.rowadd;
+      r->ld_rowadd = g.ld_rowadd;
+      r->rows_per_group = g.rows_per_group;
+      r->resid = g.resid;
+      r->ldr = g.ldr;
+    }
+  }
+  return rc;
+}
diff --git a/view_neti_amd/csrc/norms.hip b/view_neti_amd/csrc/norms.hip
--- a/view_neti_amd/csrc/norms.hip
+++ b/view_neti_amd/csrc/norms.hip
@@ -1,4 +1,5 @@
 #include "common.h"
+#include "splitk_epilogue.h"
 #include "../../include/vneti.h"
 
 namespace {
@@ -373,18 +374,33 @@
   }
 }
 
-template <bool BWD, bool SILU>
+struct GNPartials {
+  const float* ws;
+  long long zstride;
+  int ksplit, N;
+  float alpha;
+  int rows_per_group;
+  const float* bias;
+  const half_t* rowadd;
+  const half_t* resid;
+  long long ld_rowadd, ldr;
+  half_t* store;
+  long long ld_store;
+};
+
+template <bool BWD, bool SILU, bool PART = false, int MAXU = BWD ? 16 : 20>
 __global__ __launch_bounds__(512) void gn_small_kernel(int HW, int C, int G, const half_t* __restrict__ x, long long ldx,
                                                        const half_t* __restrict__ dy, long long lddy,
                                                        const float* __restrict__ gamma, const float* __restrict__ beta,
                                                        float* __restrict__ mean, float* __restrict__ rstd, float eps,
                                                        half_t* __restrict__ out, long long ldo,
-                                                       const half_t* __restrict__ accum, long long ldacc, double inv_n) {
-  constexpr int MAXU = BWD ? 16 : 20;
+                                                       const half_t* __restrict__ accum, long long ldacc, double inv_n,
+                                                       const GNPartials pp) {
   constexpr int NTH = 512;
   __shared__ double red[2][8];
   __shared__ float stat[2];
   __shared__ float sga[128], sbe[128];
+  __shared__ float sbi[PART ? 128 : 1];
   const int gi = blockIdx.x, b = blockIdx.y;
   const int cpg = C / G, hp = cpg / 2;
   const int c0 = gi * cpg;
@@ -394,14 +410,15 @@
   for (int i = threadIdx.x; i < cpg; i += NTH) {
     sga[i] = gamma[c0 + i];
     sbe[i] = beta[c0 + i];
+    if (PART) sbi[i] = pp.bias ? pp.bias[c0 + i] : 0.f;
   }
   float m = 0.f, rs = 0.f;
   if (BWD) {
     m = mean[b * G + gi];
     rs = rstd[b * G + gi];
   }
-  const half_t* xb = x + (long long)b * HW * ldx + c0;
-  const half_t* dyb = BWD ? dy + (long long)b * HW * lddy + c0 : nullptr;
+  const half_t* xb = (PART && !BWD) ? nullptr : x + (long long)b * HW * ldx + c0;
+  const half_t* dyb = (BWD && !PART) ? dy + (long long)b * HW * lddy + c0 : nullptr;
   const half_t* ab = accum ? accum + (long long)b * HW * ldacc + c0 : nullptr;
   const float rcp_hp = __builtin_amdgcn_rcpf((float)hp);
   half2_t xv[MAXU], dv[BWD ? MAXU : 1], av[BWD ? MAXU : 1];
@@ -418,14 +435,59 @@
       av[u] = xv[u];
     }
     if (p < total) {
-      xv[u] = *reinterpret_cast<const half2_t*>(xb + (long long)rows[u] * ldx + cps[u]);
+      if (!(PART && !BWD)) xv[u] = *reinterpret_cast<const half2_t*>(xb + (long long)rows[u] * ldx + cps[u]);
       if (BWD) {
-        dv[u] = *reinterpret_cast<const half2_t*>(dyb + (long long)rows[u] * lddy + cps[u]);
+        if (!PART) dv[u] = *reinterpret_cast<const half2_t*>(dyb + (long long)rows[u] * lddy + cps[u]);
         if (ab) av[u] = *reinterpret_cast<const half2_t*>(ab + (long long)rows[u] * ldacc + cps[u]);
       }
     }
   }
-  __syncthreads();
+  if constexpr (PART) {
+    const unsigned row0 = (unsigned)b * (unsigned)HW;
+    const unsigned rpg = (unsigned)pp.rows_per_group;
+    const unsigned grp0 = row0 / rpg;
+    const bool one_grp = row0 - grp0 * rpg + (unsigned)HW <= rpg;
+    half_t* sb = pp.store ? pp.store + (long long)b * HW * pp.ld_store + c0 : nullptr;
+    constexpr int CH = MAXU <= 10 ? MAXU : MAXU / 2;
+#pragma unroll
+    for (int h = 0; h < MAXU; h += CH) {
+      unsigned off[CH];
+      bool on[CH];
+      half2_t ra[CH], rh[CH];
+#pragma unroll
+      for (int i = 0; i < CH; ++i) {
+        const int u = h + i;
+        on[i] = threadIdx.x + u * NTH < total;
+        const unsigned row = row0 + (unsigned)rows[u];
+        off[i] = on[i] ? row * (unsigned)pp.N + (unsigned)(c0 + cps[u]) : row0 * (unsigned)pp.N + (unsigned)c0;
+        ra[i] = half2_t{(half_t)0.f, (half_t)0.f};
+        rh[i] = ra[i];
+        if (on[i]) {
+          if (pp.rowadd)
+            ra[i] = *reinterpret_cast<const half2_t*>(pp.rowadd + (long long)(one_grp ? grp0 : row / rpg) * pp.ld_rowadd + c0 + cps[u]);
+          if (pp.resid) rh[i] = *reinterpret_cast<const half2_t*>(pp.resid + (long long)row * pp.ldr + c0 + cps[u]);
+        }
+      }
+      f32x2 acc[CH];
+      vn_splitk_sum_n<f32x2, CH, (CH <= 4 ? 8 : 2)>(pp.ws, off, pp.ksplit, pp.zstride, acc);
+      if (h == 0) __syncthreads();
+#pragma unroll
+      for (int i = 0; i < CH; ++i) {
+        const int u = h + i;
+        if (!on[i]) continue;
+        half2_t r;
+#pragma unroll
+        for (int j = 0; j < 2; ++j)
+          r[j] = (half_t)vn_splitk_round_add(vn_splitk_scale_bias(acc[i][j], pp.alpha, pp.bias != nullptr, sbi[cps[u] + j]),
+                                             pp.rowadd != nullptr, ra[i][j], pp.resid != nullptr, rh[i][j]);
+        if (BWD) dv[u] = r;
+        else xv[u] = r;
+        if (sb) *reinterpret_cast<half2_t*>(sb + (long long)rows[u] * pp.ld_store + cps[u]) = r;
+      }
+    }
+  } else {
+    __syncthreads();
+  }
   float s0 = 0.f, s1 = 0.f;
 #pragma unroll
   for (int u = 0; u < MAXU; ++u) {
@@ -512,6 +574,8 @@
   if (cpg % 2 != 0 || cpg > 128 || getenv("VNETI_GN_NO_SMALL")) return false;
   return (long long)HW * cpg * 2 <= (bwd ? 32 : 40) * 1024 && Bn * G >= 64;
 }
+
+inline int gn_small_pairs(int HW, int C, int G) { return (HW * (C / G / 2) + 511) / 512; }
 
 int gn_geom(GNGeom& g, int Bn, int HW, int C, int G) {
   if (Bn <= 0 || HW <= 0 || C <= 0 || G <= 0 || G > 64 || C % G != 0 || C % 8 != 0) return -1;
@@ -783,11 +847,11 @@
     if (silu)
       hipLaunchKernelGGL((gn_small_kernel<false, true>), dim3(G, Bn), dim3(512), 0, st, HW, C, G, (const half_t*)x, ldx,
                          (const half_t*)nullptr, 0LL, gamma, beta, mean, rstd, eps, (half_t*)y, ldy,
-                         (const half_t*)nullptr, 0LL, g.inv_n);
+                         (const half_t*)nullptr, 0LL, g.inv_n, GNPartials{});
     else
       hipLaunchKernelGGL((gn_small_kernel<false, false>), dim3(G, Bn), dim3(512), 0, st, HW, C, G, (const half_t*)x, ldx,
                          (const half_t*)nullptr, 0LL, gamma, beta, mean, rstd, eps, (half_t*)y, ldy,
-                         (const half_t*)nullptr, 0LL, g.inv_n);
+                         (const half_t*)nullptr, 0LL, g.inv_n, GNPartials{});
     return vneti_check_launch("groupnorm_fwd");
   }
   dim3 grid(g.nslab, Bn);
@@ -866,11 +930,11 @@
     if (silu)
       hipLaunchKernelGGL((gn_small_kernel<true, true>), dim3(G, Bn), dim3(512), 0, st, HW, C, G, (const half_t*)x, ldx,
                          (const half_t*)dy, lddy, gamma, beta, const_cast<float*>(mean), const_cast<float*>(rstd), 0.f,
-                         (half_t*)dx, lddx, (const half_t*)dx_accum, ldacc, g.inv_n);
+                         (half_t*)dx, lddx, (const half_t*)dx_accum, ldacc, g.inv_n, GNPartials{});
     else
       hipLaunchKernelGGL((gn_small_kernel<true, false>), dim3(G, Bn), dim3(512), 0, st, HW, C, G, (const half_t*)x, ldx,
                          (const half_t*)dy, lddy, gamma, beta, const_cast<float*>(mean), const_cast<float*>(rstd), 0.f,
-                         (half_t*)dx, lddx, (const half_t*)dx_accum, ldacc, g.inv_n);
+                         (half_t*)dx, lddx, (const half_t*)dx_accum, ldacc, g.inv_n, GNPartials{});
     return vneti_check_launch("groupnorm_bwd");
   }
   dim3 grid(g.nslab, Bn);
@@ -892,6 +956,81 @@
                        (const half_t*)dy, lddy, gamma, beta, mean, rstd, (const float*)c1, (const float*)c2,
                        (half_t*)dx, lddx, (const half_t*)dx_accum, ldacc);
   return vneti_check_launch("groupnorm_bwd");
+}
+
+static int gn_partials_args(GNPartials& pp, const char* who, const vneti_splitk_partials* p, void* store, long long ld_store,
+                            int Bn, int HW, int C, int G, bool bwd) {
+  VN_REQUIRE(p && p->ksplit > 1 && p->ws, "%s: needs the report of a split launch (ksplit > 1)", who);
+  VN_REQUIRE(gn_use_small(Bn, HW, C, G, bwd), "%s: B=%d HW=%d C=%d G=%d is beyond the one-launch GroupNorm", who, Bn, HW, C, G);
+  VN_REQUIRE(p->N == C && (long long)p->M == (long long)Bn * HW && p->zstride == (long long)p->M * p->N,
+             "%s: the partials are [%d][%d], the tensor is [%d][%d]", who, p->M, p->N, Bn * HW, C);
+  VN_REQUIRE((long long)p->ksplit * p->zstride * 4 < 0x7fffffffLL, "%s: partials larger than 2 GiB", who);
+  VN_REQUIRE(p->N % 4 == 0 && p->ldr % 4 == 0 && p->ld_rowadd % 4 == 0 && ld_store % 8 == 0 && p->rows_per_group > 0,
+             "%s: bad leading dimension", who);
+  pp.ws = p->ws;
+  pp.zstride = p->zstride;
+  pp.ksplit = p->ksplit;
+  pp.N = p->N;
+  pp.alpha = p->alpha;
+  pp.rows_per_group = p->rows_per_group;
+  pp.bias = p->bias;
+  pp.rowadd = (const half_t*)p->rowadd;
+  pp.resid = (const half_t*)p->resid;
+  pp.ld_rowadd = p->ld_rowadd;
+  pp.ldr = p->ldr;
+  pp.store = (half_t*)store;
+  pp.ld_store = ld_store;
+  return VNETI_OK;
+}
+
+extern "C" int vneti_groupnorm_fwd_partials(const vneti_splitk_partials* p, void* x, long long ldx, void* y, long long ldy,
+                                            const float* gamma, const float* beta, float* mean, float* rstd, int Bn,
+                                            int HW, int C, int G, float eps, int silu, void* stream) {
+  GNGeom g;
+  VN_REQUIRE(gn_geom(g, Bn, HW, C, G) == 0, "groupnorm: unsupported shape B=%d HW=%d C=%d G=%d", Bn, HW, C, G);
+  VN_REQUIRE(x && y && gamma && beta && mean && rstd, "groupnorm_fwd_partials: null pointer");
+  VN_REQUIRE(ldx % 8 == 0 && ldy % 8 == 0, "groupnorm_fwd_partials: ld must be a multiple of 8");
+  GNPartials pp;
+  const int rc = gn_partials_args(pp, "groupnorm_fwd_partials", p, x, ldx, Bn, HW, C, G, false);
+  if (rc != VNETI_OK) return rc;
+  VN_REQUIRE(x == p->C && ldx == p->ldc, "groupnorm_fwd_partials: x must be the C of the launch that left the partials");
+  VN_REQUIRE_OUT("groupnorm_fwd_partials", vn_out_bytes((long long)Bn * HW, ldy, C, 2));
+  hipStream_t st = (hipStream_t)stream;
+#define VN_GO(S, U)                                                                                                       \
+  hipLaunchKernelGGL((gn_small_kernel<false, S, true, U>), dim3(G, Bn), dim3(512), 0, st, HW, C, G, (const half_t*)nullptr, \
+                     0LL, (const half_t*)nullptr, 0LL, gamma, beta, mean, rstd, eps, (half_t*)y, ldy,                       \
+                     (const half_t*)nullptr, 0LL, g.inv_n, pp)
+  const int nu = gn_small_pairs(HW, C, G);
+  if (silu) { if (nu <= 4) VN_GO(true, 4); else if (nu <= 10) VN_GO(true, 10); else VN_GO(true, 20); }
+  else { if (nu <= 4) VN_GO(false, 4); else if (nu <= 10) VN_GO(false, 10); else VN_GO(false, 20); }
+#undef VN_GO
+  return vneti_check_launch("groupnorm_fwd_partials");
+}
+
+extern "C" int vneti_groupnorm_bwd_partials(const vneti_splitk_partials* p, void* dy_out, long long lddy, const void* x,
+                                            long long ldx, const float* gamma, const float* beta, const float* mean,
+                                            const float* rstd, void* dx, long long lddx, const void* dx_accum,
+                                            long long ldacc, int Bn, int HW, int C, int G, int silu, void* stream) {
+  GNGeom g;
+  VN_REQUIRE(gn_geom(g, Bn, HW, C, G) == 0, "groupnorm: unsupported shape B=%d HW=%d C=%d G=%d", Bn, HW, C, G);
+  VN_REQUIRE(x && gamma && beta && mean && rstd && dx, "groupnorm_bwd_partials: null pointer");
+  VN_REQUIRE(ldx % 8 == 0 && lddx % 8 == 0 && ldacc % 8 == 0, "groupnorm_bwd_partials: ld %% 8 != 0");
+  GNPartials pp;
+  const int rc = gn_partials_args(pp, "groupnorm_bwd_partials", p, dy_out, lddy, Bn, HW, C, G, true);
+  if (rc != VNETI_OK) return rc;
+  VN_REQUIRE(!dy_out || (dy_out == p->C && lddy == p->ldc),
+             "groupnorm_bwd_partials: dy_out must be NULL or the C of the launch that left the partials");
+  VN_REQUIRE_OUT("groupnorm_bwd_partials", vn_out_bytes((long long)Bn * HW, lddx, C, 2));
+  hipStream_t st = (hipStream_t)stream;
+#define VN_GO(S, U)                                                                                                      \
+  hipLaunchKernelGGL((gn_small_kernel<true, S, true, U>), dim3(G, Bn), dim3(512), 0, st, HW, C, G, (const half_t*)x, ldx, \
+                     (const half_t*)nullptr, 0LL, gamma, beta, const_cast<float*>(mean), const_cast<float*>(rstd), 0.f,   \
+                     (half_t*)dx, lddx, (const half_t*)dx_accum, ldacc, g.inv_n, pp)
+  const int nu = gn_small_pairs(HW, C, G);
+  if (silu) { if (nu <= 4) VN_GO(true, 4); else if (nu <= 10) VN_GO(true, 10); else VN_GO(true, 16); }
+  else { if (nu <= 4) VN_GO(false, 4); else if (nu <= 10) VN_GO(false, 10); else VN_GO(false, 16); }
+#undef VN_GO
+  return vneti_check_launch("groupnorm_bwd_partials");
 }
 
 extern "C" int vneti_groupnorm_bwd_2l(const void* dy, long long lddy, const void* x, long long ldx, const float* gamma,
diff --git a/view_neti_amd/csrc/splitk_epilogue.h b/view_neti_amd/csrc/splitk_epilogue.h
--- /dev/null
+++ b/view_neti_amd/csrc/splitk_epilogue.h
@@ -0,0 +1,63 @@
+#pragma once
+#include "common.h"
+
+namespace {
+
+template <typename V>
+__device__ __forceinline__ V vn_splitk_sum(const float* __restrict__ p0, int ksplit, long long zstride) {
+  V v = {};
+  int z = 0;
+  for (; z + 4 <= ksplit; z += 4) {
+    const V t0 = *reinterpret_cast<const V*>(p0 + (z + 0) * zstride);
+    const V t1 = *reinterpret_cast<const V*>(p0 + (z + 1) * zstride);
+    const V t2 = *reinterpret_cast<const V*>(p0 + (z + 2) * zstride);
+    const V t3 = *reinterpret_cast<const V*>(p0 + (z + 3) * zstride);
+    v += t0;
+    v += t1;
+    v += t2;
+    v += t3;
+  }
+  for (; z < ksplit; ++z) v += *reinterpret_cast<const V*>(p0 + z * zstride);
+  return v;
+}
+
+template <typename V, int NE, int ZC>
+__device__ __forceinline__ void vn_splitk_trip(const float* __restrict__ pz, const unsigned (&off)[NE], long long zstride,
+                                               V (&v)[NE]) {
+  V t[ZC][NE];
+#pragma unroll
+  for (int k = 0; k < ZC; ++k)
+#pragma unroll
+    for (int u = 0; u < NE; ++u) t[k][u] = *reinterpret_cast<const V*>(pz + k * zstride + off[u]);
+#pragma unroll
+  for (int u = 0; u < NE; ++u)
+#pragma unroll
+    for (int k = 0; k < ZC; ++k) v[u] += t[k][u];
+}
+
+template <typename V, int NE, int ZMAX>
+__device__ __forceinline__ void vn_splitk_sum_n(const float* __restrict__ ws, const unsigned (&off)[NE], int ksplit,
+                                                long long zstride, V (&v)[NE]) {
+#pragma unroll
+  for (int u = 0; u < NE; ++u) v[u] = V{};
+  int z = 0;
+  if constexpr (ZMAX >= 8)
+    for (; z + 8 <= ksplit; z += 8) vn_splitk_trip<V, NE, 8>(ws + z * zstride, off, zstride, v);
+  if constexpr (ZMAX >= 4)
+    for (; z + 4 <= ksplit; z += 4) vn_splitk_trip<V, NE, 4>(ws + z * zstride, off, zstride, v);
+  for (; z + 2 <= ksplit; z += 2) vn_splitk_trip<V, NE, 2>(ws + z * zstride, off, zstride, v);
+  if (z < ksplit) vn_splitk_trip<V, NE, 1>(ws + z * zstride, off, zstride, v);
+}
+
+__device__ __forceinline__ float vn_splitk_scale_bias(float sum, float alpha, bool has_bias, float bias) {
+  return has_bias ? __builtin_fmaf(sum, alpha, bias) : sum * alpha;
+}
+
+__device__ __forceinline__ float vn_splitk_round_add(float x, bool has_rowadd, half_t rowadd, bool has_resid, half_t resid) {
+  float y = (float)(half_t)x;
+  if (has_rowadd) y = (float)(half_t)(y + (float)rowadd);
+  if (has_resid) y = (float)(half_t)(y + (float)resid);
+  return y;
+}
+
+}
diff --git a/view_neti_amd/engine/schedule.py b/view_neti_amd/engine/schedule.py
--- a/view_neti_amd/engine/schedule.py
+++ b/view_neti_amd/engine/schedule.py
@@ -178,6 +178,7 @@
         conv = f.keywords.get("conv")
         kw = dict(f.keywords)
         kw["tile_hint"], kw["split_k"] = pick[0], pick[1]
+        kw.pop("partials", None)
         args = f.args
         if pick[2] and _chunk_major_ok(conv):
             if B_cm is None:
@@ -216,6 +217,7 @@
 
     def fuse_gn_stats(self, fuse: bool = True):
         n = self._fuse_gn_stats() if fuse else 0
+        self.pair_splitk_gn()
         if getattr(self, "_gn2_used", 0):
             self.fwd.insert(0, self._gn2_arena[:self._gn2_used].zero_)
         return n
@@ -264,6 +266,92 @@
         self.fwd.insert(0, arena.zero_)
         self._gn_fusable = []
         return len(todo)
+
+    def _splits(self, f):
+        kw = f.keywords
+        sk = kw.get("split_k") or 0
+        if sk == 0:
+            M_, N_, K_ = self._gemm_key(f)[:3]
+            ws = kw.get("workspace") if kw.get("workspace") is not None else ops._default_ws
+            wsb = ws.numel() * ws.element_size() if ws is not None else 0
+            sk = ops.gemm_select_split(M_, N_, K_, 1, kw.get("tile_hint") or 0, wsb)
+        return sk
+
+    GN_PARTIALS_MAX_SLICE = 8 * 1024
+
+    def _gn_partials_slice(self):
+        import os
+        return int(os.environ.get("VNETI_GN_PARTIALS_SLICE", self.GN_PARTIALS_MAX_SLICE))
+
+    def _pairable_gemm(self, f, t, bwd):
+        if getattr(f, "func", None) is not ops.gemm:
+            return 0
+        kw, out = f.keywords, f.args[2]
+        if any(kw.get(k) for k in ("act", "geglu", "batch")) or out.dtype == torch.float32 or \
+                any(kw.get(k) is not None for k in ("gate", "out2", "gn_sums", "partials")):
+            return 0
+        if out.data_ptr() != t.data_ptr() or out.shape != t.shape or out.stride() != t.stride():
+            return 0
+        rows, Cc = t.shape
+        N_ = kw.get("N") or f.args[1].shape[-2]
+        if N_ != Cc or N_ % 4 or rows % self.B or not ops.gn_use_small(self.B, rows // self.B, Cc, self.groups, bwd):
+            return 0
+        if (rows // self.B) * (Cc // self.groups) * 2 > self._gn_partials_slice():
+            return 0
+        if any(x is not None and x.stride(0) % 4 for x in (out, kw.get("resid"), kw.get("rowadd"))):
+            return 0
+        sk = self._splits(f)
+        return sk if sk > 1 else 0
+
+    def pair_splitk_gn(self):
+        import os
+        self.gn_partial_pairs = (0, 0)
+        if os.environ.get("VNETI_NO_GN_PARTIALS"):
+            return 0, 0
+        nf = nb = 0
+        for i in range(len(self.fwd) - 1):
+            f, nxt = self.fwd[i], self.fwd[i + 1]
+            fn = getattr(nxt, "func", None)
+            if fn is ops.groupnorm_fwd_2l:
+                x, y, ga, be, _, _, mean, rstd = nxt.args[:8]
+                tail = nxt.args[8:]
+            elif fn is ops.groupnorm_fwd:
+                x, y, ga, be, mean, rstd = nxt.args[:6]
+                tail = nxt.args[7:]
+            else:
+                continue
+            sk = self._pairable_gemm(f, x, False)
+            if not sk:
+                continue
+            part = ops.splitk_partials()
+            self.fwd[i] = self._rebound(f, ops.gemm, dict(f.keywords, partials=part))
+            self.fwd[i + 1] = partial(ops.groupnorm_fwd_partials, part, x, y, ga, be, mean, rstd, self.gn_ws, *tail,
+                                      ksplit_hint=sk)
+            nf += 1
+        for i in range(len(self.bwd) - 1):
+            f, nxt = self.bwd[i], self.bwd[i + 1]
+            info = getattr(getattr(nxt, "func", None), "vn_gn", None)
+            if info is None:
+                continue
+            rec, dy, private = info
+            sk = self._pairable_gemm(f, dy, True)
+            if not sk:
+                continue
+            part = ops.splitk_partials()
+            self.bwd[i] = self._rebound(f, ops.gemm, dict(f.keywords, partials=part))
+            fn2 = self._gn_bwd_fn(rec, dy, private, part=part, ksplit_hint=sk)
+            self.bwd[i + 1] = self._tagged(partial(fn2, *nxt.args), fn2)
+            nb += 1
+        for lst in (self.fwd, self.bwd):
+            for i, f in enumerate(lst):
+                part = (getattr(f, "keywords", None) or {}).get("partials") if getattr(f, "func", None) is ops.gemm else None
+                if part is not None:
+                    nxt = lst[i + 1] if i + 1 < len(lst) else None
+                    cons = nxt.args[0] if getattr(nxt, "func", None) is ops.groupnorm_fwd_partials else \
+                        getattr(getattr(nxt, "func", None), "vn_part", None)
+                    assert cons is part, f"launch {i}: the partials of a split-K GEMM must be consumed by the very next launch"
+        self.gn_partial_pairs = (nf, nb)
+        return nf, nb
 
     def _gn(self, x: T, name, w, eps, silu):
         Cc = x.cols
@@ -286,8 +374,16 @@
                                          eps=eps, silu=silu))
         return y, rec
 
-    def _gn_bwd_fn(self, rec, dy):
+    def _gn_bwd_fn(self, rec, dy, dy_private=False, part=None, ksplit_hint=0):
         x = rec["x"]
+        if part is not None:
+            fn = lambda out, accum: ops.groupnorm_bwd_partials(part, dy, x.v, rec["gamma"], rec["beta"], rec["mean"],
+                                                               rec["rstd"], out, self.gn_ws, self.B, rec["hw"], x.cols,
+                                                               self.groups, rec["silu"], accum=accum, store_dy=not dy_private)
+            n = self.B * rec["hw"] * x.cols
+            fn.vn_cost = ("GroupNorm(+SiLU) bwd (reduces split-K partials)", n * (4.0 * ksplit_hint + 2 * 2 + (0 if dy_private else 2)))
+            fn.vn_part = part
+            return fn
         if "bsums" not in rec:
             fn = lambda out, accum: ops.groupnorm_bwd(dy, x.v, rec["gamma"], rec["beta"], rec["mean"], rec["rstd"], out,
                                                       self.gn_ws, self.B, rec["hw"], x.cols, self.groups,
@@ -297,6 +393,7 @@
                                                          rec["bsums"], self.GN_SLOTS, self.gn_ws, self.B, rec["hw"], x.cols,
                                                          self.groups, rec["silu"], accum=accum)
         fn.vn_cost = ("GroupNorm(+SiLU) bwd", 5.0 * self.B * rec["hw"] * x.cols * 2)
+        fn.vn_gn = (rec, dy, dy_private)
         return fn
 
     def _conv_desc(self, Hi, Wi, Ci, Ho, Wo, stride, pad, ups, ldx, mode=1):
@@ -353,15 +450,15 @@
         self.bwd.append(partial(ops.gemm, dout, r["w2d"], dn2, M=M,
                                 conv=self._conv_desc(h, wd, cout, h, wd, 1, 1, 0, dout.stride(0), mode=2)))
         dh1 = self._tmp("dB", M, cout)
-        self.bwd.append(partial(self._gn_bwd_fn(r["gn2"], dn2), dh1, None))
+        self.bwd.append(partial(self._gn_bwd_fn(r["gn2"], dn2, dy_private=True), dh1, None))
         dn1 = self._tmp("dC", M, cin)
         self.bwd.append(partial(ops.gemm, dh1, r["w1d"], dn1, M=M,
                                 conv=self._conv_desc(h, wd, cout, h, wd, 1, 1, 0, cout, mode=2)))
         if "wscd" in r:
             self._contrib_gemm(x, dout, r["wscd"])
-            self._contrib(x, self._gn_bwd_fn(r["gn1"], dn1))
+            self._contrib(x, self._gn_bwd_fn(r["gn1"], dn1, dy_private=True))
         else:
-            self._contrib(x, self._gn_bwd_fn(r["gn1"], dn1), extra=dout)
+            self._contrib(x, self._gn_bwd_fn(r["gn1"], dn1, dy_private=True), extra=dout)
 
     def _ln(self, xv, name, w):
         rows, Cc = xv.shape
diff --git a/view_neti_amd/engine/unet.py b/view_neti_amd/engine/unet.py
--- a/view_neti_amd/engine/unet.py
+++ b/view_neti_amd/engine/unet.py
@@ -241,7 +241,7 @@
         bw.append(partial(self._ln_bwd, r["ln1"], dn1, dh0, dh1))
         dg = self._tmp("tA", M, Cc)
         bw.append(partial(ops.gemm, dh0, r["w_ind"], dg))
-        self._contrib(x, self._gn_bwd_fn(r["gn"], dg), extra=dout)
+        self._contrib(x, self._gn_bwd_fn(r["gn"], dg, dy_private=True), extra=dout)
 
     def _upsample(self, x: T, Cc, name, w, out_view, h, wd):
         M = x.rows * 4
@@ -391,7 +391,7 @@
                                 self.W, 1, 1, 1, (self.H * self.W * ld, 1, self.W * ld, ld)))
         dn = self._tmp("dA", M0, x.cols)
         self.bwd.append(partial(ops.gemm, col, r["wd_"], dn))
-        self._contrib(x, self._gn_bwd_fn(r["gn"], dn))
+        self._contrib(x, self._gn_bwd_fn(r["gn"], dn, dy_private=True))
 
     def _build_backward(self):
         for r in reversed(self.tape):
diff --git a/view_neti_amd/lib.py b/view_neti_amd/lib.py
--- a/view_neti_amd/lib.py
+++ b/view_neti_amd/lib.py
@@ -101,6 +101,7 @@
 with open(HEADER_PATH) as _f:
     _STRUCTS, _PROTOS = parse_header(_f.read())
 GemmDesc, TransposeDesc = _STRUCTS["vneti_gemm_desc"], _STRUCTS["vneti_transpose_desc"]
+SplitKPartials = _STRUCTS["vneti_splitk_partials"]
 SIGNATURES = {n[len("vneti_"):]: argtypes for n, (_, argtypes) in _PROTOS.items()}
 VALUE_FUNCS = frozenset({
     "version", "precision", "last_error", "gemm_select_tile", "gemm_select_split", "img_resample_ksize",
diff --git a/view_neti_amd/ops.py b/view_neti_amd/ops.py
--- a/view_neti_amd/ops.py
+++ b/view_neti_amd/ops.py
@@ -35,7 +35,7 @@
 def gemm(A, B, out, *, bias=None, rowadd=None, rows_per_group=1, resid=None, alpha=1.0, act=0,
          tile_hint=0, batch=0, strideA=0, strideB=0, strideC=0, M=None, N=None, K=None, conv=None,
          lda=None, ldc=None, workspace=None, split_k=0, gate=None, gate_act=0, out2=None, act2=0,
-         gn_sums=None, gn_hw=0, gn_groups=0, gn_slots=0, geglu=0):
+         gn_sums=None, gn_hw=0, gn_groups=0, gn_slots=0, geglu=0, partials=None):
     d = _l.GemmDesc()
     d.A, d.B, d.C = _p(A), _p(B), _p(out)
     d.ldb = _ld(B)
@@ -78,6 +78,8 @@
         d.workspace = ws.data_ptr()
         d.workspace_bytes = ws.numel() * ws.element_size()
     d.split_k = split_k if ws is not None else 1
+    if partials is not None:
+        d.leave_partials = C.addressof(partials)
     _l.call("gemm_f16", C.byref(d), stream())
 
 
@@ -138,6 +140,33 @@
 def groupnorm_bwd(dy, x, gamma, beta, mean, rstd, dx, ws, Bn, HW, Cc, G, silu, accum=None):
     _l.call("groupnorm_bwd", _p(dy), _ld(dy), _p(x), _ld(x), _p(gamma), _p(beta), _p(mean), _p(rstd),
             _p(dx), _ld(dx), _p(accum), _ld(accum) if accum is not None else 0, _p(ws),
+            Bn, HW, Cc, G, 1 if silu else 0, stream())
+
+
+def splitk_partials():
+    return _l.SplitKPartials()
+
+
+def gn_use_small(Bn, HW, Cc, G, bwd):
+    import os
+    cpg = Cc // G
+    if cpg % 2 or cpg > 128 or os.environ.get("VNETI_GN_NO_SMALL"):
+        return False
+    return HW * cpg * 2 <= (32 if bwd else 40) * 1024 and Bn * G >= 64
+
+
+def groupnorm_fwd_partials(part, x, y, gamma, beta, mean, rstd, ws, Bn, HW, Cc, G, eps, silu, ksplit_hint=0):
+    if part.ksplit <= 1:
+        return groupnorm_fwd(x, y, gamma, beta, mean, rstd, ws, Bn, HW, Cc, G, eps, silu)
+    _l.call("groupnorm_fwd_partials", C.byref(part), _p(x), _ld(x), _p(y), _ld(y), _p(gamma), _p(beta), _p(mean), _p(rstd),
+            Bn, HW, Cc, G, eps, 1 if silu else 0, stream())
+
+
+def groupnorm_bwd_partials(part, dy, x, gamma, beta, mean, rstd, dx, ws, Bn, HW, Cc, G, silu, accum=None, store_dy=True):
+    if part.ksplit <= 1:
+        return groupnorm_bwd(dy, x, gamma, beta, mean, rstd, dx, ws, Bn, HW, Cc, G, silu, accum=accum)
+    _l.call("groupnorm_bwd_partials", C.byref(part), _p(dy) if store_dy else None, _ld(dy) if store_dy else 0, _p(x), _ld(x),
+            _p(gamma), _p(beta), _p(mean), _p(rstd), _p(dx), _ld(dx), _p(accum), _ld(accum) if accum is not None else 0,
             Bn, HW, Cc, G, 1 if silu else 0, stream())
 
 
diff --git a/view_neti_amd/roofline.py b/view_neti_amd/roofline.py
--- a/view_neti_amd/roofline.py
+++ b/view_neti_amd/roofline.py
@@ -69,6 +69,10 @@
     if fn in (ops.groupnorm_fwd, ops.groupnorm_fwd_sums, ops.groupnorm_fwd_2l):
         Bn, HW, C = (a[7], a[8], a[9]) if fn is ops.groupnorm_fwd else (a[8], a[9], a[10])
         return ("GroupNorm(+SiLU) fwd" + (" (stats in producer)" if fn is ops.groupnorm_fwd_sums else ""), 0, 2.0 * Bn * HW * C * 2)
+    if fn is ops.groupnorm_fwd_partials:
+        part, x = a[0], a[1]
+        ks = part.ksplit if part.ksplit > 1 else kw.get("ksplit_hint") or 1
+        return ("GroupNorm(+SiLU) fwd (reduces split-K partials)", 0, x.numel() * (4.0 * ks + 2 * 2))
     if fn is ops.layernorm_fwd:
         x, y = a[0], a[1]
         return ("LayerNorm fwd", 0, x.numel() * x.element_size() + y.numel() * y.element_size())
```

Result: no change. 38.39 steps/s (-0.0%).
